# ronantakizawa/cudabulletproof

Measured on AMD Instinct MI355X. Metric: 64-bit range-proof verifies/sec (batched), higher is better.
Workload: dtype u64

## Files before the change

### cudabulletproof_amd/__init__.py

```python
import ctypes
import os
import subprocess

import numpy as np

HERE = os.path.dirname(os.path.abspath(__file__))
ROOT = os.path.dirname(HERE)
LIB_PATH = os.path.join(HERE, "libcudabulletproof_hip.so")
CSRC = os.path.join(HERE, "csrc")
SOURCES = ["bp_terms1.hip", "bp_terms2.hip", "bp_terms4.hip", "bp_terms16.hip", "bp_kernels.hip", "bp_prove.hip",
           "bp_prove_seed.hip", "bp_ipa_prove.hip", "bp_pippenger.hip", "bp_capi.hip"]

_lib = None


class BulletproofError(RuntimeError):
    pass


def build(force=False, verbose=False):
    srcs = [os.path.join(CSRC, s) for s in SOURCES]
    deps = srcs + [os.path.join(CSRC, f) for f in os.listdir(CSRC) if f.endswith(".h")]
    deps.append(os.path.join(ROOT, "include", "cudabulletproof_hip.h"))
    if not force and os.path.exists(LIB_PATH):
        t = os.path.getmtime(LIB_PATH)
        if all(os.path.getmtime(d) <= t for d in deps):
            return LIB_PATH
    import tempfile
    flags = ["--offload-arch=gfx950", "-O3", "-std=c++17", "-fPIC", "-Wno-unused-result"]
    flags += os.environ.get("HIPBP_EXTRA_CFLAGS", "").split()
    with tempfile.TemporaryDirectory() as tmp:
        objs = [os.path.join(tmp, os.path.basename(s) + ".o") for s in srcs]
        procs = []
        for s, o in zip(srcs, objs):
            cmd = ["hipcc"] + flags + ["-c", s, "-o", o]
            if verbose:
                print(" ".join(cmd))
            procs.append((cmd, subprocess.Popen(cmd)))
        for cmd, p in procs:
            if p.wait() != 0:
                raise subprocess.CalledProcessError(p.returncode, cmd)
        cmd = ["hipcc", "--offload-arch=gfx950", "-shared", "-fPIC", "-o", LIB_PATH + ".tmp"] + objs
        if verbose:
            print(" ".join(cmd))
        subprocess.check_call(cmd)
    os.replace(LIB_PATH + ".tmp", LIB_PATH)
    return LIB_PATH


_c = ctypes.c_void_p
_sz = ctypes.c_size_t


class FieldVector(ctypes.Structure):
    _fields_ = [("elements", _c), ("length", _sz)]


PointVector = FieldVector


class InnerProductProof(ctypes.Structure):
    _fields_ = [("n", _sz), ("a", FieldVector), ("b", FieldVector), ("c", ctypes.c_uint64 * 4),
                ("L", PointVector), ("R", PointVector), ("L_len", _sz), ("x", ctypes.c_uint64 * 4)]


class RangeProofC(ctypes.Structure):
    _fields_ = [("V", ctypes.c_uint64 * 16), ("A", ctypes.c_uint64 * 16), ("S", ctypes.c_uint64 * 16),
                ("T1", ctypes.c_uint64 * 16), ("T2", ctypes.c_uint64 * 16), ("taux", ctypes.c_uint64 * 4),
                ("mu", ctypes.c_uint64 * 4), ("t", ctypes.c_uint64 * 4), ("ip_proof", InnerProductProof)]


class ProofBatchC(ctypes.Structure):
    _fields_ = [("count", _sz), ("n", _sz), ("ab_len", _sz), ("L_len", _sz)] + \
               [(k, _c) for k in ("V", "A", "S", "T1", "T2", "t", "a", "b", "c", "x", "L", "R", "taux", "mu", "Vp")]


class ProveInputC(ctypes.Structure):
    _fields_ = [("count", _sz), ("n", _sz)] + [(k, _c) for k in ("v", "gamma", "sL", "sR", "rnd")]


class ProofOutC(ctypes.Structure):
    _fields_ = [(k, _c) for k in ("V", "A", "S", "T1", "T2", "taux", "mu", "t", "c", "x", "a", "b", "L", "R", "valid")]


class ProveIpaInputC(ctypes.Structure):
    _fields_ = [("count", _sz), ("n", _sz)] + [(k, _c) for k in ("a", "b", "c", "transcript")]


class IpaProofOutC(ctypes.Structure):
    _fields_ = [(k, _c) for k in ("a", "b", "c", "x", "c_final", "L", "R")]


assert ctypes.sizeof(InnerProductProof) == 144 and ctypes.sizeof(RangeProofC) == 880

EXPORTS = [
    "cuda_point_vector_multi_scalar_mul", "cuda_point_vector_multi_scalar_mul_shared",
    "cuda_field_vector_inner_product", "cuda_field_vector_inner_product_shared",
    "cuda_batch_field_vector_inner_product", "cuda_batch_field_add", "cuda_batch_field_sub",
    "cuda_batch_field_mul", "cuda_batch_field_mul_karatsuba", "cuda_batch_field_square",
    "cuda_batch_field_invert", "cuda_soa_field_add", "cuda_range_proof_verify", "cuda_inner_product_verify",
    "cuda_benchmark_multi_scalar_mul", "cuda_benchmark_inner_product", "cuda_benchmark_field_operations",
    "cuda_benchmark_range_proof", "hipbp_last_error", "hipbp_device_count", "hipbp_batch_range_proof_verify",
    "hipbp_batch_range_proof_verify_std", "hipbp_batch_range_proof_verify_gens", "hipbp_batch_inner_product_verify", "hipbp_batch_generate_range_proof", "hipbp_msm",
    "hipbp_msm_pippenger", "hipbp_msm_pippenger_batch", "hipbp_msm_pippenger_windows",
    "hipbp_msm_pippenger_horner", "hipbp_msm_batch", "hipbp_msm_batch_gens", "hipbp_point_tree", "hipbp_field_op",
    "hipbp_sha_probe", "hipbp_sync", "hipbp_timing_enable",
    "hipbp_timing_collect", "hipbp_kernel_count", "hipbp_kernel_name", "hipbp_pipeline_create",
    "hipbp_pipeline_push", "hipbp_pipeline_flush", "hipbp_pipeline_depth", "hipbp_pipeline_destroy",
    "hipbp_pipeline_defer_msm",
    "hipbp_release_stream_workspaces",
    "hipbp_batch_inner_product_prove", "hipbp_batch_inner_product_prove_gens", "hipbp_inner_product_prove_host",
    "hipbp_derive_prover_scalars", "hipbp_batch_generate_range_proof_seeded",
    "hipbp_batch_generate_range_proof_seeded_gens", "hipbp_batch_generate_range_proof_host",
    "hipbp_batch_generate_range_proof_accepted", "hipbp_batch_generate_range_proof_accepted_gens",
    "hipbp_derive_prover_scalars_at", "hipbp_accepted_last_stats",
]


def lib():
    global _lib
    if _lib is None:
        if not os.path.exists(LIB_PATH):
            raise BulletproofError(f"{LIB_PATH} missing: run cudabulletproof_amd.build() (hipcc, gfx950)")
        try:
            import torch
        except ImportError:
            pass
        L = ctypes.CDLL(LIB_PATH)
        L.hipbp_last_error.restype = ctypes.c_char_p
        for f in ("cuda_range_proof_verify", "cuda_inner_product_verify"):
            getattr(L, f).restype = ctypes.c_bool
        for f in ("hipbp_batch_range_proof_verify", "hipbp_batch_range_proof_verify_host",
                  "hipbp_batch_range_proof_verify_std", "hipbp_batch_range_proof_verify_gens",
                  "hipbp_batch_inner_product_verify", "hipbp_batch_generate_range_proof", "hipbp_msm",
                  "hipbp_msm_pippenger", "hipbp_msm_pippenger_batch", "hipbp_msm_pippenger_windows",
                  "hipbp_msm_pippenger_horner", "hipbp_msm_batch", "hipbp_msm_batch_gens", "hipbp_point_tree",
                  "hipbp_field_op", "hipbp_sha_probe", "hipbp_sync", "hipbp_device_count",
                  "hipbp_release_stream_workspaces", "hipbp_batch_inner_product_prove",
                  "hipbp_batch_inner_product_prove_gens", "hipbp_inner_product_prove_host",
                  "hipbp_derive_prover_scalars", "hipbp_batch_generate_range_proof_seeded",
                  "hipbp_batch_generate_range_proof_seeded_gens", "hipbp_batch_generate_range_proof_host",
                  "hipbp_batch_generate_range_proof_accepted", "hipbp_batch_generate_range_proof_accepted_gens",
                  "hipbp_derive_prover_scalars_at", "hipbp_accepted_last_stats"):
            getattr(L, f).restype = ctypes.c_int
        _lib = L
    return _lib


def require_gpu():
    n = lib().hipbp_device_count()
    if n < 1:
        raise BulletproofError("no HIP device visible: the engine has no CPU fallback")
    return n


def _chk(rc):
    if rc != 0:
        raise BulletproofError(lib().hipbp_last_error().decode())


def _p(a):
    return ctypes.c_void_p(a.ctypes.data)


def _u64(a, last):
    a = np.ascontiguousarray(a, dtype=np.uint64)
    if a.shape[-1] != last:
        raise ValueError(f"expected trailing dimension {last}, got {a.shape}")
    return a


def cuda_point_vector_multi_scalar_mul(scalars, points, shared=False):
    require_gpu()
    s, P = _u64(scalars, 4), _u64(points, 16)
    if len(s) != len(P):
        raise ValueError("Vector lengths must match for multi-scalar multiplication")
    out = np.zeros(16, np.uint64)
    sv, pv = FieldVector(_p(s).value, len(s)), PointVector(_p(P).value, len(P))
    f = lib().cuda_point_vector_multi_scalar_mul_shared if shared else lib().cuda_point_vector_multi_scalar_mul
    f(_p(out), ctypes.byref(sv), ctypes.byref(pv))
    return out


def cuda_field_vector_inner_product(a, b, shared=False):
    require_gpu()
    a, b = _u64(a, 4), _u64(b, 4)
    out = np.zeros(4, np.uint64)
    av, bv = FieldVector(_p(a).value, len(a)), FieldVector(_p(b).value, len(b))
    f = lib().cuda_field_vector_inner_product_shared if shared else lib().cuda_field_vector_inner_product
    f(_p(out), ctypes.byref(av), ctypes.byref(bv))
    return out


def cuda_batch_field_vector_inner_product(a_vectors, b_vectors):
    require_gpu()
    a, b = _u64(a_vectors, 4), _u64(b_vectors, 4)
    nv, n = a.shape[0], a.shape[1]
    av = (FieldVector * nv)(*[FieldVector(_p(a).value + i * n * 32, n) for i in range(nv)])
    bv = (FieldVector * nv)(*[FieldVector(_p(b).value + i * n * 32, n) for i in range(nv)])
    out = np.zeros((nv, 4), np.uint64)
    lib().cuda_batch_field_vector_inner_product(_p(out), av, bv, _sz(nv))
    return out


def _field(name, a, b=None):
    require_gpu()
    a = _u64(a, 4).reshape(-1, 4)
    out = np.zeros_like(a)
    if b is None:
        getattr(lib(), name)(_p(out), _p(a), _sz(len(a)))
    else:
        b = _u64(b, 4).reshape(-1, 4)
        if len(b) != len(a):
            raise ValueError("length mismatch")
        getattr(lib(), name)(_p(out), _p(a), _p(b), _sz(len(a)))
    return out


def cuda_batch_field_add(a, b):
    return _field("cuda_batch_field_add", a, b)


def cuda_batch_field_sub(a, b):
    return _field("cuda_batch_field_sub", a, b)


def cuda_batch_field_mul(a, b):
    return _field("cuda_batch_field_mul", a, b)


def cuda_batch_field_mul_karatsuba(a, b):
    return _field("cuda_batch_field_mul_karatsuba", a, b)


def cuda_batch_field_square(a):
    return _field("cuda_batch_field_square", a)


def cuda_batch_field_invert(a):
    return _field("cuda_batch_field_invert", a)


def cuda_soa_field_add(a, b):
    return _field("cuda_soa_field_add", a, b)


def _range_proof_struct(proof, n, keep):
    head = np.asarray(proof["head"], np.uint64)
    a, b = _u64(proof["a"], 4), _u64(proof["b"], 4)
    L, R = _u64(proof["L"], 16).reshape(-1, 16), _u64(proof["R"], 16).reshape(-1, 16)
    keep += [a, b, L, R]
    rp = RangeProofC()
    for i, k in enumerate(("V", "A", "S", "T1", "T2")):
        getattr(rp, k)[:] = [int(v) for v in head[16 * i:16 * i + 16]]
    for i, k in enumerate(("taux", "mu", "t")):
        getattr(rp, k)[:] = [int(v) for v in head[80 + 4 * i:84 + 4 * i]]
    ip = rp.ip_proof
    ip.n = n
    ip.a = FieldVector(_p(a).value, len(a))
    ip.b = FieldVector(_p(b).value, len(b))
    ip.c[:] = [int(v) for v in head[92:96]]
    ip.L = PointVector(_p(L).value, len(L))
    ip.R = PointVector(_p(R).value, len(R))
    ip.L_len = len(L)
    ip.x[:] = [int(v) for v in head[96:100]]
    return rp


def cuda_range_proof_verify(proof, V, n, G, H, g, h):
    require_gpu()
    keep = []
    rp = _range_proof_struct(proof, n, keep)
    V, g, h = _u64(V, 16), _u64(g, 16), _u64(h, 16)
    G, H = _u64(G, 16), _u64(H, 16)
    gv, hv = PointVector(_p(G).value, len(G)), PointVector(_p(H).value, len(H))
    return bool(lib().cuda_range_proof_verify(ctypes.byref(rp), _p(V), _sz(n), ctypes.byref(gv), ctypes.byref(hv),
                                              _p(g), _p(h)))


def batch_range_proof_verify_host(proofs, V, n, G, H, g, h, num_gpus=0):
    require_gpu()
    keep = []
    count = len(proofs)
    arr = (RangeProofC * max(count, 1))()
    for i, pr in enumerate(proofs):
        arr[i] = _range_proof_struct(pr, n, keep)
    V = _u64(V, 16).reshape(-1, 16)
    g, h = _u64(g, 16), _u64(h, 16)
    G, H = _u64(G, 16), _u64(H, 16)
    gv, hv = PointVector(_p(G).value, len(G)), PointVector(_p(H).value, len(H))
# ... 263 lines not shown
    require_gpu()
    sd = _seed_arg(seed)
    v, gamma = _u64(v, 4).reshape(-1, 4), _u64(gamma, 4).reshape(-1, 4)
    if len(v) != len(gamma):
        raise ValueError("v and gamma must have the same length")
    G, H, g, h = _u64(G, 16), _u64(H, 16), _u64(g, 16), _u64(h, 16)
    count = len(v)
    arr = (RangeProofC * max(count, 1))()
    valid = np.zeros(max(count, 1), np.uint8)
    gv, hv = PointVector(_p(G).value, len(G)), PointVector(_p(H).value, len(H))
    _chk(lib().hipbp_batch_generate_range_proof_host(arr, _p(valid), _p(v), _p(gamma), _sz(count), _sz(int(n)),
                                                     ctypes.byref(gv), ctypes.byref(hv), _p(g), _p(h), sd,
                                                     ctypes.c_uint64(int(index_base) & (2**64 - 1))))
    proofs = []
    for i in range(count):
        rp = arr[i]
        ip = rp.ip_proof
        head = np.concatenate([np.array(getattr(rp, k), np.uint64) for k in ("V", "A", "S", "T1", "T2", "taux", "mu", "t")] +
                              [np.array(ip.c, np.uint64), np.array(ip.x, np.uint64)])
        proofs.append(dict(head=head, a=_take(ip.a, 4), b=_take(ip.b, 4), L=_take(ip.L, 16), R=_take(ip.R, 16),
                           n=int(ip.n), L_len=int(ip.L_len)))
    return proofs, valid[:count].astype(bool)


def batch_inner_product_prove(n, a, b, c, G, H, Q, transcript=None, stream=None, gens=None):
    import contextlib

    import torch
    B = int(a.shape[0])
    Lr = int(n).bit_length() - 1
    dev = a.device
    with torch.cuda.stream(stream) if stream is not None else contextlib.nullcontext():
        z = lambda *shape: torch.empty(*shape, dtype=torch.int64, device=dev)
        out = dict(a=z(B, 1, 4), b=z(B, 1, 4), c=z(B, 4), x=z(B, 4), c_final=z(B, 4), L=z(B, max(Lr, 0), 16),
                   R=z(B, max(Lr, 0), 16))
    ins = [t.contiguous() for t in (a, b, c)] + [transcript.contiguous() if transcript is not None else None]
    if ins[0].numel() != B * int(n) * 4 or ins[1].numel() != B * int(n) * 4 or ins[2].numel() != B * 4:
        raise BulletproofError("batch_inner_product_prove: a, b must be (B, n, 4) and c (B, 4)")
    ic = ProveIpaInputC(B, int(n), *[t.data_ptr() if t is not None else None for t in ins])
    oc = IpaProofOutC(*[out[k].data_ptr() if out[k].numel() else None for k in ("a", "b", "c", "x", "c_final", "L", "R")])
    if gens is not None:
        _chk(lib().hipbp_batch_inner_product_prove_gens(ctypes.byref(ic), _c(gens.h), ctypes.byref(oc),
                                                        _stream_ptr(stream)))
    else:
        _chk(lib().hipbp_batch_inner_product_prove(ctypes.byref(ic), _c(G.data_ptr()), _c(H.data_ptr()),
                                                   _c(Q.data_ptr()), ctypes.byref(oc), _stream_ptr(stream)))
    out["_keep"] = ins
    return out


def ipa_proof_batch(n, proof, c="c_final"):
    import torch
    if c not in ("c", "c_final"):
        raise ValueError("c must be 'c' or 'c_final'")
    B, dev = int(proof["a"].shape[0]), proof["a"].device
    zp = torch.zeros(B, 16, dtype=torch.int64, device=dev)
    return RangeProofBatch(n, V=zp, A=zp, S=zp, T1=zp, T2=zp, t=torch.zeros(B, 4, dtype=torch.int64, device=dev),
                           a=proof["a"], b=proof["b"], c=proof[c], x=proof["x"], L=proof["L"], R=proof["R"])


def inner_product_prove(a, b, G, H, Q, c, transcript=None):
    require_gpu()
    a, b, G, H = _u64(a, 4), _u64(b, 4), _u64(G, 16), _u64(H, 16)
    Q, c = _u64(Q, 16), _u64(c, 4)
    tr = np.zeros(32, np.uint8) if transcript is None else np.ascontiguousarray(transcript, np.uint8)
    pr = InnerProductProof()
    av, bv = FieldVector(_p(a).value, len(a)), FieldVector(_p(b).value, len(b))
    gv, hv = PointVector(_p(G).value, len(G)), PointVector(_p(H).value, len(H))
    rc = lib().hipbp_inner_product_prove_host(ctypes.byref(pr), ctypes.byref(av), ctypes.byref(bv), ctypes.byref(gv),
                                              ctypes.byref(hv), _p(Q), _p(c), _p(tr))
    if rc != 0:
        if not pr.a.elements and rc == 1:
            return None
        _chk(rc)
    return dict(a=_take(pr.a, 4), b=_take(pr.b, 4), c=np.array(pr.c, np.uint64), x=np.array(pr.x, np.uint64),
                L=_take(pr.L, 16), R=_take(pr.R, 16), L_len=int(pr.L_len), n=int(pr.n))


def msm(result, scalars, points, stream=None):
    _chk(lib().hipbp_msm(_c(result.data_ptr()), _c(scalars.data_ptr()), _c(points.data_ptr()),
                         _sz(points.shape[0]), _stream_ptr(stream)))


def msm_batch(results, scalars, points, stream=None):
    n = points.shape[0]
    count = results.shape[0]
    if scalars.numel() != count * n * 4:
        raise BulletproofError("msm_batch: scalars must hold count * n rows")
    _chk(lib().hipbp_msm_batch(_c(results.data_ptr()), _c(scalars.data_ptr()), _c(points.data_ptr()), _sz(n),
                               _sz(count), _stream_ptr(stream)))


def msm_batch_gens(results, scalars, gens, stream=None):
    count, n2 = results.shape[0], 2 * gens.n
    if scalars.numel() != count * n2 * 4:
        raise BulletproofError("msm_batch_gens: scalars must hold count * 2n rows")
    _chk(lib().hipbp_msm_batch_gens(_c(results.data_ptr()), _c(scalars.data_ptr()), _c(gens.h), _sz(count),
                                    _stream_ptr(stream)))


def msm_pippenger(result, scalars, points, window_bits=12, stream=None):
    _chk(lib().hipbp_msm_pippenger(_c(result.data_ptr()), _c(scalars.data_ptr()), _c(points.data_ptr()),
                                   _sz(points.shape[0]), ctypes.c_int(window_bits), _stream_ptr(stream)))


def msm_pippenger_batch(results, scalars, points, window_bits=12, stream=None):
    count, n = results.shape[0], points.shape[0]
    if scalars.numel() != count * n * 4:
        raise BulletproofError("msm_pippenger_batch: scalars must hold count * n rows")
    _chk(lib().hipbp_msm_pippenger_batch(_c(results.data_ptr()), _c(scalars.data_ptr()), _c(points.data_ptr()),
                                         _sz(n), _sz(count), ctypes.c_int(window_bits), _stream_ptr(stream)))


def pippenger_num_windows(window_bits=12):
    return (256 + int(window_bits) - 1) // int(window_bits)


def msm_pippenger_windows(window_sums, scalars, points, w_begin, w_end, window_bits=12, stream=None):
    W = pippenger_num_windows(window_bits)
    if window_sums.numel() != W * 16:
        raise BulletproofError(f"msm_pippenger_windows: window_sums must be ({W}, 16)")
    if scalars.numel() != points.shape[0] * 4:
        raise BulletproofError("msm_pippenger_windows: one scalar per point")
    _chk(lib().hipbp_msm_pippenger_windows(_c(window_sums.data_ptr()), _c(scalars.data_ptr()),
                                           _c(points.data_ptr()), _sz(points.shape[0]), ctypes.c_int(window_bits),
                                           ctypes.c_int(w_begin), ctypes.c_int(w_end), _stream_ptr(stream)))


def msm_pippenger_horner(results, window_sums, window_bits=12, stream=None):
    W = pippenger_num_windows(window_bits)
    count = results.numel() // 16
    if window_sums.numel() != count * W * 16:
        raise BulletproofError(f"msm_pippenger_horner: window_sums must hold count * {W} rows")
    _chk(lib().hipbp_msm_pippenger_horner(_c(results.data_ptr()), _c(window_sums.data_ptr()), _sz(count),
                                          ctypes.c_int(window_bits), _stream_ptr(stream)))


def release_stream_workspaces(stream=None):
    _chk(lib().hipbp_release_stream_workspaces(_stream_ptr(stream)))


def point_tree(result, points, stream=None):
    _chk(lib().hipbp_point_tree(_c(result.data_ptr()), _c(points.data_ptr()), _sz(points.shape[0]),
                                _stream_ptr(stream)))


def field_op(op, r, a, b=None, stream=None):
    ops = {"add": 0, "sub": 1, "mul": 2, "square": 3, "soa_add": 4, "invert": 5, "fold": 6, "sq": 7,
           "addsub_add": 8, "addsub_sub": 9,
           "mul_q4": 10,
           "mul_k": 11,
           "mul_q4_k": 12,
           "add_lat": 13, "add_defer": 14, "addsub_lat_add": 15, "addsub_lat_sub": 16,
           "addsub_defer_add": 17, "addsub_defer_sub": 18, "fold_lat": 19, "fold_defer": 20}
    _chk(lib().hipbp_field_op(ops[op], _c(r.data_ptr()), _c(a.data_ptr()), _c(b.data_ptr()) if b is not None else None,
                              _sz(a.shape[0]), _stream_ptr(stream)))


def sha_probe(kind, out, inp, stream=None):
    _chk(lib().hipbp_sha_probe(int(kind), _c(out.data_ptr()), _c(inp.data_ptr()), _sz(inp.shape[0]),
                               _stream_ptr(stream)))


def timing_enable(on=True):
    L = lib()
    L.hipbp_timing_enable.restype = ctypes.c_int
    _chk(L.hipbp_timing_enable(1 if on else 0))


def timing_collect():
    L = lib()
    L.hipbp_kernel_name.restype = ctypes.c_char_p
    L.hipbp_timing_collect.restype = ctypes.c_int
    k = L.hipbp_kernel_count()
    ms = (ctypes.c_double * k)()
    cnt = (ctypes.c_uint64 * k)()
    _chk(L.hipbp_timing_collect(ms, cnt))
    return {L.hipbp_kernel_name(i).decode(): (ms[i], cnt[i]) for i in range(k)}


class VerifyPipeline:

    def __init__(self, max_batch, n, G, H, h, range_mode=True, stream=None, g=None):
        L = lib()
        L.hipbp_pipeline_create.restype = ctypes.c_void_p
        L.hipbp_pipeline_push.restype = ctypes.c_int
        L.hipbp_pipeline_flush.restype = ctypes.c_int
        L.hipbp_pipeline_depth.restype = ctypes.c_int
        self._keep = (G, H, h, g)
        self.stream = stream
        self.mode = int(range_mode)
        self.h = L.hipbp_pipeline_create(_sz(max_batch), _sz(n), self.mode, _c(G.data_ptr()), _c(H.data_ptr()),
                                         _c(g.data_ptr()) if g is not None else None, _c(h.data_ptr()),
                                         _stream_ptr(stream))
        if not self.h:
            raise BulletproofError(L.hipbp_last_error().decode())
        self.depth = L.hipbp_pipeline_depth(_c(self.h))

    def push(self, batch, ok=None, P_out=None, check_out=None, P_in=None, flags_out=None, poly_out=None):
        s = batch.c_struct() if batch is not None else None
        opt = lambda t: _c(t.data_ptr()) if t is not None else None
        _chk(lib().hipbp_pipeline_push(
            _c(self.h), ctypes.byref(s) if s is not None else None, opt(P_in), opt(ok), opt(P_out), opt(check_out),
            opt(flags_out), opt(poly_out)))

    def flush(self):
        _chk(lib().hipbp_pipeline_flush(_c(self.h)))

    def use_gens(self, gens):
        _chk(lib().hipbp_pipeline_use_gens(_c(self.h), _c(gens.h)))
        self._gens = gens

    def defer_msm(self, on=True):
        _chk(lib().hipbp_pipeline_defer_msm(_c(self.h), ctypes.c_int(1 if on else 0)))

    def prefix_tables(self, bits):
        _chk(lib().hipbp_pipeline_prefix_tables(_c(self.h), ctypes.c_int(int(bits))))

    def close(self):
        if self.h:
            lib().hipbp_pipeline_destroy(_c(self.h))
            self.h = None

    def __del__(self):
        try:
            self.close()
        except Exception:
            pass
```

### cudabulletproof_amd/csrc/bp_capi.hip

```cpp
#include <hip/hip_runtime.h>
#include <map>
#include <mutex>
#include <string>
#include <vector>
#include <cstdio>
#include <cstdlib>
#include <cstring>
#include <algorithm>
#include <chrono>
#include <thread>

#include "../../include/cudabulletproof_hip.h"
#include "bp_tick_plan.h"
#include "bp_buf.h"
#include "ge25519_dev.h"
#include "bp_prove_seed.h"

static_assert(sizeof(fe25519) == 32, "fe25519 layout");
static_assert(sizeof(ge25519) == 128, "ge25519 layout");
static_assert(sizeof(bp::fe) == 32 && sizeof(bp::ge) == 128, "device layout");
static_assert(sizeof(InnerProductProof) == 144, "InnerProductProof layout (SURVEY 8b)");
static_assert(sizeof(RangeProof) == 880, "RangeProof layout (SURVEY 8b)");

namespace {
// ... 1319 lines not shown
        w.L = Lr ? (bp::ge*)out->L + p0 * Lr : nullptr;
        w.R = Lr ? (bp::ge*)out->R + p0 * Lr : nullptr;
        w.ptab = ptab; w.pbits = ptab ? pbits : 0;
        bp::launch_ipa_load(w, ia + p0 * n, ibv + p0 * n, itr ? itr + p0 : nullptr, st);
        for (int r = 0; r < Lr; r++) bp::launch_ipa_round(w, r, G, H, Q, e.dtab, st);
        bp::launch_ipa_final(w, ic + p0, (bp::fe*)out->a + p0, (bp::fe*)out->b + p0, (bp::fe*)out->c + p0,
                             (bp::fe*)out->x + p0, out->c_final ? (bp::fe*)out->c_final + p0 : nullptr, st);
        BP_RET_ON(hipGetLastError());
    }
    if (chunks > 1) {
        BP_RET_ON(hipEventRecord(ib->ipa_ev[1], ib->ipa_side));
        BP_RET_ON(hipStreamWaitEvent(s, ib->ipa_ev[1], 0));
    }
    return HIPBP_OK;
}

static int ipa_check(const hipbp_ipa_prove_input* in, const hipbp_ipa_proof_out* out) {
    if (!in || !out) { g_err = "ipa prover: null argument"; return HIPBP_ERR_ARG; }
    if (!is_pow2(in->n) || in->n > MAX_N) { g_err = "ipa prover: n must be a power of two <= 65536"; return HIPBP_ERR_ARG; }
    if (in->count > ((size_t)1 << 24)) { g_err = "ipa prover: batch too large"; return HIPBP_ERR_ARG; }
    if (!in->a || !in->b || !in->c) { g_err = "ipa prover: null input"; return HIPBP_ERR_ARG; }
    if (!out->a || !out->b || !out->c || !out->x || (in->n > 1 && (!out->L || !out->R))) {
        g_err = "ipa prover: null output";
        return HIPBP_ERR_ARG;
    }
    return HIPBP_OK;
}

int hipbp_batch_inner_product_prove(const hipbp_ipa_prove_input* in, const ge25519* G, const ge25519* H,
                                    const ge25519* Q, hipbp_ipa_proof_out* out, void* stream) {
    BP_ENGINE_OR_RET(e);
    if (!G || !H || !Q) { g_err = "ipa prover: null generator"; return HIPBP_ERR_ARG; }
    if (int rc = ipa_check(in, out)) return rc;
    if (in->count == 0) return HIPBP_OK;
    std::lock_guard<std::mutex> lk(e->mu);
    return ipa_enqueue(*e, in, (const bp::ge*)G, (const bp::ge*)H, (const bp::ge*)Q, nullptr, 0, out,
                       pick(stream));
}

int hipbp_batch_inner_product_prove_gens(const hipbp_ipa_prove_input* in, void* gens, hipbp_ipa_proof_out* out,
                                         void* stream) {
    BP_ENGINE_OR_RET(e);
    Gens* gs = (Gens*)gens;
    if (!gs) { g_err = "null gens"; return HIPBP_ERR_ARG; }
    if (int rc = ipa_check(in, out)) return rc;
    if (int rc = gens_check(gs, in->n, "ipa prover: input n differs from the generator set's")) return rc;
    if (in->count == 0) return HIPBP_OK;
    std::lock_guard<std::mutex> lk(e->mu);
    return ipa_enqueue(*e, in, gs->G(), gs->H(), gs->h(), gs->bits ? gs->tab.as<bp::ge>() : nullptr, gs->bits, out,
                       pick(stream));
}

int hipbp_inner_product_prove_host(InnerProductProof* proof, const FieldVector* a, const FieldVector* b,
                                   const PointVector* G, const PointVector* H, const ge25519* Q,
                                   const fe25519* c_in, const uint8_t* transcript32) {
    if (!proof || !a || !b || !G || !H || !Q || !c_in) { g_err = "ipa prover: null argument"; return HIPBP_ERR_ARG; }
    if (a->length != b->length || a->length != G->length || a->length != H->length) {
        fprintf(stderr, "Error: Vector lengths must match for inner product proof\n");
        return HIPBP_ERR_ARG;
    }
    const size_t n = a->length;
    if (!is_pow2(n)) {
        fprintf(stderr, "Error: Inner product proof length must be a power of 2\n");
        return HIPBP_ERR_ARG;
    }
    if (n > MAX_N) { g_err = "ipa prover: n must be a power of two <= 65536"; return HIPBP_ERR_ARG; }
    Engine& e = engine_or_exit();
    std::lock_guard<std::mutex> lk(e.mu);
    const size_t FE = sizeof(fe25519), GE = sizeof(ge25519), Lr = (size_t)log2i(n);
    BP_EXIT_ON(e.ipa_stage.need((2 * n + 1 + 2 * Lr) * GE + (2 * n + 6) * FE));
    ge25519* dG = e.ipa_stage.as<ge25519>();
    ge25519 *dH = dG + n, *dQ = dH + n, *dL = dQ + 1, *dR = dL + Lr;
    fe25519* da = (fe25519*)(dR + Lr);
    fe25519 *db = da + n, *dc = db + n, *dt = dc + 1, *oa = dt + 1;
    hipStream_t s = e.stream;
    BP_EXIT_ON(hipMemcpyAsync(dG, G->elements, n * GE, hipMemcpyHostToDevice, s));
    BP_EXIT_ON(hipMemcpyAsync(dH, H->elements, n * GE, hipMemcpyHostToDevice, s));
    BP_EXIT_ON(hipMemcpyAsync(dQ, Q, GE, hipMemcpyHostToDevice, s));
    BP_EXIT_ON(hipMemcpyAsync(da, a->elements, n * FE, hipMemcpyHostToDevice, s));
    BP_EXIT_ON(hipMemcpyAsync(db, b->elements, n * FE, hipMemcpyHostToDevice, s));
    BP_EXIT_ON(hipMemcpyAsync(dc, c_in, FE, hipMemcpyHostToDevice, s));
    if (transcript32) BP_EXIT_ON(hipMemcpyAsync(dt, transcript32, FE, hipMemcpyHostToDevice, s));
    hipbp_ipa_prove_input in{1, n, da, db, dc, transcript32 ? dt : nullptr};
    hipbp_ipa_proof_out out{oa, oa + 1, oa + 2, oa + 3, nullptr, dL, dR};
    if (ipa_enqueue(e, &in, (const bp::ge*)dG, (const bp::ge*)dH, (const bp::ge*)dQ, nullptr, 0, &out, s) != HIPBP_OK) {
        fprintf(stderr, "HIP error in inner_product_prove - %s\n", g_err.c_str());
        exit(EXIT_FAILURE);
    }
    fe25519 res[4];
    if (!bp::proof_vectors_alloc(*proof, n, Lr)) {
        fprintf(stderr, "Error: Failed to allocate memory for field vector\n");
        exit(1);
    }
    BP_EXIT_ON(hipMemcpyAsync(res, oa, 4 * FE, hipMemcpyDeviceToHost, s));
    if (Lr) {
        BP_EXIT_ON(hipMemcpyAsync(proof->L.elements, dL, Lr * GE, hipMemcpyDeviceToHost, s));
        BP_EXIT_ON(hipMemcpyAsync(proof->R.elements, dR, Lr * GE, hipMemcpyDeviceToHost, s));
    }
    BP_EXIT_ON(hipStreamSynchronize(s));
    *proof->a.elements = res[0];
    *proof->b.elements = res[1];
    proof->c = res[2];
    proof->x = res[3];
    return HIPBP_OK;
}

int hipbp_pipeline_use_gens(void* handle, void* gens) {
    Pipeline* pl = (Pipeline*)handle;
    Gens* gs = (Gens*)gens;
    if (!pl || !gs) { g_err = "null pipeline or gens"; return HIPBP_ERR_ARG; }
    if ((int)gs->n != pl->n) { g_err = "pipeline n differs from the generator set's"; return HIPBP_ERR_ARG; }
    if (gs->device != pl->e->device) { g_err = "gens: created on another device"; return HIPBP_ERR_ARG; }
    std::lock_guard<std::mutex> lk(pl->e->mu);
    if (pl->busy()) { g_err = "use_gens: pipeline has batches in flight (flush first)"; return HIPBP_ERR_ARG; }
    BP_RET_ON(hipStreamSynchronize(pl->s));
    BP_RET_ON(pl->ptab.release());
    pl->set_gens(gs->G(), gs->H(), gs->g(), gs->h());
    pl->ext_tab = gs->bits ? gs->tab.as<bp::ge>() : nullptr;
    pl->pbits = gs->bits;
    return HIPBP_OK;
}

int hipbp_pipeline_defer_msm(void* handle, int on) {
    Pipeline* pl = (Pipeline*)handle;
    if (!pl) { g_err = "null pipeline"; return HIPBP_ERR_ARG; }
    if (on && !bp::defer_ok(pl->cfg)) {
        g_err = "defer_msm: needs cuda_range_proof_verify / range_proof_verify semantics, 4 <= n <= the lane-tree limit "
                "and n <= 512 (a split tick's region list)";
        return HIPBP_ERR_ARG;
    }
    std::lock_guard<std::mutex> lk(pl->e->mu);
    pl->defer_msm = on != 0;
    return HIPBP_OK;
}

int hipbp_point_tree(ge25519* result, const ge25519* points, size_t n, void* stream) {
    BP_ENGINE_OR_RET(e);
    if (n == 0) return HIPBP_OK;
    if (!result || !points) { g_err = "null argument"; return HIPBP_ERR_ARG; }
    std::lock_guard<std::mutex> lk(e->mu);
    hipStream_t s = pick(stream);
    Buf(&w)[bp::MB_COUNT] = e->streams[s].msm;
    size_t sz[bp::MB_COUNT];
    bp::tree_sizes(n, sz);
    BP_RET_ON(need_all(w, sz));
    bp::launch_tree_full((bp::ge*)result, (const bp::ge*)points, n, w[bp::MB_TREE0].as<bp::ge>(),
                         w[bp::MB_TREE1].as<bp::ge>(), s);
    BP_RET_ON(hipGetLastError());
    return HIPBP_OK;
}

int hipbp_field_op(int op, fe25519* r, const fe25519* a, const fe25519* b, size_t count, void* stream) {
    BP_ENGINE_OR_RET(e);
    if (op < 0 || op > 20) { g_err = "bad op"; return HIPBP_ERR_ARG; }
    if (!a || (!b && op != 3 && op != 5 && op != 7 && op != 11 && op != 12)) { g_err = "null operand"; return HIPBP_ERR_ARG; }
    if (count == 0) return HIPBP_OK;
    hipStream_t s = pick(stream);
    if (op == 5)
        bp::launch_invert((bp::fe*)r, (const bp::fe*)a, count, s);
    else
        bp::launch_field_op(op, (bp::fe*)r, (const bp::fe*)a, (const bp::fe*)b, count, s);
    BP_RET_ON(hipGetLastError());
    return HIPBP_OK;
}

int hipbp_sha_probe(int kind, fe25519* out, const fe25519* in, size_t count, void* stream) {
    BP_ENGINE_OR_RET(e);
    if (kind < 0 || kind > 5) { g_err = "bad sha probe kind"; return HIPBP_ERR_ARG; }
    if (!out || !in) { g_err = "null operand"; return HIPBP_ERR_ARG; }
    if (count == 0) return HIPBP_OK;
    bp::launch_sha_probe(kind, (bp::fe*)out, (const bp::fe*)in, count, pick(stream));
    BP_RET_ON(hipGetLastError());
    return HIPBP_OK;
}


void cuda_point_vector_multi_scalar_mul(ge25519* result, const FieldVector* scalars, const PointVector* points) {
    if (scalars->length != points->length) {
        fprintf(stderr, "Error: Vector lengths must match for multi-scalar multiplication\n");
        return;
    }
    size_t n = scalars->length;
    if (n == 0) return;
    Engine& e = engine_or_exit();
    std::lock_guard<std::mutex> lk(e.mu);
    BP_EXIT_ON(e.op_a.need(n * sizeof(fe25519)));
    BP_EXIT_ON(e.op_b.need(n * sizeof(ge25519)));
    BP_EXIT_ON(e.op_out.need(sizeof(ge25519)));
    BP_EXIT_ON(hipMemcpyAsync(e.op_a.p, scalars->elements, n * sizeof(fe25519), hipMemcpyHostToDevice, e.stream));
    BP_EXIT_ON(hipMemcpyAsync(e.op_b.p, points->elements, n * sizeof(ge25519), hipMemcpyHostToDevice, e.stream));
    BP_EXIT_ON(msm_run(e, e.op_out.as<bp::ge>(), e.op_a.as<bp::fe>(), e.op_b.as<bp::ge>(), n, 1, e.stream));
    BP_EXIT_ON(hipMemcpyAsync(result, e.op_out.p, sizeof(ge25519), hipMemcpyDeviceToHost, e.stream));
    BP_EXIT_ON(hipStreamSynchronize(e.stream));
}

void cuda_point_vector_multi_scalar_mul_shared(ge25519* result, const FieldVector* scalars,
                                               const PointVector* points) {
    cuda_point_vector_multi_scalar_mul(result, scalars, points);
}

static void ip_common(fe25519* result, const FieldVector* a, const FieldVector* b, bool force_shared) {
    if (a->length != b->length) {
        fprintf(stderr, "Error: Vector lengths must match for inner product\n");
        return;
    }
    size_t n = a->length;
    if (n == 0) return;
    Engine& e = engine_or_exit();
    std::lock_guard<std::mutex> lk(e.mu);
    BP_EXIT_ON(e.op_a.need(n * sizeof(fe25519)));
    BP_EXIT_ON(e.op_b.need(n * sizeof(fe25519)));
    BP_EXIT_ON(e.op_out.need(sizeof(fe25519)));
    BP_EXIT_ON(e.ip_part.need(1024 * sizeof(fe25519)));
    BP_EXIT_ON(hipMemcpyAsync(e.op_a.p, a->elements, n * sizeof(fe25519), hipMemcpyHostToDevice, e.stream));
    BP_EXIT_ON(hipMemcpyAsync(e.op_b.p, b->elements, n * sizeof(fe25519), hipMemcpyHostToDevice, e.stream));
    if (force_shared || n <= 512)
        bp::launch_ip_shared(e.op_out.as<bp::fe>(), e.op_a.as<bp::fe>(), e.op_b.as<bp::fe>(), n, e.stream);
    else
        bp::launch_ip_grid(e.op_out.as<bp::fe>(), e.ip_part.as<bp::fe>(), e.op_a.as<bp::fe>(),
                           e.op_b.as<bp::fe>(), n, e.stream);
    BP_EXIT_ON(hipGetLastError());
    BP_EXIT_ON(hipMemcpyAsync(result, e.op_out.p, sizeof(fe25519), hipMemcpyDeviceToHost, e.stream));
    BP_EXIT_ON(hipStreamSynchronize(e.stream));
}

void cuda_field_vector_inner_product(fe25519* result, const FieldVector* a, const FieldVector* b) {
    ip_common(result, a, b, false);
}

void cuda_field_vector_inner_product_shared(fe25519* result, const FieldVector* a, const FieldVector* b) {
    ip_common(result, a, b, true);
}

void cuda_batch_field_vector_inner_product(fe25519* results, const FieldVector* a_vectors,
                                           const FieldVector* b_vectors, size_t num_vectors) {
    if (num_vectors == 0) return;
    size_t n = a_vectors[0].length;
    Engine& e = engine_or_exit();
    std::lock_guard<std::mutex> lk(e.mu);
    size_t tot = num_vectors * n;
    BP_EXIT_ON(e.op_a.need(tot * sizeof(fe25519) + 32));
    BP_EXIT_ON(e.op_b.need(tot * sizeof(fe25519) + 32));
    BP_EXIT_ON(e.op_out.need(num_vectors * sizeof(fe25519)));
    for (size_t i = 0; i < num_vectors; i++) {
        BP_EXIT_ON(hipMemcpyAsync(e.op_a.as<fe25519>() + i * n, a_vectors[i].elements, n * sizeof(fe25519),
                                  hipMemcpyHostToDevice, e.stream));
        BP_EXIT_ON(hipMemcpyAsync(e.op_b.as<fe25519>() + i * n, b_vectors[i].elements, n * sizeof(fe25519),
                                  hipMemcpyHostToDevice, e.stream));
    }
    bp::launch_ip_batch(e.op_out.as<bp::fe>(), e.op_a.as<bp::fe>(), e.op_b.as<bp::fe>(), n, num_vectors, e.stream);
    BP_EXIT_ON(hipGetLastError());
    BP_EXIT_ON(hipMemcpyAsync(results, e.op_out.p, num_vectors * sizeof(fe25519), hipMemcpyDeviceToHost, e.stream));
    BP_EXIT_ON(hipStreamSynchronize(e.stream));
}

static void field_common(int op, fe25519* results, const fe25519* a, const fe25519* b, size_t count) {
    if (count == 0) return;
    Engine& e = engine_or_exit();
    std::lock_guard<std::mutex> lk(e.mu);
    BP_EXIT_ON(e.op_a.need(count * sizeof(fe25519)));
    BP_EXIT_ON(e.op_b.need(count * sizeof(fe25519)));
    BP_EXIT_ON(e.op_out.need(count * sizeof(fe25519)));
    BP_EXIT_ON(hipMemcpyAsync(e.op_a.p, a, count * sizeof(fe25519), hipMemcpyHostToDevice, e.stream));
    if (b) BP_EXIT_ON(hipMemcpyAsync(e.op_b.p, b, count * sizeof(fe25519), hipMemcpyHostToDevice, e.stream));
    if (op == 5)
        bp::launch_invert(e.op_out.as<bp::fe>(), e.op_a.as<bp::fe>(), count, e.stream);
    else
        bp::launch_field_op(op, e.op_out.as<bp::fe>(), e.op_a.as<bp::fe>(), e.op_b.as<bp::fe>(), count, e.stream);
    BP_EXIT_ON(hipGetLastError());
    BP_EXIT_ON(hipMemcpyAsync(results, e.op_out.p, count * sizeof(fe25519), hipMemcpyDeviceToHost, e.stream));
    BP_EXIT_ON(hipStreamSynchronize(e.stream));
}

void cuda_batch_field_add(fe25519* r, const fe25519* a, const fe25519* b, size_t count) { field_common(0, r, a, b, count); }
void cuda_batch_field_sub(fe25519* r, const fe25519* a, const fe25519* b, size_t count) { field_common(1, r, a, b, count); }
void cuda_batch_field_mul(fe25519* r, const fe25519* a, const fe25519* b, size_t count) { field_common(2, r, a, b, count); }
void cuda_batch_field_mul_karatsuba(fe25519* r, const fe25519* a, const fe25519* b, size_t count) {
    field_common(2, r, a, b, count);
}
void cuda_batch_field_square(fe25519* r, const fe25519* in, size_t count) { field_common(3, r, in, nullptr, count); }
void cuda_batch_field_invert(fe25519* r, const fe25519* in, size_t count) { field_common(5, r, in, nullptr, count); }
void cuda_soa_field_add(fe25519* r, const fe25519* a, const fe25519* b, size_t count) { field_common(4, r, a, b, count); }

static bool stage_single(Engine& e, const InnerProductProof* ip, const RangeProof* rp, const ge25519* V,
                         hipbp_proof_batch* b) {
    size_t abl = ip->a.length, Lr = ip->L_len;
    if (ip->b.length != abl || abl == 0 || ip->L.length < Lr || ip->R.length < Lr) return false;
    const bp::ChunkLayout lay{1, abl, Lr};
    const size_t bytes = lay.bytes();
    BP_EXIT_ON(e.proof1.need(bytes));
    BP_EXIT_ON(e.need_pinned(bytes));
    BP_EXIT_ON(hipStreamSynchronize(e.stream));
    lay.pack(e.pinned.p, 0, *ip, rp, V);
    BP_EXIT_ON(hipMemcpyAsync(e.proof1.p, e.pinned.p, bytes, hipMemcpyHostToDevice, e.stream));
    lay.view(e.proof1.p, b);
    return true;
}

static bool verify_single(const InnerProductProof* ip, const RangeProof* rp, const ge25519* V, const ge25519* P,
                          size_t n, const PointVector* G, const PointVector* H, const ge25519* h) {
    Engine& e = engine_or_exit();
    std::lock_guard<std::mutex> lk(e.mu);
    hipbp_proof_batch b;
    memset(&b, 0, sizeof b);
    if (!stage_single(e, ip, rp, V, &b)) return false;
    b.n = n;
    const size_t cap0 = e.gens1.cap;
    BP_EXIT_ON(e.gens1.need(2 * n * sizeof(ge25519) + 3 * sizeof(ge25519)));
    if (e.gens1.cap != cap0) e.single_gens.clear();
    ge25519* dg = e.gens1.as<ge25519>();
    const size_t GB = n * sizeof(ge25519);
    std::vector<uint8_t>& sg = e.single_gens;
    const bool same = e.single_gens_dev == (const void*)dg && sg.size() == 2 * GB + sizeof(ge25519) &&
                      memcmp(sg.data(), G->elements, GB) == 0 && memcmp(sg.data() + GB, H->elements, GB) == 0 &&
// ... 428 lines not shown
```

### cudabulletproof_amd/csrc/bp_kernels.h

```cpp
#pragma once
#include <hip/hip_runtime.h>
#include <stddef.h>
#include <stdint.h>

namespace bp {
struct fe;
struct ge;

struct BatchView {
    int B;
    int n;
    int ab_len;
    int L_len;
    const ge* V;
    const ge* A;
    const ge* S;
    const ge* T1;
    const ge* T2;
    const fe* t;
    const fe* a;
    const fe* b;
    const fe* c;
    const fe* x;
    const ge* L;
// ... 103 lines not shown
}

__host__ __device__ inline bool round_per_lane(int n, int r) { return (n >> r) < 64; }

constexpr int MSM_BINS = 513;

enum SortSetKind { SS_STAGE0 = 0, SS_ROUND = 1, SS_FT = 2 };
constexpr int LANE_SORT_SETS = 18;
constexpr int LANE_SORT_BLOCK = 256;
struct LaneSortPlan {
    int count;
    int pad;
    const SlotDev* slot;
    struct Set {
        int kind, r;
        unsigned long long items;
        uint32_t* perm;
        unsigned block0;
        unsigned pad;
    } set[LANE_SORT_SETS];
    unsigned blocks;
    int longest_first;
};
void launch_lane_sort(const LaneSortPlan& plan, unsigned* bins, unsigned* offs, hipStream_t s);

enum RegionKind { RK_STAGE0 = 0, RK_ROUND = 1, RK_FINAL_TERMS = 2, RK_FINAL = 4, RK_PREP = 5,
                  RK_TREE = 6, RK_POLY = 7, RK_M3 = 8,
                  RK_LTREE = 9 ,
                  RK_MSMT = 10  };
struct Region {
    int kind;
    int slot;
    int r;
    int pad;
    unsigned long long begin;
    unsigned long long items;
};
constexpr int LANE_TREE_MAX = 64;
constexpr int MAX_REGIONS = 24;
struct RegionList {
    int count;
    int pad;
    unsigned long long total;
    Region reg[MAX_REGIONS];
};

enum KernelKind { KT_PREP = 0, KT_TERMS, KT_TREE, KT_COMBINE, KT_COUNT };

void launch_prefix_tables(ge* tab, const ge* G, const ge* H, const ge* h, const ge* g, int n, int K, hipStream_t s);
void launch_terms(const RegionList& rl, const SlotDev* slots, const ge* G, const ge* H, const ge* g, const ge* h,
                  const ge* dtab, const fe* two_i, hipStream_t s, int ql = 1);
void launch_upload(void* dst, const void* src, size_t bytes, hipStream_t s);
#define BP_DECL_TERMS(Q)                                                                                    \
    void launch_terms##Q(const RegionList& rl, const SlotDev* slots, const ge* G, const ge* H, const ge* g,  \
                         const ge* h, const ge* dtab, const fe* two_i, hipStream_t s, unsigned lds_pad);
BP_DECL_TERMS(1)
BP_DECL_TERMS(2)
BP_DECL_TERMS(4)
BP_DECL_TERMS(16)
#undef BP_DECL_TERMS
inline bool region_is_sm(int kind) {
    return kind == RK_STAGE0 || kind == RK_ROUND || kind == RK_FINAL_TERMS || kind == RK_M3 || kind == RK_MSMT;
}
inline int region_lanes(int kind, int ql) {
    if (region_is_sm(kind)) return ql;
    return (ql >= 4 && (kind == RK_FINAL || kind == RK_LTREE || kind == RK_PREP)) ? 4 : 1;
}

constexpr size_t MSM_SORT_MIN = 4096;
void launch_msm_points(ge* pts, const fe* scal, const ge* P, size_t m, uint32_t* perm, unsigned* bins,
                       const ge* dtab, hipStream_t s, size_t pm = 0, const ge* ptab = nullptr, int K = 0);
void launch_tree(ge* out, const ge* in, int S, size_t m, hipStream_t s);
void launch_ops_scan(unsigned* bins, int longest_first, hipStream_t s);
struct PipPair;
hipError_t msm_pippenger(PipPair& pp, ge* result, const fe* scal, const ge* P, size_t n, size_t count, int c,
                         const ge* dtab, hipStream_t s);
hipError_t msm_pippenger_windows(PipPair& pp, ge* Sw, const fe* scal, const ge* P, size_t n, int c, int w0, int w1,
                                 const ge* dtab, hipStream_t s);
hipError_t pippenger_horner(ge* result, const ge* Sw, size_t count, int c, hipStream_t s);



struct ProveIn {
    int B, n, L;
    const fe* v;
    const fe* gamma;
    const fe* sL;
    const fe* sR;
    const fe* rnd;
};
struct ProveOut {
    ge *V, *A, *S, *T1, *T2;
    fe *taux, *mu, *t, *c, *x, *a, *b;
    ge *L, *R;
    uint8_t* valid;
};
struct ProveWs {
    fe* ps;
    ge* pterm;
    ge* chain;
    ge* pts;
    fe* st;
    fe* tsc;
    ge* tt;
    fe* acur;
    fe* bcur;
    fe* iscal;
    fe* csc;
    ge* iterm;
    fe* misc;
    uint8_t* valid;
    uint32_t* list;
    unsigned* cnt;
    size_t cap;
    ge* ctab;
    uint32_t* slist;
    unsigned* sbins;
    const ge* ptab;
    int pbits;
};
enum ProveStage { PS_PREP = 0, PS_TERMS0, PS_CHAIN0, PS_COMMIT, PS_TERMS1, PS_TX, PS_RTERMS, PS_RCHAIN, PS_ROUND,
                  PS_FINAL, PS_SORT0  };
void launch_prove(int stage, int r, const ProveIn& in, const ProveWs& ws, const ProveOut& out, const ge* G,
                  const ge* H, const ge* g, const ge* h, const ge* dtab, const fe* two_i, hipStream_t s);

struct IpaWs {
    int B, n, Lr;
    fe* a;
    fe* b;
    fe* prod;
    fe* sc;
    fe* csc;
    ge* term;
    ge* cq;
    ge* chain;
    fe* tr;
    fe* uu;
    fe* x;
    uint32_t* slist;
    uint32_t* llist;
    unsigned* ctl;
    ge* L;
    ge* R;
    const ge* ptab;
    int pbits;
};
void launch_ipa_load(const IpaWs& ws, const fe* a, const fe* b, const fe* tr , hipStream_t s);
void launch_ipa_round(const IpaWs& ws, int r, const ge* G, const ge* H, const ge* Q, const ge* dtab, hipStream_t s);
void launch_ipa_final(const IpaWs& ws, const fe* c_in, fe* a, fe* b, fe* c, fe* x, fe* c_final ,
                      hipStream_t s);

void launch_field_op(int op, fe* r, const fe* a, const fe* b, size_t count, hipStream_t s);
void launch_sha_probe(int kind, fe* out, const fe* in, size_t count, hipStream_t s);
void launch_ip_shared(fe* out, const fe* a, const fe* b, size_t n, hipStream_t s);
void launch_ip_grid(fe* out, fe* part, const fe* a, const fe* b, size_t n, hipStream_t s);
void launch_ip_batch(fe* out, const fe* a, const fe* b, size_t n, size_t nvec, hipStream_t s);
void launch_invert(fe* r, const fe* a, size_t count, hipStream_t s);
void launch_tree_full(ge* result, const ge* in, size_t n, ge* part0, ge* part1, hipStream_t s, int S = 1);
void launch_msm_full(ge* result, const fe* scal, const ge* P, size_t n, ge* ptsbuf, ge* part0, ge* part1,
                     uint32_t* perm, unsigned* bins, const ge* dtab, hipStream_t s, size_t count = 1,
                     const ge* ptab = nullptr, int K = 0);
}
```

### cudabulletproof_amd/csrc/bp_kernels.hip

```cpp
#include "bp_kernels.h"
#include "ge25519_dev.h"
#include "ge25519_quad.h"
#include "sha256_dev.h"

namespace bp {

constexpr int TPB = 256;
#ifndef BP_TERMS_OCC
#define BP_TERMS_OCC 4
#endif


__device__ __forceinline__ size_t gid() { return (size_t)blockIdx.x * blockDim.x + threadIdx.x; }

__global__ __launch_bounds__(TPB) void k_prefix_tables(ge* tab, const ge* __restrict__ G, const ge* __restrict__ H,
                                                       const ge* __restrict__ h, const ge* __restrict__ g, int n,
                                                       int K, size_t total) {
    const size_t i = gid();
    if (i >= total) return;
    const size_t b = i >> K;
    const uint32_t p = (uint32_t)(i & ((1ull << K) - 1));
    const ge* P = b < (size_t)n ? &G[b] : b < 2 * (size_t)n ? &H[b - n] : b == 2 * (size_t)n ? h : g;
    if (!P) return;
    const geq q = ge_prep(*P);
// ... 123 lines not shown
void launch_tree(ge* out, const ge* in, int S, size_t m, hipStream_t s) {
    int nb = (int)((m + TPB - 1) / TPB);
    k_tree<<<S * nb, TPB, 0, s>>>(out, in, m, nb);
}

__device__ __forceinline__ int lane_key(const SlotDev& sd, int kind, int r, size_t j) {
    const BatchView& bv = sd.bv;
    const VerifyWs& ws = sd.ws;
    const size_t B = bv.B;
    const int n = bv.n, Lr = bv.L_len;
    fe s;
    int K = 0;
    if (kind == SS_STAGE0) {
        size_t i = stage0_class_item(sd, r, (uint32_t)j);
        if (sd.ptab) K = sd.pbits;
        const size_t nA = sd.range_mode ? B * 2 * n : 0, nB = Lr > 0 ? B * 2 * n : 0;
        if (i < nA) {
            size_t seg = i / n, p = seg >> 1;
            s = (seg & 1) ? ws.sH[p * n + i % n] : ws.sG[p];
        } else if (i - nA < nB) {
            i -= nA;
            size_t p = i / (2 * n);
            int grp = (int)(i % (2 * n)) / (n >> 1);
            s = grp < 2 ? ws.uinv[p * Lr] : ws.u[p * Lr];
        } else if (i - nA - nB < 2 * B) {
            i -= nA + nB;
            bool isC = i & 1;
            if (!isC && !sd.range_mode) return 0;
            s = ws.sc[(i >> 1) * 4 + (isC ? 3 : 0)];
        } else {
            i -= nA + nB + 2 * B;
            s = ws.psc[(i / 7) * 8 + i % 7];
            const int k = (int)(i % 7);
            if (k == 2 || k == 5 || k == 6) K = 0;
        }
    } else if (kind == SS_ROUND) {
        const int np = n >> (r + 1);
        size_t p = j / (4 * np);
        int grp = (int)(j % (4 * np)) / np;
        s = grp < 2 ? ws.uinv[p * Lr + r] : ws.u[p * Lr + r];
    } else {
        s = ws.sc[(j >> 1) * 4 + ((j & 1) ? 2 : 1)];
    }
    return sm_ops_prefix(s, K);
}

__device__ __forceinline__ int lane_set_of(const LaneSortPlan& pl, unsigned b, LaneSortPlan::Set& st) {
    int idx = 0;
    st = pl.set[0];
#pragma unroll
    for (int k = 1; k < LANE_SORT_SETS; k++)
        if (k < pl.count && b >= pl.set[k].block0) { st = pl.set[k]; idx = k; }
    return idx;
}

__global__ __launch_bounds__(LANE_SORT_BLOCK) void k_lane_hist(LaneSortPlan pl, unsigned* bins) {
    __shared__ unsigned h[OPS_BINS];
    for (int k = threadIdx.x; k < OPS_BINS; k += LANE_SORT_BLOCK) h[k] = 0;
    __syncthreads();
    LaneSortPlan::Set st;
    const int si = lane_set_of(pl, blockIdx.x, st);
    const size_t j = (size_t)(blockIdx.x - st.block0) * LANE_SORT_BLOCK + threadIdx.x;
    if (j < st.items) atomicAdd(&h[lane_key(*pl.slot, st.kind, st.r, j)], 1u);
    __syncthreads();
    for (int k = threadIdx.x; k < OPS_BINS; k += LANE_SORT_BLOCK)
        if (h[k]) atomicAdd(&bins[si * OPS_BINS + k], h[k]);
}

constexpr int LS_PER = (OPS_BINS + LANE_SORT_BLOCK - 1) / LANE_SORT_BLOCK;
__global__ __launch_bounds__(LANE_SORT_BLOCK) void k_lane_scan(unsigned* bins, unsigned* offs, int longest_first) {
    __shared__ unsigned wsum[LANE_SORT_BLOCK / 64];
    const int t = threadIdx.x;
    unsigned* bb = bins + (size_t)blockIdx.x * OPS_BINS;
    unsigned v[LS_PER], sum = 0;
#pragma unroll
    for (int u = 0; u < LS_PER; u++) {
        const int p = LS_PER * t + u, k = longest_first ? OPS_BINS - 1 - p : p;
        v[u] = p < OPS_BINS ? bb[k] : 0u;
        sum += v[u];
    }
    unsigned inc = sum;
#pragma unroll
    for (int d = 1; d < 64; d <<= 1) {
        const unsigned x = __shfl_up(inc, d, 64);
        if ((t & 63) >= d) inc += x;
    }
    if ((t & 63) == 63) wsum[t >> 6] = inc;
    __syncthreads();
    unsigned run = inc - sum;
    for (int w = 0; w < (t >> 6); w++) run += wsum[w];
#pragma unroll
    for (int u = 0; u < LS_PER; u++) {
        const int p = LS_PER * t + u, k = longest_first ? OPS_BINS - 1 - p : p;
        if (p < OPS_BINS) {
            offs[(size_t)blockIdx.x * OPS_BINS + k] = run;
            bb[k] = 0;
        }
        run += v[u];
    }
}

__global__ __launch_bounds__(LANE_SORT_BLOCK) void k_lane_scatter(LaneSortPlan pl, unsigned* offs) {
    __shared__ unsigned cnt[OPS_BINS], base[OPS_BINS];
    for (int k = threadIdx.x; k < OPS_BINS; k += LANE_SORT_BLOCK) cnt[k] = 0;
    __syncthreads();
    LaneSortPlan::Set st;
    const int si = lane_set_of(pl, blockIdx.x, st);
    const size_t j = (size_t)(blockIdx.x - st.block0) * LANE_SORT_BLOCK + threadIdx.x;
    int key = 0;
    unsigned rank = 0;
    if (j < st.items) {
        key = lane_key(*pl.slot, st.kind, st.r, j);
        rank = atomicAdd(&cnt[key], 1u);
    }
    __syncthreads();
    for (int k = threadIdx.x; k < OPS_BINS; k += LANE_SORT_BLOCK)
        if (cnt[k]) base[k] = atomicAdd(&offs[si * OPS_BINS + k], cnt[k]);
    __syncthreads();
    if (j < st.items) st.perm[base[key] + rank] = (uint32_t)j;
}

void launch_lane_sort(const LaneSortPlan& plan, unsigned* bins, unsigned* offs, hipStream_t s) {
    if (!plan.count || !plan.blocks) return;
    k_lane_hist<<<plan.blocks, LANE_SORT_BLOCK, 0, s>>>(plan, bins);
    k_lane_scan<<<plan.count, LANE_SORT_BLOCK, 0, s>>>(bins, offs, plan.longest_first);
    k_lane_scatter<<<plan.blocks, LANE_SORT_BLOCK, 0, s>>>(plan, offs);
}

static inline unsigned nblk(size_t items) { return (unsigned)((items + TPB - 1) / TPB); }

void launch_terms(const RegionList& rl, const SlotDev* slots, const ge* G, const ge* H, const ge* g, const ge* h,
                  const ge* dtab, const fe* two_i, hipStream_t s, int ql) {
    if (!rl.total) return;
    static const unsigned pad = [] { const char* e = getenv("HIPBP_TERMS_LDS_PAD"); return e ? (unsigned)atoi(e) : 0u; }();
    if (ql == 16) launch_terms16(rl, slots, G, H, g, h, dtab, two_i, s, pad);
    else if (ql == 4) launch_terms4(rl, slots, G, H, g, h, dtab, two_i, s, pad);
    else if (ql == 2) launch_terms2(rl, slots, G, H, g, h, dtab, two_i, s, pad);
    else launch_terms1(rl, slots, G, H, g, h, dtab, two_i, s, pad);
}


__global__ __launch_bounds__(TPB) void k_field_op(int op, fe* r, const fe* __restrict__ a, const fe* __restrict__ b,
                                                  size_t count) {
    size_t i = gid();
    if (op == 10 || op == 12) {
        i >>= 2;
        if (i >= count) return;
        const fe z = op == 10 ? fe_mul_q4(a[i], b[i]) : fe_mul_q4_k(a[i]);
        if ((threadIdx.x & 3) == 0) r[i] = z;
        return;
    }
    if (i >= count) return;
    fe x = a[i], y;
    if (op != 3 && op != 7 && op != 11) y = b[i];
    fe z;
    switch (op) {
        case 0: z = fe_add(x, y); break;
        case 1: z = fe_sub(x, y); break;
        case 2: z = fe_mul(x, y); break;
        case 3: z = fe_square_kernel_quirk(x); break;
        case 6: {
            uint64_t t[8] = {x.v[0], x.v[1], x.v[2], x.v[3], y.v[0], y.v[1], y.v[2], y.v[3]};
            z = fe_fold512(t);
            break;
        }
        case 7: z = fe_sq(x); break;
        case 11: z = fe_mul_k(x); break;
        case 8:
        case 9: {
            fe sm, df;
            fe_addsub(x, y, sm, df);
            z = op == 8 ? sm : df;
            break;
        }
        case 13: z = fe_add<1>(x, y); break;
        case 14: {
            uint32_t acc = 0;
            z = fe_add<2>(x, y, &acc);
            if (acc == 0xFFFFFFFFu) z = fe_add<1>(x, y);
            break;
        }
        case 15:
        case 16: {
            fe sm, df;
            fe_addsub<1>(x, y, sm, df);
            z = op == 15 ? sm : df;
            break;
        }
        case 17:
        case 18: {
            fe sm, df;
            uint32_t acc = 0;
            fe_addsub<2>(x, y, sm, df, &acc);
            if (acc == 0xFFFFFFFFu) fe_addsub<1>(x, y, sm, df);
            z = op == 17 ? sm : df;
            break;
        }
        case 19:
        case 20: {
            uint64_t t[8] = {x.v[0], x.v[1], x.v[2], x.v[3], y.v[0], y.v[1], y.v[2], y.v[3]};
            if (op == 19) {
                z = fe_fold512<1>(t);
            } else {
                uint32_t acc = 0;
                z = fe_fold512<2>(t, &acc);
                if (acc == 0xFFFFFFFFu) z = fe_fold512<1>(t);
            }
            break;
        }
        default:
#pragma unroll
            for (int k = 0; k < 4; k++) z.v[k] = x.v[k] + y.v[k];
            break;
    }
    r[i] = z;
}

__global__ __launch_bounds__(TPB) void k_sha_probe(int kind, fe* out, const fe* __restrict__ in, size_t count) {
    const size_t i = gid();
    if (i >= count) return;
    const fe* f = in + i * 6;
    auto pt = [&](int k) { return ge{f[k], f[k + 1], fe_set(1), fe_set(0)}; };
    fe r;
    switch (kind) {
        case 0: r = chal_y(pt(0), pt(2), pt(4)); break;
        case 1: r = chal_z(f[0]); break;
        case 2: r = chal_x(pt(0), pt(2)); break;
        case 3: r = chal_ip(f[0], f[1], f[2]); break;
        case 4: r = chal_ip_start(f[0], f[1], f[2]); break;
        default: r = sha_4fe(f[0], f[1], f[2], f[3]); break;
    }
    out[i] = r;
}

void launch_sha_probe(int kind, fe* out, const fe* in, size_t count, hipStream_t s) {
    if (count == 0) return;
    k_sha_probe<<<nblk(count), TPB, 0, s>>>(kind, out, in, count);
}

void launch_field_op(int op, fe* r, const fe* a, const fe* b, size_t count, hipStream_t s) {
    if (count == 0) return;
    k_field_op<<<nblk(op == 10 || op == 12 ? 4 * count : count), TPB, 0, s>>>(op, r, a, b, count);
}


__device__ __forceinline__ fe fe_wave_tail(fe v, int tid, unsigned st, size_t lim) {
    for (; st > 0; st >>= 1) {
        fe o;
#pragma unroll
        for (int i = 0; i < 4; i++) {
            uint32_t lo = (uint32_t)__shfl_down((int)(uint32_t)v.v[i], st, 64);
            uint32_t hi = (uint32_t)__shfl_down((int)(uint32_t)(v.v[i] >> 32), st, 64);
            o.v[i] = (uint64_t)lo | ((uint64_t)hi << 32);
        }
        if (tid < (int)st && (size_t)(tid + st) < lim) v = fe_add(v, o);
    }
    return v;
}

__global__ __launch_bounds__(512) void k_ip_shared(fe* out, const fe* __restrict__ a, const fe* __restrict__ b,
                                                   size_t n) {
    __shared__ fe sh[512];
    int tid = threadIdx.x;
    sh[tid] = fe_mul(a[tid], b[tid]);
    __syncthreads();
    unsigned st = blockDim.x / 2;
    for (; st > 32; st >>= 1) {
        if (tid < (int)st && (size_t)(tid + st) < n) sh[tid] = fe_add(sh[tid], sh[tid + st]);
        __syncthreads();
    }
    if (tid < 64) {
        fe v = sh[tid];
        v = fe_wave_tail(v, tid, st, n);
        if (tid == 0) *out = v;
    }
}

__global__ __launch_bounds__(TPB) void k_ip_grid(fe* out, const fe* __restrict__ a, const fe* __restrict__ b,
                                                 size_t n, size_t grid_threads, int warp_tail) {
    (void)warp_tail;
    __shared__ fe sh[TPB];
    int tid = threadIdx.x;
    size_t vec = blockIdx.y;
    a += vec * n;
    b += vec * n;
    fe acc = fe_set(0);
    for (size_t idx = (size_t)blockIdx.x * TPB + tid; idx < n; idx += grid_threads) acc = fe_add(acc, fe_mul(a[idx], b[idx]));
    sh[tid] = acc;
    __syncthreads();
    unsigned st = TPB / 2;
    for (; st > 32; st >>= 1) {
        if (tid < (int)st) sh[tid] = fe_add(sh[tid], sh[tid + st]);
        __syncthreads();
    }
    if (tid < 64) {
        fe v = sh[tid];
        v = fe_wave_tail(v, tid, st, TPB);
        if (tid == 0) out[vec * gridDim.x + blockIdx.x] = v;
    }
}

__global__ __launch_bounds__(TPB) void k_ip_reduce(fe* out, const fe* __restrict__ part, size_t np) {
    __shared__ fe sh[TPB];
    int tid = threadIdx.x;
    sh[tid] = (size_t)tid < np ? part[tid] : fe_set(0);
    __syncthreads();
    unsigned st = TPB / 2;
    for (; st > 32; st >>= 1) {
        if (tid < (int)st && (size_t)(tid + st) < np) sh[tid] = fe_add(sh[tid], sh[tid + st]);
        __syncthreads();
    }
    if (tid < 64) {
        fe v = sh[tid];
        v = fe_wave_tail(v, tid, st, np);
        if (tid == 0) *out = v;
    }
}

void launch_ip_shared(fe* out, const fe* a, const fe* b, size_t n, hipStream_t s) {
    unsigned nt = (unsigned)(n < 512 ? n : 512);
    if (nt == 0) return;
    k_ip_shared<<<1, nt, 0, s>>>(out, a, b, n);
}

void launch_ip_grid(fe* out, fe* part, const fe* a, const fe* b, size_t n, hipStream_t s) {
    size_t nb = (n + TPB - 1) / TPB;
    if (nb > 1024) nb = 1024;
    k_ip_grid<<<dim3((unsigned)nb, 1), TPB, 0, s>>>(part, a, b, n, nb * TPB, 0);
    k_ip_reduce<<<1, TPB, 0, s>>>(out, part, nb);
}

void launch_ip_batch(fe* out, const fe* a, const fe* b, size_t n, size_t nvec, hipStream_t s) {
    size_t nb = (n + TPB - 1) / TPB;
    if (nb > 1024) nb = 1024;
    if (nb == 0) nb = 1;
    k_ip_grid<<<dim3(1, (unsigned)nvec), TPB, 0, s>>>(out, a, b, n, nb * TPB, 1);
}

__global__ __launch_bounds__(TPB) void k_invert(fe* r, const fe* __restrict__ a, size_t count) {
    size_t i = gid();
    if (i < count) r[i] = fe_invert(a[i]);
}
void launch_invert(fe* r, const fe* a, size_t count, hipStream_t s) {
    if (count) k_invert<<<nblk(count), TPB, 0, s>>>(r, a, count);
}

void launch_tree_full(ge* result, const ge* in, size_t n, ge* part0, ge* part1, hipStream_t s, int S) {
    size_t m = n;
    ge* bufs[2] = {part0, part1};
    int w = 0;
    while (true) {
        size_t nb = (m + TPB - 1) / TPB;
        ge* out = (nb == 1) ? result : bufs[w];
        launch_tree(out, in, S, m, s);
        if (nb == 1) break;
        in = out;
        m = nb;
        w ^= 1;
    }
}

void launch_msm_full(ge* result, const fe* scal, const ge* P, size_t n, ge* ptsbuf, ge* part0, ge* part1,
                     uint32_t* perm, unsigned* bins, const ge* dtab, hipStream_t s, size_t count, const ge* ptab,
                     int K) {
    launch_msm_points(ptsbuf, scal, P, n * count, perm, bins, dtab, s, n, ptab, K);
    launch_tree_full(result, ptsbuf, n, part0, part1, s, (int)count);
}

}
```

### cudabulletproof_amd/csrc/fe25519_dev.h

```cpp
#pragma once
#include <hip/hip_runtime.h>
#include <stdint.h>

#ifndef BP_MUL_ASM
#define BP_MUL_ASM 1
#endif
#include "mul512_asm.h"
#ifndef BP_FIELD_ASM
#define BP_FIELD_ASM 1
#endif
#include "field_asm.h"

namespace bp {

struct fe {
    uint64_t v[4];
};

#define BP_DEV __host__ __device__ __forceinline__

constexpr uint64_t P0 = 0xFFFFFFFFFFFFFFEDull;
constexpr uint64_t P3 = 0x7FFFFFFFFFFFFFFFull;
constexpr uint64_t M64 = 0xFFFFFFFFFFFFFFFFull;

BP_DEV fe fe_set(uint64_t x) { return fe{{x, 0, 0, 0}}; }

BP_DEV bool fe_ge_p(const fe& t) {
    bool top = (t.v[3] >> 63) != 0;
    bool eq = (t.v[3] == P3) & (t.v[2] == M64) & (t.v[1] == M64) & (t.v[0] >= P0);
    return top | eq;
}

BP_DEV fe fe_lossy_sub_p(const fe& t) {
    fe d;
    uint64_t br1 = t.v[0] < P0;
    d.v[0] = t.v[0] + 19;
    d.v[1] = t.v[1] + 1 - br1;
    uint64_t br2 = (br1 == 0) & (t.v[1] != M64);
    d.v[2] = t.v[2] + 1 - br2;
    uint64_t br3 = (br2 == 0) & (t.v[2] != M64);
    d.v[3] = t.v[3] - P3 - br3;
    return d;
}

BP_DEV fe fe_cond_sub_p(const fe& t, bool m) {
    bool br1 = t.v[0] < P0;
    bool br2 = !br1 & (t.v[1] != M64);
    bool br3 = !br2 & (t.v[2] != M64);
    fe o;
    o.v[0] = t.v[0] + (m ? 19ull : 0ull);
    o.v[1] = t.v[1] + (uint64_t)(m & !br1);
    o.v[2] = t.v[2] + (uint64_t)(m & !br2);
    o.v[3] = t.v[3] + (m ? (0x8000000000000000ull + (uint64_t)!br3) : 0ull);
    return o;
}

BP_DEV fe fe_fix(const fe& t, bool carry) {
    bool lt0 = t.v[0] < P0;
    bool f1 = t.v[1] == M64, f2 = t.v[2] == M64;
    bool top = (int64_t)t.v[3] < 0;
    bool e3 = t.v[3] == P3;
    bool m = carry | top | (e3 & f2 & f1 & !lt0);
    bool br2 = !lt0 & !f1;
    bool br3 = !br2 & !f2;
    fe o;
    o.v[0] = t.v[0] + (m ? 19ull : 0ull);
    o.v[1] = t.v[1] + (uint64_t)(m & !lt0);
    o.v[2] = t.v[2] + (uint64_t)(m & !br2);
    o.v[3] = t.v[3] + (m ? (0x8000000000000000ull + (uint64_t)!br3) : 0ull);
    return o;
}

BP_DEV uint64_t mul19(uint64_t x) {
#ifdef __HIP_DEVICE_COMPILE__
    uint64_t y, z;
    asm("v_lshl_add_u64 %0, %1, 4, %1" : "=v"(y) : "v"(x));
    asm("v_lshl_add_u64 %0, %1, 1, %2" : "=v"(z) : "v"(x), "v"(y));
    return z;
#else
    return x * 19ull;
#endif
}

BP_DEV fe fe_canon(const fe& t) {
#if BP_FIELD_ASM && defined(__HIP_DEVICE_COMPILE__)
    uint32_t a[8], o[8];
#pragma unroll
    for (int i = 0; i < 4; i++) {
        a[2 * i] = (uint32_t)t.v[i];
        a[2 * i + 1] = (uint32_t)(t.v[i] >> 32);
    }
    fe_canon_asm(o, a);
    return fe{{(uint64_t)o[0] | ((uint64_t)o[1] << 32), (uint64_t)o[2] | ((uint64_t)o[3] << 32),
               (uint64_t)o[4] | ((uint64_t)o[5] << 32), (uint64_t)o[6] | ((uint64_t)o[7] << 32)}};
#else
    return fe_cond_sub_p(t, fe_ge_p(t));
#endif
}

BP_DEV uint32_t lo32(uint64_t x) { return (uint32_t)x; }
BP_DEV uint32_t hi32(uint64_t x) { return (uint32_t)(x >> 32); }
BP_DEV uint64_t cat64(uint32_t lo, uint32_t hi) { return (uint64_t)lo | ((uint64_t)hi << 32); }

template <int LAT = 0>
BP_DEV fe fe_add(const fe& f, const fe& g, uint32_t* acc = nullptr) {
#if BP_FIELD_ASM && defined(__HIP_DEVICE_COMPILE__)
    uint32_t a[8], b[8], o[8];
#pragma unroll
    for (int i = 0; i < 4; i++) {
        a[2 * i] = lo32(f.v[i]); a[2 * i + 1] = hi32(f.v[i]);
        b[2 * i] = lo32(g.v[i]); b[2 * i + 1] = hi32(g.v[i]);
    }
    if constexpr (LAT == 2) fe_add_asm_lat_acc(o, a, b, *acc); else if constexpr (LAT == 1) fe_add_asm_lat(o, a, b); else fe_add_asm(o, a, b);
    return fe{{cat64(o[0], o[1]), cat64(o[2], o[3]), cat64(o[4], o[5]), cat64(o[6], o[7])}};
#else
    fe h;
    unsigned c = 0;
#pragma unroll
    for (int i = 0; i < 4; i++) {
        uint32_t l = __builtin_addc(lo32(f.v[i]), lo32(g.v[i]), c, &c);
        uint32_t u = __builtin_addc(hi32(f.v[i]), hi32(g.v[i]), c, &c);
        h.v[i] = cat64(l, u);
    }
    return fe_fix(h, c != 0);
#endif
}

BP_DEV fe fe_sub(const fe& f, const fe& g) {
#if BP_FIELD_ASM && defined(__HIP_DEVICE_COMPILE__)
    uint32_t a[8], b[8], o[8];
#pragma unroll
    for (int i = 0; i < 4; i++) {
        a[2 * i] = lo32(f.v[i]); a[2 * i + 1] = hi32(f.v[i]);
        b[2 * i] = lo32(g.v[i]); b[2 * i + 1] = hi32(g.v[i]);
    }
    fe_sub_asm(o, a, b);
    return fe{{cat64(o[0], o[1]), cat64(o[2], o[3]), cat64(o[4], o[5]), cat64(o[6], o[7])}};
#else
    fe t;
    unsigned br = 0;
#pragma unroll
    for (int i = 0; i < 4; i++) {
        unsigned b1, b2;
        uint32_t l = __builtin_subc(lo32(f.v[i]), lo32(g.v[i]), br, &b1);
        uint32_t u = __builtin_subc(hi32(f.v[i]), hi32(g.v[i]), b1, &b2);
        t.v[i] = cat64(l, u);
        br = b2 & !((g.v[i] == M64) & (br != 0));
    }
    const bool m = br != 0;
    fe o;
    o.v[0] = t.v[0] - (m ? 19ull : 0ull);
    bool cy0 = t.v[0] >= 19;
    o.v[1] = t.v[1] - (uint64_t)(m & !cy0);
    bool cy1 = o.v[1] != M64;
    o.v[2] = t.v[2] - (uint64_t)(m & !cy1);
    bool cy2 = o.v[2] != M64;
    o.v[3] = t.v[3] + (m ? (cy2 ? 0x8000000000000000ull : P3) : 0ull);
    return o;
#endif
}

template <int LAT = 0>
BP_DEV void fe_addsub(const fe& f, const fe& g, fe& sum, fe& diff, uint32_t* acc = nullptr) {
#if BP_FIELD_ASM && defined(__HIP_DEVICE_COMPILE__)
    uint32_t a[8], b[8], os[8], od[8];
#pragma unroll
    for (int i = 0; i < 4; i++) {
        a[2 * i] = lo32(f.v[i]); a[2 * i + 1] = hi32(f.v[i]);
        b[2 * i] = lo32(g.v[i]); b[2 * i + 1] = hi32(g.v[i]);
    }
    if constexpr (LAT == 2) fe_addsub_asm_lat_acc(os, od, a, b, *acc);
    else if constexpr (LAT == 1) fe_addsub_asm_lat(os, od, a, b);
    else fe_addsub_asm(os, od, a, b);
    sum = fe{{cat64(os[0], os[1]), cat64(os[2], os[3]), cat64(os[4], os[5]), cat64(os[6], os[7])}};
    diff = fe{{cat64(od[0], od[1]), cat64(od[2], od[3]), cat64(od[4], od[5]), cat64(od[6], od[7])}};
#else
    sum = fe_add(f, g);
    diff = fe_sub(f, g);
#endif
}

template <int LAT = 0>
BP_DEV fe fe_fold512(const uint64_t t[8], uint32_t* acc = nullptr) {
#if BP_FIELD_ASM && defined(__HIP_DEVICE_COMPILE__)
    uint32_t a[8], xh[8], o[8];
#pragma unroll
    for (int i = 0; i < 4; i++) {
        uint64_t x = mul19(t[i + 4]);
        a[2 * i] = lo32(t[i]); a[2 * i + 1] = hi32(t[i]);
        xh[2 * i] = lo32(x); xh[2 * i + 1] = hi32(x);
    }
    if constexpr (LAT == 2) fe_fold_asm_lat_acc(o, a, xh, *acc); else if constexpr (LAT == 1) fe_fold_asm_lat(o, a, xh); else fe_fold_asm(o, a, xh);
    return fe{{cat64(o[0], o[1]), cat64(o[2], o[3]), cat64(o[4], o[5]), cat64(o[6], o[7])}};
#else
    fe h;
    unsigned cy = 0;
#pragma unroll
    for (int i = 0; i < 4; i++) {
        uint64_t x = mul19(t[i + 4]);
        unsigned k, c;
        uint32_t l = __builtin_addc(lo32(t[i]), lo32(x), cy, &k);
        uint32_t u = __builtin_addc(hi32(t[i]), hi32(x), k, &c);
        h.v[i] = cat64(l, u);
        cy = c & !((x == M64) & (cy != 0));
    }
    return fe_fix(h, cy != 0);
#endif
}

BP_DEV void mul512(uint64_t t[8], const fe& f, const fe& g) {
    uint32_t a[8], b[8], w[16];
#pragma unroll
    for (int i = 0; i < 4; i++) {
        a[2 * i] = (uint32_t)f.v[i];
        a[2 * i + 1] = (uint32_t)(f.v[i] >> 32);
        b[2 * i] = (uint32_t)g.v[i];
        b[2 * i + 1] = (uint32_t)(g.v[i] >> 32);
    }
#if BP_MUL_ASM && defined(__HIP_DEVICE_COMPILE__)
    mul512_bounded_asm(w, a, b);
    if (__builtin_expect(__any(max(a[0], b[7]) > MUL_BOUNDED_WORD), 0)) mul512_asm(w, a, b);
#else
    uint64_t acc = 0;
    uint32_t c2 = 0;
#pragma unroll
    for (int k = 0; k < 15; k++) {
#pragma unroll
        for (int i = 0; i < 8; i++) {
            int j = k - i;
            if (j < 0 || j > 7) continue;
            uint64_t p = (uint64_t)a[i] * b[j];
            acc += p;
            c2 += acc < p;
        }
        w[k] = (uint32_t)acc;
        acc = (acc >> 32) | ((uint64_t)c2 << 32);
        c2 = 0;
    }
    w[15] = (uint32_t)acc;
#endif
#pragma unroll
    for (int i = 0; i < 8; i++) t[i] = (uint64_t)w[2 * i] | ((uint64_t)w[2 * i + 1] << 32);
}

BP_DEV fe fe_mul(const fe& f, const fe& g) {
    uint64_t t[8];
    mul512(t, f, g);
    return fe_fold512(t);
}

BP_DEV void sqr512(uint64_t t[8], const fe& f) {
    uint32_t a[8], o[16], w[16];
#pragma unroll
    for (int i = 0; i < 4; i++) {
        a[2 * i] = (uint32_t)f.v[i];
        a[2 * i + 1] = (uint32_t)(f.v[i] >> 32);
    }
#if BP_MUL_ASM && defined(__HIP_DEVICE_COMPILE__)
    sqr512_offdiag_bounded_asm(o, a);
    if (__builtin_expect(__any(max(a[0], a[7]) > MUL_BOUNDED_WORD), 0)) sqr512_offdiag_asm(o, a);
#else
    uint64_t acc = 0;
    uint32_t c2 = 0;
    o[0] = 0;
#pragma unroll
    for (int k = 1; k < 14; k++) {
#pragma unroll
        for (int i = 0; i < 8; i++) {
            int j = k - i;
            if (j <= i || j > 7) continue;
            uint64_t p = (uint64_t)a[i] * a[j];
            acc += p;
            c2 += acc < p;
        }
        o[k] = (uint32_t)acc;
        acc = (acc >> 32) | ((uint64_t)c2 << 32);
        c2 = 0;
    }
    o[14] = (uint32_t)acc;
    o[15] = (uint32_t)(acc >> 32);
#endif
    unsigned c = 0;
    uint64_t d0 = (uint64_t)a[0] * a[0];
    w[0] = (uint32_t)d0;
    w[1] = __builtin_addc(o[1] << 1, (uint32_t)(d0 >> 32), 0u, &c);
#pragma unroll
    for (int i = 1; i < 8; i++) {
        uint64_t di = (uint64_t)a[i] * a[i];
        uint32_t lo = (o[2 * i] << 1) | (o[2 * i - 1] >> 31);
        uint32_t hi = (o[2 * i + 1] << 1) | (o[2 * i] >> 31);
        w[2 * i] = __builtin_addc(lo, (uint32_t)di, c, &c);
        w[2 * i + 1] = __builtin_addc(hi, (uint32_t)(di >> 32), c, &c);
    }
#pragma unroll
    for (int i = 0; i < 8; i++) t[i] = (uint64_t)w[2 * i] | ((uint64_t)w[2 * i + 1] << 32);
}

BP_DEV fe fe_sq(const fe& f) {
    uint64_t t[8];
    sqr512(t, f);
    return fe_fold512(t);
}

BP_DEV fe fe_mul_one(const fe& f) { return fe_canon(f); }

BP_DEV fe fe_invert(const fe& f) {
    fe f2 = fe_sq(f);
    fe t1 = fe_sq(f2);
    t1 = fe_sq(t1);
    t1 = fe_mul(t1, f);
    fe t0 = fe_mul(t1, f2);
    t1 = fe_sq(t0);
    t1 = fe_sq(t1);
    t1 = fe_sq(t1);
    t1 = fe_sq(t1);
    t1 = fe_mul(t1, t1);
    fe t2 = fe_mul(f2, f);
    return fe_mul(t1, t2);
}

BP_DEV bool fe_is_one(const fe& f) {
    return (f.v[0] == 1) & (f.v[1] == 0) & (f.v[2] == 0) & (f.v[3] == 0);
}

BP_DEV bool fe_eq(const fe& a, const fe& b) {
    return (a.v[0] == b.v[0]) & (a.v[1] == b.v[1]) & (a.v[2] == b.v[2]) & (a.v[3] == b.v[3]);
}

BP_DEV fe fe_square_kernel_quirk(const fe& f) {
    uint64_t t[8] = {0, 0, 0, 0, 0, 0, 0, 0};
#pragma unroll
    for (int i = 0; i < 4; i++) {
        unsigned __int128 d = (unsigned __int128)f.v[i] * f.v[i];
        t[2 * i] += (uint64_t)d;
        if (2 * i + 1 < 8) t[2 * i + 1] += (uint64_t)(d >> 64);
#pragma unroll
        for (int j = i + 1; j < 4; j++) {
            unsigned __int128 m = ((unsigned __int128)f.v[i] * f.v[j]) << 1;
            t[i + j] += (uint64_t)m;
            if (i + j + 1 < 8) t[i + j + 1] += (uint64_t)(m >> 64);
        }
    }
    return fe_fold512(t);
}

BP_DEV uint32_t fe_byte(const fe& f, int i) { return (uint32_t)(f.v[i >> 3] >> (8 * (i & 7))) & 0xff; }

BP_DEV uint32_t fe_bit(const fe& s, int i) { return (uint32_t)(s.v[i >> 6] >> (i & 63)) & 1u; }

}
```

### cudabulletproof_amd/csrc/field_asm.h

```cpp
#pragma once
#include <stdint.h>
namespace bp {
__device__ __forceinline__ void fe_fix_fast_asm(uint32_t& h0, uint32_t& h1, uint32_t& h4, uint32_t& h7, uint32_t m1) {
    uint64_t l0 = (uint64_t)h0 | ((uint64_t)h1 << 32), sd;
    asm("v_mad_u64_u32 %[l0], %[sd], %[m1], 19, %[l0]\n\tv_add_u32 %[h4], %[h4], %[m1]\n\tv_lshl_add_u32 %[h7], %[m1], 31, %[h7]"
                 : [l0] "+v"(l0), [h4] "+v"(h4), [h7] "+v"(h7), [sd] "=&s"(sd)
                 : [m1] "v"(m1));
    h0 = (uint32_t)l0; h1 = (uint32_t)(l0 >> 32);
    (void)sd;
}
__device__ __forceinline__ void fe_subp_fast_asm(uint32_t& h0, uint32_t& h1, uint32_t& h7, uint32_t mn) {
    uint64_t l0 = (uint64_t)h0 | ((uint64_t)h1 << 32), sd;
    asm("v_mad_i64_i32 %[l0], %[sd], %[mn], 19, %[l0]\n\tv_lshl_add_u32 %[h7], %[mn], 31, %[h7]"
                 : [l0] "+v"(l0), [h7] "+v"(h7), [sd] "=&s"(sd)
                 : [mn] "v"(mn));
    h0 = (uint32_t)l0; h1 = (uint32_t)(l0 >> 32);
    (void)sd;
}

__device__ __forceinline__ void fe_add_asm(uint32_t o0[8], const uint32_t fa[8], const uint32_t ga[8]) {
    const uint32_t a0 = fa[0], a1 = fa[1], a2 = fa[2], a3 = fa[3], a4 = fa[4], a5 = fa[5], a6 = fa[6], a7 = fa[7];
    const uint32_t b0 = ga[0], b1 = ga[1], b2 = ga[2], b3 = ga[3], b4 = ga[4], b5 = ga[5], b6 = ga[6], b7 = ga[7];
    uint32_t h0, h1, h2, h3, h4, h5, h6, h7, vt1, vt2, vt3;
    uint64_t scy, srare;
// ... 64 lines not shown
                 : [p0l] "s"(0xFFFFFFEDu)
                 : "scc");
    out[0] = h0;
    out[1] = h1;
    out[2] = h2;
    out[3] = h3;
    out[4] = h4;
    out[5] = h5;
    out[6] = h6;
    out[7] = h7;
    (void)sf1; (void)sf2; (void)se3; (void)stp; (void)sg0; (void)sg1; (void)sm; (void)sd1; (void)sd2; (void)sd3; (void)sk0; (void)sk1; (void)sk2; (void)sk3; (void)srare; (void)vt1; (void)vt2; (void)vt3; (void)vt4;
}

__device__ __forceinline__ void fe_addsub_asm(uint32_t o0[8], uint32_t o1[8], const uint32_t fa[8], const uint32_t ga[8]) {
    const uint32_t a0 = fa[0], a1 = fa[1], a2 = fa[2], a3 = fa[3], a4 = fa[4], a5 = fa[5], a6 = fa[6], a7 = fa[7];
    const uint32_t b0 = ga[0], b1 = ga[1], b2 = ga[2], b3 = ga[3], b4 = ga[4], b5 = ga[5], b6 = ga[6], b7 = ga[7];
    uint32_t h0, h1, h2, h3, h4, h5, h6, h7, t0, t1, t2, t3, t4, t5, t6, t7, vt1, vt2, vt3, vt4, vt5;
    uint64_t scy, sby, srare;
    asm volatile("v_max3_u32 %[vt3], %[b2], %[b4], %[b6]\n\tv_add_co_u32 %[h0], %[scy], %[a0], %[b0]\n\tv_sub_co_u32 %[t0], %[sby], %[a0], %[b0]\n\tv_addc_co_u32 %[h1], %[scy], %[a1], %[b1], %[scy]\n\tv_subb_co_u32 %[t1], %[sby], %[a1], %[b1], %[sby]\n\tv_addc_co_u32 %[h2], %[scy], %[a2], %[b2], %[scy]\n\tv_subb_co_u32 %[t2], %[sby], %[a2], %[b2], %[sby]\n\tv_addc_co_u32 %[h3], %[scy], %[a3], %[b3], %[scy]\n\tv_subb_co_u32 %[t3], %[sby], %[a3], %[b3], %[sby]\n\tv_addc_co_u32 %[h4], %[scy], %[a4], %[b4], %[scy]\n\tv_subb_co_u32 %[t4], %[sby], %[a4], %[b4], %[sby]\n\tv_not_b32 %[vt4], %[t1]\n\tv_max3_u32 %[vt3], %[vt3], %[h1], %[h4]\n\tv_max3_u32 %[vt3], %[vt3], %[vt4], %[t2]\n\tv_max_u32 %[vt3], %[vt3], %[t4]\n\tv_cmp_eq_u32 %[srare], -1, %[vt3]\n\tv_addc_co_u32 %[h5], %[scy], %[a5], %[b5], %[scy]\n\tv_subb_co_u32 %[t5], %[sby], %[a5], %[b5], %[sby]\n\tv_addc_co_u32 %[h6], %[scy], %[a6], %[b6], %[scy]\n\tv_subb_co_u32 %[t6], %[sby], %[a6], %[b6], %[sby]\n\tv_addc_co_u32 %[h7], %[scy], %[a7], %[b7], %[scy]\n\tv_subb_co_u32 %[t7], %[sby], %[a7], %[b7], %[sby]\n\tv_lshrrev_b32 %[vt1], 31, %[h7]\n\tv_cndmask_b32 %[vt1], %[vt1], 1, %[scy]\n\tv_cndmask_b32 %[vt4], 0, -1, %[sby]"
                 : [h0] "=&v"(h0), [h1] "=&v"(h1), [h2] "=&v"(h2), [h3] "=&v"(h3), [h4] "=&v"(h4), [h5] "=&v"(h5), [h6] "=&v"(h6), [h7] "=&v"(h7), [t0] "=&v"(t0), [t1] "=&v"(t1), [t2] "=&v"(t2), [t3] "=&v"(t3), [t4] "=&v"(t4), [t5] "=&v"(t5), [t6] "=&v"(t6), [t7] "=&v"(t7), [vt1] "=&v"(vt1), [vt3] "=&v"(vt3), [vt4] "=&v"(vt4), [scy] "=&s"(scy), [sby] "=&s"(sby), [srare] "=&s"(srare)
                 : [a0] "v"(a0), [a1] "v"(a1), [a2] "v"(a2), [a3] "v"(a3), [a4] "v"(a4), [a5] "v"(a5), [a6] "v"(a6), [a7] "v"(a7), [b0] "v"(b0), [b1] "v"(b1), [b2] "v"(b2), [b3] "v"(b3), [b4] "v"(b4), [b5] "v"(b5), [b6] "v"(b6), [b7] "v"(b7));
    fe_fix_fast_asm(h0, h1, h4, h7, vt1);
    fe_subp_fast_asm(t0, t1, t7, vt4);
    if (__builtin_expect(srare != 0, 0)) {
        uint64_t sf1, sf2, se3, stp, sg0, sg1, sm, sd1, sd2, sd3, sk0, sk1, sk2, sk3, scy, sby, sq1, sq2, sq3;
        asm volatile("v_add_co_u32 %[h0], %[scy], %[a0], %[b0]\n\ts_nop 0\n\tv_addc_co_u32 %[h1], %[scy], %[a1], %[b1], %[scy]\n\ts_nop 0\n\tv_addc_co_u32 %[h2], %[scy], %[a2], %[b2], %[scy]\n\ts_nop 0\n\tv_addc_co_u32 %[h3], %[scy], %[a3], %[b3], %[scy]\n\ts_nop 0\n\tv_addc_co_u32 %[h4], %[scy], %[a4], %[b4], %[scy]\n\ts_nop 0\n\tv_addc_co_u32 %[h5], %[scy], %[a5], %[b5], %[scy]\n\ts_nop 0\n\tv_addc_co_u32 %[h6], %[scy], %[a6], %[b6], %[scy]\n\ts_nop 0\n\tv_addc_co_u32 %[h7], %[scy], %[a7], %[b7], %[scy]\n\tv_and_b32 %[vt1], %[h2], %[h3]\n\tv_and_b32 %[vt2], %[h4], %[h5]\n\tv_or_b32 %[vt3], %[c80], %[h7]\n\tv_cmp_eq_u32 %[sf1], -1, %[vt1]\n\tv_cmp_eq_u32 %[sf2], -1, %[vt2]\n\tv_and_b32 %[vt3], %[vt3], %[h6]\n\tv_cmp_eq_u32 %[se3], -1, %[vt3]\n\tv_cmp_gt_i32 %[stp], 0, %[h7]\n\tv_cmp_eq_u32 %[sg0], -1, %[h1]\n\tv_cmp_le_u32 %[sg1], %[p0l], %[h0]\n\ts_and_b64 %[sg0], %[sg0], %[sg1]\n\ts_and_b64 %[se3], %[se3], %[sf1]\n\ts_and_b64 %[se3], %[se3], %[sf2]\n\ts_and_b64 %[se3], %[se3], %[sg0]\n\ts_or_b64 %[sm], %[scy], %[stp]\n\ts_or_b64 %[sm], %[sm], %[se3]\n\ts_and_b64 %[sd1], %[sm], %[sg0]\n\ts_orn2_b64 %[sg1], %[sf1], %[sg0]\n\ts_and_b64 %[sd2], %[sm], %[sg1]\n\ts_andn2_b64 %[sg1], %[sg0], %[sf1]\n\ts_or_b64 %[sg1], %[sg1], %[sf2]\n\ts_and_b64 %[sd3], %[sm], %[sg1]\n\tv_cndmask_b32 %[vt1], 0, 19, %[sm]\n\tv_cndmask_b32 %[vt2], 0, %[c80], %[sm]\n\tv_add_co_u32 %[h0], %[sk0], %[h0], %[vt1]\n\tv_addc_co_u32 %[h2], %[sk1], %[h2], 0, %[sd1]\n\tv_addc_co_u32 %[h4], %[sk2], %[h4], 0, %[sd2]\n\tv_addc_co_u32 %[h6], %[sk3], %[h6], 0, %[sd3]\n\tv_addc_co_u32 %[h1], %[sk0], %[h1], 0, %[sk0]\n\tv_addc_co_u32 %[h3], %[sk1], %[h3], 0, %[sk1]\n\tv_addc_co_u32 %[h5], %[sk2], %[h5], 0, %[sk2]\n\tv_addc_co_u32 %[h7], %[sk3], %[h7], %[vt2], %[sk3]\n\tv_and_b32 %[vt1], %[b2], %[b3]\n\tv_cmp_eq_u32 %[sq1], -1, %[vt1]\n\tv_and_b32 %[vt1], %[b4], %[b5]\n\tv_cmp_eq_u32 %[sq2], -1, %[vt1]\n\tv_and_b32 %[vt1], %[b6], %[b7]\n\tv_cmp_eq_u32 %[sq3], -1, %[vt1]\n\tv_sub_co_u32 %[t0], %[sk0], %[a0], %[b0]\n\ts_nop 0\n\tv_subb_co_u32 %[t1], %[sby], %[a1], %[b1], %[sk0]\n\ts_nop 0\n\tv_subb_co_u32 %[t2], %[sk0], %[a2], %[b2], %[sby]\n\ts_nop 0\n\tv_subb_co_u32 %[t3], %[sk1], %[a3], %[b3], %[sk0]\n\ts_and_b64 %[sq1], %[sq1], %[sby]\n\ts_andn2_b64 %[sby], %[sk1], %[sq1]\n\tv_subb_co_u32 %[t4], %[sk0], %[a4], %[b4], %[sby]\n\ts_nop 0\n\tv_subb_co_u32 %[t5], %[sk1], %[a5], %[b5], %[sk0]\n\ts_and_b64 %[sq2], %[sq2], %[sby]\n\ts_andn2_b64 %[sby], %[sk1], %[sq2]\n\tv_subb_co_u32 %[t6], %[sk0], %[a6], %[b6], %[sby]\n\ts_nop 0\n\tv_subb_co_u32 %[t7], %[sk1], %[a7], %[b7], %[sk0]\n\ts_and_b64 %[sq3], %[sq3], %[sby]\n\ts_andn2_b64 %[sby], %[sk1], %[sq3]\n\tv_cndmask_b32 %[vt1], 0, 19, %[sby]\n\tv_cndmask_b32 %[vt2], 0, %[c80], %[sby]\n\tv_sub_co_u32 %[t0], %[sk0], %[t0], %[vt1]\n\ts_nop 0\n\tv_subb_co_u32 %[t1], %[sd1], %[t1], 0, %[sk0]\n\ts_nop 0\n\tv_subb_co_u32 %[t2], %[sk1], %[t2], 0, %[sd1]\n\ts_nop 0\n\tv_subb_co_u32 %[t3], %[sk1], %[t3], 0, %[sk1]\n\tv_and_b32 %[vt1], %[t2], %[t3]\n\tv_cmp_eq_u32 %[sd2], -1, %[vt1]\n\ts_and_b64 %[sd2], %[sd2], %[sby]\n\tv_subb_co_u32 %[t4], %[sk2], %[t4], 0, %[sd2]\n\ts_nop 0\n\tv_subb_co_u32 %[t5], %[sk2], %[t5], 0, %[sk2]\n\tv_and_b32 %[vt1], %[t4], %[t5]\n\tv_cmp_eq_u32 %[sd3], -1, %[vt1]\n\ts_and_b64 %[sd3], %[sd3], %[sby]\n\tv_subb_co_u32 %[t6], %[sk3], %[t6], 0, %[sd3]\n\ts_nop 0\n\tv_subb_co_u32 %[t7], %[sk3], %[t7], 0, %[sk3]\n\tv_add_u32 %[t7], %[t7], %[vt2]"
                     : [h0] "=&v"(h0), [h1] "=&v"(h1), [h2] "=&v"(h2), [h3] "=&v"(h3), [h4] "=&v"(h4), [h5] "=&v"(h5), [h6] "=&v"(h6), [h7] "=&v"(h7), [t0] "=&v"(t0), [t1] "=&v"(t1), [t2] "=&v"(t2), [t3] "=&v"(t3), [t4] "=&v"(t4), [t5] "=&v"(t5), [t6] "=&v"(t6), [t7] "=&v"(t7), [vt1] "=&v"(vt1), [vt2] "=&v"(vt2), [vt3] "=&v"(vt3), [vt4] "=&v"(vt4), [vt5] "=&v"(vt5), [sf1] "=&s"(sf1), [sf2] "=&s"(sf2), [se3] "=&s"(se3), [stp] "=&s"(stp), [sg0] "=&s"(sg0), [sg1] "=&s"(sg1), [sm] "=&s"(sm), [sd1] "=&s"(sd1), [sd2] "=&s"(sd2), [sd3] "=&s"(sd3), [sk0] "=&s"(sk0), [sk1] "=&s"(sk1), [sk2] "=&s"(sk2), [sk3] "=&s"(sk3), [scy] "=&s"(scy), [sby] "=&s"(sby), [sq1] "=&s"(sq1), [sq2] "=&s"(sq2), [sq3] "=&s"(sq3)
                     : [a0] "v"(a0), [a1] "v"(a1), [a2] "v"(a2), [a3] "v"(a3), [a4] "v"(a4), [a5] "v"(a5), [a6] "v"(a6), [a7] "v"(a7), [b0] "v"(b0), [b1] "v"(b1), [b2] "v"(b2), [b3] "v"(b3), [b4] "v"(b4), [b5] "v"(b5), [b6] "v"(b6), [b7] "v"(b7), [c80] "v"(0x80000000u), [p0l] "s"(0xFFFFFFEDu)
                     : "scc");
        (void)sf1; (void)sf2; (void)se3; (void)stp; (void)sg0; (void)sg1; (void)sm; (void)sd1; (void)sd2; (void)sd3; (void)sk0; (void)sk1; (void)sk2; (void)sk3; (void)scy; (void)sby; (void)sq1; (void)sq2; (void)sq3;
    }
    o0[0] = h0; o0[1] = h1; o0[2] = h2; o0[3] = h3; o0[4] = h4; o0[5] = h5; o0[6] = h6; o0[7] = h7;
    o1[0] = t0; o1[1] = t1; o1[2] = t2; o1[3] = t3; o1[4] = t4; o1[5] = t5; o1[6] = t6; o1[7] = t7;
    (void)scy; (void)sby; (void)srare; (void)vt1; (void)vt2; (void)vt3; (void)vt4; (void)vt5;
}

__device__ __forceinline__ void q4_sum_asm(uint32_t r[16], const uint32_t w[10]) {
    const uint32_t w0 = w[0], w1 = w[1], w2 = w[2], w3 = w[3], w4 = w[4], w5 = w[5], w6 = w[6], w7 = w[7], w8 = w[8], w9 = w[9];
    uint32_t q2, q3, q4, q5, q6, q7, q8, q9, q10, q11, r4, r5, r6, r7, r8, r9, r10, r11, r12, r13, r14, r15, n0, n1, n2, n3, n4, n5, n6, n7, n8, n9, m0, m1, m2, m3, m4, m5, m6, m7, m8, m9, m10, m11;
    uint64_t sa, sb;
    asm volatile("s_nop 1\n\tv_mov_b32_dpp %[m0], %[w0] quad_perm:[2,2,2,2] row_mask:0xf bank_mask:0xf bound_ctrl:1\n\tv_mov_b32_dpp %[m1], %[w1] quad_perm:[2,2,2,2] row_mask:0xf bank_mask:0xf bound_ctrl:1\n\tv_mov_b32_dpp %[n0], %[w0] quad_perm:[1,1,3,3] row_mask:0xf bank_mask:0xf bound_ctrl:1\n\tv_add_co_u32 %[q2], %[sa], %[w2], %[n0]\n\tv_mov_b32_dpp %[n1], %[w1] quad_perm:[1,1,3,3] row_mask:0xf bank_mask:0xf bound_ctrl:1\n\tv_addc_co_u32 %[q3], %[sa], %[w3], %[n1], %[sa]\n\tv_mov_b32_dpp %[m2], %[q2] quad_perm:[2,2,2,2] row_mask:0xf bank_mask:0xf bound_ctrl:1\n\tv_mov_b32_dpp %[n2], %[w2] quad_perm:[1,1,3,3] row_mask:0xf bank_mask:0xf bound_ctrl:1\n\tv_addc_co_u32 %[q4], %[sa], %[w4], %[n2], %[sa]\n\tv_add_co_u32 %[r4], %[sb], %[q4], %[m0]\n\tv_mov_b32_dpp %[m3], %[q3] quad_perm:[2,2,2,2] row_mask:0xf bank_mask:0xf bound_ctrl:1\n\tv_mov_b32_dpp %[m4], %[q4] quad_perm:[2,2,2,2] row_mask:0xf bank_mask:0xf bound_ctrl:1\n\tv_mov_b32_dpp %[n3], %[w3] quad_perm:[1,1,3,3] row_mask:0xf bank_mask:0xf bound_ctrl:1\n\tv_addc_co_u32 %[q5], %[sa], %[w5], %[n3], %[sa]\n\tv_addc_co_u32 %[r5], %[sb], %[q5], %[m1], %[sb]\n\tv_mov_b32_dpp %[n4], %[w4] quad_perm:[1,1,3,3] row_mask:0xf bank_mask:0xf bound_ctrl:1\n\tv_addc_co_u32 %[q6], %[sa], %[w6], %[n4], %[sa]\n\tv_addc_co_u32 %[r6], %[sb], %[q6], %[m2], %[sb]\n\tv_mov_b32_dpp %[m5], %[q5] quad_perm:[2,2,2,2] row_mask:0xf bank_mask:0xf bound_ctrl:1\n\tv_mov_b32_dpp %[m6], %[q6] quad_perm:[2,2,2,2] row_mask:0xf bank_mask:0xf bound_ctrl:1\n\tv_mov_b32_dpp %[n5], %[w5] quad_perm:[1,1,3,3] row_mask:0xf bank_mask:0xf bound_ctrl:1\n\tv_addc_co_u32 %[q7], %[sa], %[w7], %[n5], %[sa]\n\tv_addc_co_u32 %[r7], %[sb], %[q7], %[m3], %[sb]\n\tv_mov_b32_dpp %[n6], %[w6] quad_perm:[1,1,3,3] row_mask:0xf bank_mask:0xf bound_ctrl:1\n\tv_addc_co_u32 %[q8], %[sa], %[w8], %[n6], %[sa]\n\tv_addc_co_u32 %[r8], %[sb], %[q8], %[m4], %[sb]\n\tv_mov_b32_dpp %[m7], %[q7] quad_perm:[2,2,2,2] row_mask:0xf bank_mask:0xf bound_ctrl:1\n\tv_mov_b32_dpp %[m8], %[q8] quad_perm:[2,2,2,2] row_mask:0xf bank_mask:0xf bound_ctrl:1\n\tv_mov_b32_dpp %[n7], %[w7] quad_perm:[1,1,3,3] row_mask:0xf bank_mask:0xf bound_ctrl:1\n\tv_addc_co_u32 %[q9], %[sa], %[w9], %[n7], %[sa]\n\tv_addc_co_u32 %[r9], %[sb], %[q9], %[m5], %[sb]\n\tv_mov_b32_dpp %[n8], %[w8] quad_perm:[1,1,3,3] row_mask:0xf bank_mask:0xf bound_ctrl:1\n\tv_addc_co_u32 %[q10], %[sa], 0, %[n8], %[sa]\n\tv_addc_co_u32 %[r10], %[sb], %[q10], %[m6], %[sb]\n\tv_mov_b32_dpp %[m9], %[q9] quad_perm:[2,2,2,2] row_mask:0xf bank_mask:0xf bound_ctrl:1\n\tv_mov_b32_dpp %[m10], %[q10] quad_perm:[2,2,2,2] row_mask:0xf bank_mask:0xf bound_ctrl:1\n\tv_mov_b32_dpp %[n9], %[w9] quad_perm:[1,1,3,3] row_mask:0xf bank_mask:0xf bound_ctrl:1\n\tv_addc_co_u32 %[q11], %[sa], 0, %[n9], %[sa]\n\tv_addc_co_u32 %[r11], %[sb], %[q11], %[m7], %[sb]\n\ts_nop 0\n\tv_addc_co_u32 %[r12], %[sb], 0, %[m8], %[sb]\n\tv_mov_b32_dpp %[m11], %[q11] quad_perm:[2,2,2,2] row_mask:0xf bank_mask:0xf bound_ctrl:1\n\tv_addc_co_u32 %[r13], %[sb], 0, %[m9], %[sb]\n\ts_nop 0\n\tv_addc_co_u32 %[r14], %[sb], 0, %[m10], %[sb]\n\ts_nop 0\n\tv_addc_co_u32 %[r15], %[sb], 0, %[m11], %[sb]"
                 : [q2] "=&v"(q2), [q3] "=&v"(q3), [q4] "=&v"(q4), [q5] "=&v"(q5), [q6] "=&v"(q6), [q7] "=&v"(q7), [q8] "=&v"(q8), [q9] "=&v"(q9), [q10] "=&v"(q10), [q11] "=&v"(q11), [r4] "=&v"(r4), [r5] "=&v"(r5), [r6] "=&v"(r6), [r7] "=&v"(r7), [r8] "=&v"(r8), [r9] "=&v"(r9), [r10] "=&v"(r10), [r11] "=&v"(r11), [r12] "=&v"(r12), [r13] "=&v"(r13), [r14] "=&v"(r14), [r15] "=&v"(r15), [n0] "=&v"(n0), [n1] "=&v"(n1), [n2] "=&v"(n2), [n3] "=&v"(n3), [n4] "=&v"(n4), [n5] "=&v"(n5), [n6] "=&v"(n6), [n7] "=&v"(n7), [n8] "=&v"(n8), [n9] "=&v"(n9), [m0] "=&v"(m0), [m1] "=&v"(m1), [m2] "=&v"(m2), [m3] "=&v"(m3), [m4] "=&v"(m4), [m5] "=&v"(m5), [m6] "=&v"(m6), [m7] "=&v"(m7), [m8] "=&v"(m8), [m9] "=&v"(m9), [m10] "=&v"(m10), [m11] "=&v"(m11), [sa] "=&s"(sa), [sb] "=&s"(sb)
                 : [w0] "v"(w0), [w1] "v"(w1), [w2] "v"(w2), [w3] "v"(w3), [w4] "v"(w4), [w5] "v"(w5), [w6] "v"(w6), [w7] "v"(w7), [w8] "v"(w8), [w9] "v"(w9));
    r[0] = w0; r[1] = w1; r[2] = q2; r[3] = q3;
    r[4] = r4; r[5] = r5; r[6] = r6; r[7] = r7; r[8] = r8; r[9] = r9; r[10] = r10; r[11] = r11; r[12] = r12; r[13] = r13; r[14] = r14; r[15] = r15;
    (void)sa; (void)sb; 
}

__device__ __forceinline__ void fe_add_asm_lat(uint32_t o0[8], const uint32_t fa[8], const uint32_t ga[8]) {
    const uint32_t a0 = fa[0], a1 = fa[1], a2 = fa[2], a3 = fa[3], a4 = fa[4], a5 = fa[5], a6 = fa[6], a7 = fa[7];
    const uint32_t b0 = ga[0], b1 = ga[1], b2 = ga[2], b3 = ga[3], b4 = ga[4], b5 = ga[5], b6 = ga[6], b7 = ga[7];
    uint32_t h0, h1, h2, h3, h4, h5, h6, h7, vt1, vt2, vt3;
    uint64_t scy, srare;
    asm volatile("v_add_co_u32 %[h0], %[scy], %[a0], %[b0]\n\ts_nop 0\n\tv_addc_co_u32 %[h1], %[scy], %[a1], %[b1], %[scy]\n\ts_nop 0\n\tv_addc_co_u32 %[h2], %[scy], %[a2], %[b2], %[scy]\n\ts_nop 0\n\tv_addc_co_u32 %[h3], %[scy], %[a3], %[b3], %[scy]\n\ts_nop 0\n\tv_addc_co_u32 %[h4], %[scy], %[a4], %[b4], %[scy]\n\tv_max_u32 %[vt3], %[h1], %[h4]\n\tv_cmp_eq_u32 %[srare], -1, %[vt3]\n\tv_addc_co_u32 %[h5], %[scy], %[a5], %[b5], %[scy]\n\ts_nop 0\n\tv_addc_co_u32 %[h6], %[scy], %[a6], %[b6], %[scy]\n\ts_nop 0\n\tv_addc_co_u32 %[h7], %[scy], %[a7], %[b7], %[scy]\n\tv_lshrrev_b32 %[vt1], 31, %[h7]\n\ts_nop 0\n\tv_cndmask_b32 %[vt1], %[vt1], 1, %[scy]"
                 : [h0] "=&v"(h0), [h1] "=&v"(h1), [h2] "=&v"(h2), [h3] "=&v"(h3), [h4] "=&v"(h4), [h5] "=&v"(h5), [h6] "=&v"(h6), [h7] "=&v"(h7), [vt1] "=&v"(vt1), [vt3] "=&v"(vt3), [scy] "=&s"(scy), [srare] "=&s"(srare)
                 : [a0] "v"(a0), [a1] "v"(a1), [a2] "v"(a2), [a3] "v"(a3), [a4] "v"(a4), [a5] "v"(a5), [a6] "v"(a6), [a7] "v"(a7), [b0] "v"(b0), [b1] "v"(b1), [b2] "v"(b2), [b3] "v"(b3), [b4] "v"(b4), [b5] "v"(b5), [b6] "v"(b6), [b7] "v"(b7));
    fe_fix_fast_asm(h0, h1, h4, h7, vt1);
    if (__builtin_expect(srare != 0, 0)) {
        uint64_t sf1, sf2, se3, stp, sg0, sg1, sm, sd1, sd2, sd3, sk0, sk1, sk2, sk3, scy;
        asm volatile("v_add_co_u32 %[h0], %[scy], %[a0], %[b0]\n\ts_nop 0\n\tv_addc_co_u32 %[h1], %[scy], %[a1], %[b1], %[scy]\n\ts_nop 0\n\tv_addc_co_u32 %[h2], %[scy], %[a2], %[b2], %[scy]\n\ts_nop 0\n\tv_addc_co_u32 %[h3], %[scy], %[a3], %[b3], %[scy]\n\ts_nop 0\n\tv_addc_co_u32 %[h4], %[scy], %[a4], %[b4], %[scy]\n\ts_nop 0\n\tv_addc_co_u32 %[h5], %[scy], %[a5], %[b5], %[scy]\n\ts_nop 0\n\tv_addc_co_u32 %[h6], %[scy], %[a6], %[b6], %[scy]\n\ts_nop 0\n\tv_addc_co_u32 %[h7], %[scy], %[a7], %[b7], %[scy]\n\tv_and_b32 %[vt1], %[h2], %[h3]\n\tv_and_b32 %[vt2], %[h4], %[h5]\n\tv_or_b32 %[vt3], %[c80], %[h7]\n\tv_cmp_eq_u32 %[sf1], -1, %[vt1]\n\tv_cmp_eq_u32 %[sf2], -1, %[vt2]\n\tv_and_b32 %[vt3], %[vt3], %[h6]\n\tv_cmp_eq_u32 %[se3], -1, %[vt3]\n\tv_cmp_gt_i32 %[stp], 0, %[h7]\n\tv_cmp_eq_u32 %[sg0], -1, %[h1]\n\tv_cmp_le_u32 %[sg1], %[p0l], %[h0]\n\ts_and_b64 %[sg0], %[sg0], %[sg1]\n\ts_and_b64 %[se3], %[se3], %[sf1]\n\ts_and_b64 %[se3], %[se3], %[sf2]\n\ts_and_b64 %[se3], %[se3], %[sg0]\n\ts_or_b64 %[sm], %[scy], %[stp]\n\ts_or_b64 %[sm], %[sm], %[se3]\n\ts_and_b64 %[sd1], %[sm], %[sg0]\n\ts_orn2_b64 %[sg1], %[sf1], %[sg0]\n\ts_and_b64 %[sd2], %[sm], %[sg1]\n\ts_andn2_b64 %[sg1], %[sg0], %[sf1]\n\ts_or_b64 %[sg1], %[sg1], %[sf2]\n\ts_and_b64 %[sd3], %[sm], %[sg1]\n\tv_cndmask_b32 %[vt1], 0, 19, %[sm]\n\tv_cndmask_b32 %[vt2], 0, %[c80], %[sm]\n\tv_add_co_u32 %[h0], %[sk0], %[h0], %[vt1]\n\tv_addc_co_u32 %[h2], %[sk1], %[h2], 0, %[sd1]\n\tv_addc_co_u32 %[h4], %[sk2], %[h4], 0, %[sd2]\n\tv_addc_co_u32 %[h6], %[sk3], %[h6], 0, %[sd3]\n\tv_addc_co_u32 %[h1], %[sk0], %[h1], 0, %[sk0]\n\tv_addc_co_u32 %[h3], %[sk1], %[h3], 0, %[sk1]\n\tv_addc_co_u32 %[h5], %[sk2], %[h5], 0, %[sk2]\n\tv_addc_co_u32 %[h7], %[sk3], %[h7], %[vt2], %[sk3]"
                     : [h0] "=&v"(h0), [h1] "=&v"(h1), [h2] "=&v"(h2), [h3] "=&v"(h3), [h4] "=&v"(h4), [h5] "=&v"(h5), [h6] "=&v"(h6), [h7] "=&v"(h7), [vt1] "=&v"(vt1), [vt2] "=&v"(vt2), [vt3] "=&v"(vt3), [sf1] "=&s"(sf1), [sf2] "=&s"(sf2), [se3] "=&s"(se3), [stp] "=&s"(stp), [sg0] "=&s"(sg0), [sg1] "=&s"(sg1), [sm] "=&s"(sm), [sd1] "=&s"(sd1), [sd2] "=&s"(sd2), [sd3] "=&s"(sd3), [sk0] "=&s"(sk0), [sk1] "=&s"(sk1), [sk2] "=&s"(sk2), [sk3] "=&s"(sk3), [scy] "=&s"(scy)
                     : [a0] "v"(a0), [a1] "v"(a1), [a2] "v"(a2), [a3] "v"(a3), [a4] "v"(a4), [a5] "v"(a5), [a6] "v"(a6), [a7] "v"(a7), [b0] "v"(b0), [b1] "v"(b1), [b2] "v"(b2), [b3] "v"(b3), [b4] "v"(b4), [b5] "v"(b5), [b6] "v"(b6), [b7] "v"(b7), [c80] "v"(0x80000000u), [p0l] "s"(0xFFFFFFEDu)
                     : "scc");
        (void)sf1; (void)sf2; (void)se3; (void)stp; (void)sg0; (void)sg1; (void)sm; (void)sd1; (void)sd2; (void)sd3; (void)sk0; (void)sk1; (void)sk2; (void)sk3; (void)scy;
    }
    o0[0] = h0; o0[1] = h1; o0[2] = h2; o0[3] = h3; o0[4] = h4; o0[5] = h5; o0[6] = h6; o0[7] = h7;
    (void)scy; (void)srare; (void)vt1; (void)vt2; (void)vt3;
}

__device__ __forceinline__ void fe_fold_asm_lat(uint32_t o0[8], const uint32_t ta[8], const uint32_t xa[8]) {
    const uint32_t a0 = ta[0], a1 = ta[1], a2 = ta[2], a3 = ta[3], a4 = ta[4], a5 = ta[5], a6 = ta[6], a7 = ta[7];
    const uint32_t x0 = xa[0], x1 = xa[1], x2 = xa[2], x3 = xa[3], x4 = xa[4], x5 = xa[5], x6 = xa[6], x7 = xa[7];
    uint32_t h0, h1, h2, h3, h4, h5, h6, h7, vt1, vt2, vt3;
    uint64_t scy, srare;
    asm volatile("v_max3_u32 %[vt3], %[x2], %[x4], %[x6]\n\tv_add_co_u32 %[h0], %[scy], %[a0], %[x0]\n\ts_nop 0\n\tv_addc_co_u32 %[h1], %[scy], %[a1], %[x1], %[scy]\n\ts_nop 0\n\tv_addc_co_u32 %[h2], %[scy], %[a2], %[x2], %[scy]\n\ts_nop 0\n\tv_addc_co_u32 %[h3], %[scy], %[a3], %[x3], %[scy]\n\ts_nop 0\n\tv_addc_co_u32 %[h4], %[scy], %[a4], %[x4], %[scy]\n\tv_max3_u32 %[vt3], %[vt3], %[h1], %[h4]\n\tv_cmp_eq_u32 %[srare], -1, %[vt3]\n\tv_addc_co_u32 %[h5], %[scy], %[a5], %[x5], %[scy]\n\ts_nop 0\n\tv_addc_co_u32 %[h6], %[scy], %[a6], %[x6], %[scy]\n\ts_nop 0\n\tv_addc_co_u32 %[h7], %[scy], %[a7], %[x7], %[scy]\n\tv_lshrrev_b32 %[vt1], 31, %[h7]\n\ts_nop 0\n\tv_cndmask_b32 %[vt1], %[vt1], 1, %[scy]"
                 : [h0] "=&v"(h0), [h1] "=&v"(h1), [h2] "=&v"(h2), [h3] "=&v"(h3), [h4] "=&v"(h4), [h5] "=&v"(h5), [h6] "=&v"(h6), [h7] "=&v"(h7), [vt1] "=&v"(vt1), [vt3] "=&v"(vt3), [scy] "=&s"(scy), [srare] "=&s"(srare)
                 : [a0] "v"(a0), [a1] "v"(a1), [a2] "v"(a2), [a3] "v"(a3), [a4] "v"(a4), [a5] "v"(a5), [a6] "v"(a6), [a7] "v"(a7), [x0] "v"(x0), [x1] "v"(x1), [x2] "v"(x2), [x3] "v"(x3), [x4] "v"(x4), [x5] "v"(x5), [x6] "v"(x6), [x7] "v"(x7));
    fe_fix_fast_asm(h0, h1, h4, h7, vt1);
    if (__builtin_expect(srare != 0, 0)) {
        uint64_t sf1, sf2, se3, stp, sg0, sg1, sm, sd1, sd2, sd3, sk0, sk1, sk2, sk3, scy, sq1, sq2, sq3;
        asm volatile("v_and_b32 %[vt1], %[x2], %[x3]\n\tv_cmp_eq_u32 %[sq1], -1, %[vt1]\n\tv_and_b32 %[vt1], %[x4], %[x5]\n\tv_cmp_eq_u32 %[sq2], -1, %[vt1]\n\tv_and_b32 %[vt1], %[x6], %[x7]\n\tv_cmp_eq_u32 %[sq3], -1, %[vt1]\n\tv_add_co_u32 %[h0], %[sk0], %[a0], %[x0]\n\ts_nop 0\n\tv_addc_co_u32 %[h1], %[scy], %[a1], %[x1], %[sk0]\n\ts_nop 0\n\tv_addc_co_u32 %[h2], %[sk0], %[a2], %[x2], %[scy]\n\ts_nop 0\n\tv_addc_co_u32 %[h3], %[sk1], %[a3], %[x3], %[sk0]\n\ts_and_b64 %[sq1], %[sq1], %[scy]\n\ts_andn2_b64 %[scy], %[sk1], %[sq1]\n\tv_addc_co_u32 %[h4], %[sk0], %[a4], %[x4], %[scy]\n\ts_nop 0\n\tv_addc_co_u32 %[h5], %[sk1], %[a5], %[x5], %[sk0]\n\ts_and_b64 %[sq2], %[sq2], %[scy]\n\ts_andn2_b64 %[scy], %[sk1], %[sq2]\n\tv_addc_co_u32 %[h6], %[sk0], %[a6], %[x6], %[scy]\n\ts_nop 0\n\tv_addc_co_u32 %[h7], %[sk1], %[a7], %[x7], %[sk0]\n\ts_and_b64 %[sq3], %[sq3], %[scy]\n\ts_andn2_b64 %[scy], %[sk1], %[sq3]\n\tv_and_b32 %[vt1], %[h2], %[h3]\n\tv_and_b32 %[vt2], %[h4], %[h5]\n\tv_or_b32 %[vt3], %[c80], %[h7]\n\tv_cmp_eq_u32 %[sf1], -1, %[vt1]\n\tv_cmp_eq_u32 %[sf2], -1, %[vt2]\n\tv_and_b32 %[vt3], %[vt3], %[h6]\n\tv_cmp_eq_u32 %[se3], -1, %[vt3]\n\tv_cmp_gt_i32 %[stp], 0, %[h7]\n\tv_cmp_eq_u32 %[sg0], -1, %[h1]\n\tv_cmp_le_u32 %[sg1], %[p0l], %[h0]\n\ts_and_b64 %[sg0], %[sg0], %[sg1]\n\ts_and_b64 %[se3], %[se3], %[sf1]\n\ts_and_b64 %[se3], %[se3], %[sf2]\n\ts_and_b64 %[se3], %[se3], %[sg0]\n\ts_or_b64 %[sm], %[scy], %[stp]\n\ts_or_b64 %[sm], %[sm], %[se3]\n\ts_and_b64 %[sd1], %[sm], %[sg0]\n\ts_orn2_b64 %[sg1], %[sf1], %[sg0]\n\ts_and_b64 %[sd2], %[sm], %[sg1]\n\ts_andn2_b64 %[sg1], %[sg0], %[sf1]\n\ts_or_b64 %[sg1], %[sg1], %[sf2]\n\ts_and_b64 %[sd3], %[sm], %[sg1]\n\tv_cndmask_b32 %[vt1], 0, 19, %[sm]\n\tv_cndmask_b32 %[vt2], 0, %[c80], %[sm]\n\tv_add_co_u32 %[h0], %[sk0], %[h0], %[vt1]\n\tv_addc_co_u32 %[h2], %[sk1], %[h2], 0, %[sd1]\n\tv_addc_co_u32 %[h4], %[sk2], %[h4], 0, %[sd2]\n\tv_addc_co_u32 %[h6], %[sk3], %[h6], 0, %[sd3]\n\tv_addc_co_u32 %[h1], %[sk0], %[h1], 0, %[sk0]\n\tv_addc_co_u32 %[h3], %[sk1], %[h3], 0, %[sk1]\n\tv_addc_co_u32 %[h5], %[sk2], %[h5], 0, %[sk2]\n\tv_addc_co_u32 %[h7], %[sk3], %[h7], %[vt2], %[sk3]"
                     : [h0] "=&v"(h0), [h1] "=&v"(h1), [h2] "=&v"(h2), [h3] "=&v"(h3), [h4] "=&v"(h4), [h5] "=&v"(h5), [h6] "=&v"(h6), [h7] "=&v"(h7), [vt1] "=&v"(vt1), [vt2] "=&v"(vt2), [vt3] "=&v"(vt3), [sf1] "=&s"(sf1), [sf2] "=&s"(sf2), [se3] "=&s"(se3), [stp] "=&s"(stp), [sg0] "=&s"(sg0), [sg1] "=&s"(sg1), [sm] "=&s"(sm), [sd1] "=&s"(sd1), [sd2] "=&s"(sd2), [sd3] "=&s"(sd3), [sk0] "=&s"(sk0), [sk1] "=&s"(sk1), [sk2] "=&s"(sk2), [sk3] "=&s"(sk3), [scy] "=&s"(scy), [sq1] "=&s"(sq1), [sq2] "=&s"(sq2), [sq3] "=&s"(sq3)
                     : [a0] "v"(a0), [a1] "v"(a1), [a2] "v"(a2), [a3] "v"(a3), [a4] "v"(a4), [a5] "v"(a5), [a6] "v"(a6), [a7] "v"(a7), [x0] "v"(x0), [x1] "v"(x1), [x2] "v"(x2), [x3] "v"(x3), [x4] "v"(x4), [x5] "v"(x5), [x6] "v"(x6), [x7] "v"(x7), [c80] "v"(0x80000000u), [p0l] "s"(0xFFFFFFEDu)
                     : "scc");
        (void)sf1; (void)sf2; (void)se3; (void)stp; (void)sg0; (void)sg1; (void)sm; (void)sd1; (void)sd2; (void)sd3; (void)sk0; (void)sk1; (void)sk2; (void)sk3; (void)scy; (void)sq1; (void)sq2; (void)sq3;
    }
    o0[0] = h0; o0[1] = h1; o0[2] = h2; o0[3] = h3; o0[4] = h4; o0[5] = h5; o0[6] = h6; o0[7] = h7;
    (void)scy; (void)srare; (void)vt1; (void)vt2; (void)vt3;
}

__device__ __forceinline__ void fe_addsub_asm_lat(uint32_t o0[8], uint32_t o1[8], const uint32_t fa[8], const uint32_t ga[8]) {
    const uint32_t a0 = fa[0], a1 = fa[1], a2 = fa[2], a3 = fa[3], a4 = fa[4], a5 = fa[5], a6 = fa[6], a7 = fa[7];
    const uint32_t b0 = ga[0], b1 = ga[1], b2 = ga[2], b3 = ga[3], b4 = ga[4], b5 = ga[5], b6 = ga[6], b7 = ga[7];
    uint32_t h0, h1, h2, h3, h4, h5, h6, h7, t0, t1, t2, t3, t4, t5, t6, t7, vt1, vt2, vt3, vt4, vt5;
    uint64_t scy, sby, srare;
    asm volatile("v_max3_u32 %[vt3], %[b2], %[b4], %[b6]\n\tv_add_co_u32 %[h0], %[scy], %[a0], %[b0]\n\tv_sub_co_u32 %[t0], %[sby], %[a0], %[b0]\n\tv_addc_co_u32 %[h1], %[scy], %[a1], %[b1], %[scy]\n\tv_subb_co_u32 %[t1], %[sby], %[a1], %[b1], %[sby]\n\tv_addc_co_u32 %[h2], %[scy], %[a2], %[b2], %[scy]\n\tv_subb_co_u32 %[t2], %[sby], %[a2], %[b2], %[sby]\n\tv_addc_co_u32 %[h3], %[scy], %[a3], %[b3], %[scy]\n\tv_subb_co_u32 %[t3], %[sby], %[a3], %[b3], %[sby]\n\tv_addc_co_u32 %[h4], %[scy], %[a4], %[b4], %[scy]\n\tv_subb_co_u32 %[t4], %[sby], %[a4], %[b4], %[sby]\n\tv_not_b32 %[vt4], %[t1]\n\tv_max3_u32 %[vt3], %[vt3], %[h1], %[h4]\n\tv_max3_u32 %[vt3], %[vt3], %[vt4], %[t2]\n\tv_max_u32 %[vt3], %[vt3], %[t4]\n\tv_cmp_eq_u32 %[srare], -1, %[vt3]\n\tv_addc_co_u32 %[h5], %[scy], %[a5], %[b5], %[scy]\n\tv_subb_co_u32 %[t5], %[sby], %[a5], %[b5], %[sby]\n\tv_addc_co_u32 %[h6], %[scy], %[a6], %[b6], %[scy]\n\tv_subb_co_u32 %[t6], %[sby], %[a6], %[b6], %[sby]\n\tv_addc_co_u32 %[h7], %[scy], %[a7], %[b7], %[scy]\n\tv_subb_co_u32 %[t7], %[sby], %[a7], %[b7], %[sby]\n\tv_lshrrev_b32 %[vt1], 31, %[h7]\n\tv_cndmask_b32 %[vt1], %[vt1], 1, %[scy]\n\tv_cndmask_b32 %[vt4], 0, -1, %[sby]"
                 : [h0] "=&v"(h0), [h1] "=&v"(h1), [h2] "=&v"(h2), [h3] "=&v"(h3), [h4] "=&v"(h4), [h5] "=&v"(h5), [h6] "=&v"(h6), [h7] "=&v"(h7), [t0] "=&v"(t0), [t1] "=&v"(t1), [t2] "=&v"(t2), [t3] "=&v"(t3), [t4] "=&v"(t4), [t5] "=&v"(t5), [t6] "=&v"(t6), [t7] "=&v"(t7), [vt1] "=&v"(vt1), [vt3] "=&v"(vt3), [vt4] "=&v"(vt4), [scy] "=&s"(scy), [sby] "=&s"(sby), [srare] "=&s"(srare)
                 : [a0] "v"(a0), [a1] "v"(a1), [a2] "v"(a2), [a3] "v"(a3), [a4] "v"(a4), [a5] "v"(a5), [a6] "v"(a6), [a7] "v"(a7), [b0] "v"(b0), [b1] "v"(b1), [b2] "v"(b2), [b3] "v"(b3), [b4] "v"(b4), [b5] "v"(b5), [b6] "v"(b6), [b7] "v"(b7));
    fe_fix_fast_asm(h0, h1, h4, h7, vt1);
    fe_subp_fast_asm(t0, t1, t7, vt4);
    if (__builtin_expect(srare != 0, 0)) {
        uint64_t sf1, sf2, se3, stp, sg0, sg1, sm, sd1, sd2, sd3, sk0, sk1, sk2, sk3, scy, sby, sq1, sq2, sq3;
        asm volatile("v_add_co_u32 %[h0], %[scy], %[a0], %[b0]\n\ts_nop 0\n\tv_addc_co_u32 %[h1], %[scy], %[a1], %[b1], %[scy]\n\ts_nop 0\n\tv_addc_co_u32 %[h2], %[scy], %[a2], %[b2], %[scy]\n\ts_nop 0\n\tv_addc_co_u32 %[h3], %[scy], %[a3], %[b3], %[scy]\n\ts_nop 0\n\tv_addc_co_u32 %[h4], %[scy], %[a4], %[b4], %[scy]\n\ts_nop 0\n\tv_addc_co_u32 %[h5], %[scy], %[a5], %[b5], %[scy]\n\ts_nop 0\n\tv_addc_co_u32 %[h6], %[scy], %[a6], %[b6], %[scy]\n\ts_nop 0\n\tv_addc_co_u32 %[h7], %[scy], %[a7], %[b7], %[scy]\n\tv_and_b32 %[vt1], %[h2], %[h3]\n\tv_and_b32 %[vt2], %[h4], %[h5]\n\tv_or_b32 %[vt3], %[c80], %[h7]\n\tv_cmp_eq_u32 %[sf1], -1, %[vt1]\n\tv_cmp_eq_u32 %[sf2], -1, %[vt2]\n\tv_and_b32 %[vt3], %[vt3], %[h6]\n\tv_cmp_eq_u32 %[se3], -1, %[vt3]\n\tv_cmp_gt_i32 %[stp], 0, %[h7]\n\tv_cmp_eq_u32 %[sg0], -1, %[h1]\n\tv_cmp_le_u32 %[sg1], %[p0l], %[h0]\n\ts_and_b64 %[sg0], %[sg0], %[sg1]\n\ts_and_b64 %[se3], %[se3], %[sf1]\n\ts_and_b64 %[se3], %[se3], %[sf2]\n\ts_and_b64 %[se3], %[se3], %[sg0]\n\ts_or_b64 %[sm], %[scy], %[stp]\n\ts_or_b64 %[sm], %[sm], %[se3]\n\ts_and_b64 %[sd1], %[sm], %[sg0]\n\ts_orn2_b64 %[sg1], %[sf1], %[sg0]\n\ts_and_b64 %[sd2], %[sm], %[sg1]\n\ts_andn2_b64 %[sg1], %[sg0], %[sf1]\n\ts_or_b64 %[sg1], %[sg1], %[sf2]\n\ts_and_b64 %[sd3], %[sm], %[sg1]\n\tv_cndmask_b32 %[vt1], 0, 19, %[sm]\n\tv_cndmask_b32 %[vt2], 0, %[c80], %[sm]\n\tv_add_co_u32 %[h0], %[sk0], %[h0], %[vt1]\n\tv_addc_co_u32 %[h2], %[sk1], %[h2], 0, %[sd1]\n\tv_addc_co_u32 %[h4], %[sk2], %[h4], 0, %[sd2]\n\tv_addc_co_u32 %[h6], %[sk3], %[h6], 0, %[sd3]\n\tv_addc_co_u32 %[h1], %[sk0], %[h1], 0, %[sk0]\n\tv_addc_co_u32 %[h3], %[sk1], %[h3], 0, %[sk1]\n\tv_addc_co_u32 %[h5], %[sk2], %[h5], 0, %[sk2]\n\tv_addc_co_u32 %[h7], %[sk3], %[h7], %[vt2], %[sk3]\n\tv_and_b32 %[vt1], %[b2], %[b3]\n\tv_cmp_eq_u32 %[sq1], -1, %[vt1]\n\tv_and_b32 %[vt1], %[b4], %[b5]\n\tv_cmp_eq_u32 %[sq2], -1, %[vt1]\n\tv_and_b32 %[vt1], %[b6], %[b7]\n\tv_cmp_eq_u32 %[sq3], -1, %[vt1]\n\tv_sub_co_u32 %[t0], %[sk0], %[a0], %[b0]\n\ts_nop 0\n\tv_subb_co_u32 %[t1], %[sby], %[a1], %[b1], %[sk0]\n\ts_nop 0\n\tv_subb_co_u32 %[t2], %[sk0], %[a2], %[b2], %[sby]\n\ts_nop 0\n\tv_subb_co_u32 %[t3], %[sk1], %[a3], %[b3], %[sk0]\n\ts_and_b64 %[sq1], %[sq1], %[sby]\n\ts_andn2_b64 %[sby], %[sk1], %[sq1]\n\tv_subb_co_u32 %[t4], %[sk0], %[a4], %[b4], %[sby]\n\ts_nop 0\n\tv_subb_co_u32 %[t5], %[sk1], %[a5], %[b5], %[sk0]\n\ts_and_b64 %[sq2], %[sq2], %[sby]\n\ts_andn2_b64 %[sby], %[sk1], %[sq2]\n\tv_subb_co_u32 %[t6], %[sk0], %[a6], %[b6], %[sby]\n\ts_nop 0\n\tv_subb_co_u32 %[t7], %[sk1], %[a7], %[b7], %[sk0]\n\ts_and_b64 %[sq3], %[sq3], %[sby]\n\ts_andn2_b64 %[sby], %[sk1], %[sq3]\n\tv_cndmask_b32 %[vt1], 0, 19, %[sby]\n\tv_cndmask_b32 %[vt2], 0, %[c80], %[sby]\n\tv_sub_co_u32 %[t0], %[sk0], %[t0], %[vt1]\n\ts_nop 0\n\tv_subb_co_u32 %[t1], %[sd1], %[t1], 0, %[sk0]\n\ts_nop 0\n\tv_subb_co_u32 %[t2], %[sk1], %[t2], 0, %[sd1]\n\ts_nop 0\n\tv_subb_co_u32 %[t3], %[sk1], %[t3], 0, %[sk1]\n\tv_and_b32 %[vt1], %[t2], %[t3]\n\tv_cmp_eq_u32 %[sd2], -1, %[vt1]\n\ts_and_b64 %[sd2], %[sd2], %[sby]\n\tv_subb_co_u32 %[t4], %[sk2], %[t4], 0, %[sd2]\n\ts_nop 0\n\tv_subb_co_u32 %[t5], %[sk2], %[t5], 0, %[sk2]\n\tv_and_b32 %[vt1], %[t4], %[t5]\n\tv_cmp_eq_u32 %[sd3], -1, %[vt1]\n\ts_and_b64 %[sd3], %[sd3], %[sby]\n\tv_subb_co_u32 %[t6], %[sk3], %[t6], 0, %[sd3]\n\ts_nop 0\n\tv_subb_co_u32 %[t7], %[sk3], %[t7], 0, %[sk3]\n\tv_add_u32 %[t7], %[t7], %[vt2]"
                     : [h0] "=&v"(h0), [h1] "=&v"(h1), [h2] "=&v"(h2), [h3] "=&v"(h3), [h4] "=&v"(h4), [h5] "=&v"(h5), [h6] "=&v"(h6), [h7] "=&v"(h7), [t0] "=&v"(t0), [t1] "=&v"(t1), [t2] "=&v"(t2), [t3] "=&v"(t3), [t4] "=&v"(t4), [t5] "=&v"(t5), [t6] "=&v"(t6), [t7] "=&v"(t7), [vt1] "=&v"(vt1), [vt2] "=&v"(vt2), [vt3] "=&v"(vt3), [vt4] "=&v"(vt4), [vt5] "=&v"(vt5), [sf1] "=&s"(sf1), [sf2] "=&s"(sf2), [se3] "=&s"(se3), [stp] "=&s"(stp), [sg0] "=&s"(sg0), [sg1] "=&s"(sg1), [sm] "=&s"(sm), [sd1] "=&s"(sd1), [sd2] "=&s"(sd2), [sd3] "=&s"(sd3), [sk0] "=&s"(sk0), [sk1] "=&s"(sk1), [sk2] "=&s"(sk2), [sk3] "=&s"(sk3), [scy] "=&s"(scy), [sby] "=&s"(sby), [sq1] "=&s"(sq1), [sq2] "=&s"(sq2), [sq3] "=&s"(sq3)
                     : [a0] "v"(a0), [a1] "v"(a1), [a2] "v"(a2), [a3] "v"(a3), [a4] "v"(a4), [a5] "v"(a5), [a6] "v"(a6), [a7] "v"(a7), [b0] "v"(b0), [b1] "v"(b1), [b2] "v"(b2), [b3] "v"(b3), [b4] "v"(b4), [b5] "v"(b5), [b6] "v"(b6), [b7] "v"(b7), [c80] "v"(0x80000000u), [p0l] "s"(0xFFFFFFEDu)
                     : "scc");
        (void)sf1; (void)sf2; (void)se3; (void)stp; (void)sg0; (void)sg1; (void)sm; (void)sd1; (void)sd2; (void)sd3; (void)sk0; (void)sk1; (void)sk2; (void)sk3; (void)scy; (void)sby; (void)sq1; (void)sq2; (void)sq3;
    }
    o0[0] = h0; o0[1] = h1; o0[2] = h2; o0[3] = h3; o0[4] = h4; o0[5] = h5; o0[6] = h6; o0[7] = h7;
    o1[0] = t0; o1[1] = t1; o1[2] = t2; o1[3] = t3; o1[4] = t4; o1[5] = t5; o1[6] = t6; o1[7] = t7;
    (void)scy; (void)sby; (void)srare; (void)vt1; (void)vt2; (void)vt3; (void)vt4; (void)vt5;
}

__device__ __forceinline__ void fe_add_asm_lat_acc(uint32_t o0[8], const uint32_t fa[8], const uint32_t ga[8], uint32_t& acc) {
    const uint32_t a0 = fa[0], a1 = fa[1], a2 = fa[2], a3 = fa[3], a4 = fa[4], a5 = fa[5], a6 = fa[6], a7 = fa[7];
    const uint32_t b0 = ga[0], b1 = ga[1], b2 = ga[2], b3 = ga[3], b4 = ga[4], b5 = ga[5], b6 = ga[6], b7 = ga[7];
    uint32_t h0, h1, h2, h3, h4, h5, h6, h7, vt1, vt3;
    uint64_t scy;
    asm volatile("v_add_co_u32 %[h0], %[scy], %[a0], %[b0]\n\ts_nop 0\n\tv_addc_co_u32 %[h1], %[scy], %[a1], %[b1], %[scy]\n\ts_nop 0\n\tv_addc_co_u32 %[h2], %[scy], %[a2], %[b2], %[scy]\n\ts_nop 0\n\tv_addc_co_u32 %[h3], %[scy], %[a3], %[b3], %[scy]\n\ts_nop 0\n\tv_addc_co_u32 %[h4], %[scy], %[a4], %[b4], %[scy]\n\tv_max_u32 %[vt3], %[h1], %[h4]\n\tv_max_u32 %[acc], %[acc], %[vt3]\n\tv_addc_co_u32 %[h5], %[scy], %[a5], %[b5], %[scy]\n\ts_nop 0\n\tv_addc_co_u32 %[h6], %[scy], %[a6], %[b6], %[scy]\n\ts_nop 0\n\tv_addc_co_u32 %[h7], %[scy], %[a7], %[b7], %[scy]\n\tv_lshrrev_b32 %[vt1], 31, %[h7]\n\ts_nop 0\n\tv_cndmask_b32 %[vt1], %[vt1], 1, %[scy]"
                 : [h0] "=&v"(h0), [h1] "=&v"(h1), [h2] "=&v"(h2), [h3] "=&v"(h3), [h4] "=&v"(h4), [h5] "=&v"(h5), [h6] "=&v"(h6), [h7] "=&v"(h7), [vt1] "=&v"(vt1), [vt3] "=&v"(vt3), [acc] "+v"(acc), [scy] "=&s"(scy)
                 : [a0] "v"(a0), [a1] "v"(a1), [a2] "v"(a2), [a3] "v"(a3), [a4] "v"(a4), [a5] "v"(a5), [a6] "v"(a6), [a7] "v"(a7), [b0] "v"(b0), [b1] "v"(b1), [b2] "v"(b2), [b3] "v"(b3), [b4] "v"(b4), [b5] "v"(b5), [b6] "v"(b6), [b7] "v"(b7));
    fe_fix_fast_asm(h0, h1, h4, h7, vt1);
    o0[0] = h0; o0[1] = h1; o0[2] = h2; o0[3] = h3; o0[4] = h4; o0[5] = h5; o0[6] = h6; o0[7] = h7;
    (void)scy; (void)vt1; (void)vt3;
}

__device__ __forceinline__ void fe_fold_asm_lat_acc(uint32_t o0[8], const uint32_t ta[8], const uint32_t xa[8], uint32_t& acc) {
    const uint32_t a0 = ta[0], a1 = ta[1], a2 = ta[2], a3 = ta[3], a4 = ta[4], a5 = ta[5], a6 = ta[6], a7 = ta[7];
    const uint32_t x0 = xa[0], x1 = xa[1], x2 = xa[2], x3 = xa[3], x4 = xa[4], x5 = xa[5], x6 = xa[6], x7 = xa[7];
    uint32_t h0, h1, h2, h3, h4, h5, h6, h7, vt1, vt3;
    uint64_t scy;
    asm volatile("v_max3_u32 %[vt3], %[x2], %[x4], %[x6]\n\tv_add_co_u32 %[h0], %[scy], %[a0], %[x0]\n\ts_nop 0\n\tv_addc_co_u32 %[h1], %[scy], %[a1], %[x1], %[scy]\n\ts_nop 0\n\tv_addc_co_u32 %[h2], %[scy], %[a2], %[x2], %[scy]\n\ts_nop 0\n\tv_addc_co_u32 %[h3], %[scy], %[a3], %[x3], %[scy]\n\ts_nop 0\n\tv_addc_co_u32 %[h4], %[scy], %[a4], %[x4], %[scy]\n\tv_max3_u32 %[vt3], %[vt3], %[h1], %[h4]\n\tv_max_u32 %[acc], %[acc], %[vt3]\n\tv_addc_co_u32 %[h5], %[scy], %[a5], %[x5], %[scy]\n\ts_nop 0\n\tv_addc_co_u32 %[h6], %[scy], %[a6], %[x6], %[scy]\n\ts_nop 0\n\tv_addc_co_u32 %[h7], %[scy], %[a7], %[x7], %[scy]\n\tv_lshrrev_b32 %[vt1], 31, %[h7]\n\ts_nop 0\n\tv_cndmask_b32 %[vt1], %[vt1], 1, %[scy]"
                 : [h0] "=&v"(h0), [h1] "=&v"(h1), [h2] "=&v"(h2), [h3] "=&v"(h3), [h4] "=&v"(h4), [h5] "=&v"(h5), [h6] "=&v"(h6), [h7] "=&v"(h7), [vt1] "=&v"(vt1), [vt3] "=&v"(vt3), [acc] "+v"(acc), [scy] "=&s"(scy)
                 : [a0] "v"(a0), [a1] "v"(a1), [a2] "v"(a2), [a3] "v"(a3), [a4] "v"(a4), [a5] "v"(a5), [a6] "v"(a6), [a7] "v"(a7), [x0] "v"(x0), [x1] "v"(x1), [x2] "v"(x2), [x3] "v"(x3), [x4] "v"(x4), [x5] "v"(x5), [x6] "v"(x6), [x7] "v"(x7));
    fe_fix_fast_asm(h0, h1, h4, h7, vt1);
    o0[0] = h0; o0[1] = h1; o0[2] = h2; o0[3] = h3; o0[4] = h4; o0[5] = h5; o0[6] = h6; o0[7] = h7;
    (void)scy; (void)vt1; (void)vt3;
}

__device__ __forceinline__ void fe_addsub_asm_lat_acc(uint32_t o0[8], uint32_t o1[8], const uint32_t fa[8], const uint32_t ga[8], uint32_t& acc) {
    const uint32_t a0 = fa[0], a1 = fa[1], a2 = fa[2], a3 = fa[3], a4 = fa[4], a5 = fa[5], a6 = fa[6], a7 = fa[7];
    const uint32_t b0 = ga[0], b1 = ga[1], b2 = ga[2], b3 = ga[3], b4 = ga[4], b5 = ga[5], b6 = ga[6], b7 = ga[7];
    uint32_t h0, h1, h2, h3, h4, h5, h6, h7, t0, t1, t2, t3, t4, t5, t6, t7, vt1, vt3, vt4;
    uint64_t scy, sby;
    asm volatile("v_max3_u32 %[vt3], %[b2], %[b4], %[b6]\n\tv_add_co_u32 %[h0], %[scy], %[a0], %[b0]\n\tv_sub_co_u32 %[t0], %[sby], %[a0], %[b0]\n\tv_addc_co_u32 %[h1], %[scy], %[a1], %[b1], %[scy]\n\tv_subb_co_u32 %[t1], %[sby], %[a1], %[b1], %[sby]\n\tv_addc_co_u32 %[h2], %[scy], %[a2], %[b2], %[scy]\n\tv_subb_co_u32 %[t2], %[sby], %[a2], %[b2], %[sby]\n\tv_addc_co_u32 %[h3], %[scy], %[a3], %[b3], %[scy]\n\tv_subb_co_u32 %[t3], %[sby], %[a3], %[b3], %[sby]\n\tv_addc_co_u32 %[h4], %[scy], %[a4], %[b4], %[scy]\n\tv_subb_co_u32 %[t4], %[sby], %[a4], %[b4], %[sby]\n\tv_not_b32 %[vt4], %[t1]\n\tv_max3_u32 %[vt3], %[vt3], %[h1], %[h4]\n\tv_max3_u32 %[vt3], %[vt3], %[vt4], %[t2]\n\tv_max_u32 %[vt3], %[vt3], %[t4]\n\tv_max_u32 %[acc], %[acc], %[vt3]\n\tv_addc_co_u32 %[h5], %[scy], %[a5], %[b5], %[scy]\n\tv_subb_co_u32 %[t5], %[sby], %[a5], %[b5], %[sby]\n\tv_addc_co_u32 %[h6], %[scy], %[a6], %[b6], %[scy]\n\tv_subb_co_u32 %[t6], %[sby], %[a6], %[b6], %[sby]\n\tv_addc_co_u32 %[h7], %[scy], %[a7], %[b7], %[scy]\n\tv_subb_co_u32 %[t7], %[sby], %[a7], %[b7], %[sby]\n\tv_lshrrev_b32 %[vt1], 31, %[h7]\n\tv_cndmask_b32 %[vt1], %[vt1], 1, %[scy]\n\tv_cndmask_b32 %[vt4], 0, -1, %[sby]"
                 : [h0] "=&v"(h0), [h1] "=&v"(h1), [h2] "=&v"(h2), [h3] "=&v"(h3), [h4] "=&v"(h4), [h5] "=&v"(h5), [h6] "=&v"(h6), [h7] "=&v"(h7), [t0] "=&v"(t0), [t1] "=&v"(t1), [t2] "=&v"(t2), [t3] "=&v"(t3), [t4] "=&v"(t4), [t5] "=&v"(t5), [t6] "=&v"(t6), [t7] "=&v"(t7), [vt1] "=&v"(vt1), [vt3] "=&v"(vt3), [vt4] "=&v"(vt4), [acc] "+v"(acc), [scy] "=&s"(scy), [sby] "=&s"(sby)
                 : [a0] "v"(a0), [a1] "v"(a1), [a2] "v"(a2), [a3] "v"(a3), [a4] "v"(a4), [a5] "v"(a5), [a6] "v"(a6), [a7] "v"(a7), [b0] "v"(b0), [b1] "v"(b1), [b2] "v"(b2), [b3] "v"(b3), [b4] "v"(b4), [b5] "v"(b5), [b6] "v"(b6), [b7] "v"(b7));
    fe_fix_fast_asm(h0, h1, h4, h7, vt1);
    fe_subp_fast_asm(t0, t1, t7, vt4);
    o0[0] = h0; o0[1] = h1; o0[2] = h2; o0[3] = h3; o0[4] = h4; o0[5] = h5; o0[6] = h6; o0[7] = h7;
    o1[0] = t0; o1[1] = t1; o1[2] = t2; o1[3] = t3; o1[4] = t4; o1[5] = t5; o1[6] = t6; o1[7] = t7;
    (void)scy; (void)sby; (void)vt1; (void)vt3; (void)vt4;
}
}
```

### cudabulletproof_amd/csrc/ge25519_dev.h

```cpp
#pragma once
#include "fe25519_dev.h"

namespace bp {

#ifndef BP_LANE_ADDSUB
#define BP_LANE_ADDSUB 1
#endif
BP_DEV void lane_addsub(const fe& f, const fe& g, fe& sum, fe& diff) {
#if BP_LANE_ADDSUB
    fe_addsub(f, g, sum, diff);
#else
    diff = fe_sub(f, g);
    sum = fe_add(f, g);
#endif
}

struct ge {
    fe X, Y, Z, T;
};

struct geq {
    fe YmX, YpX, Z, T;
};

BP_DEV fe k_const() {
    return fe{{0x75EB4DCA135978A3ull, 0x00700A4D4141D8ABull, 0x8CC740797779E898ull, 0x52036CEE2B6FFE73ull}};
}

BP_DEV fe fe_mul_k(const fe& f) {
#if BP_MUL_ASM && defined(__HIP_DEVICE_COMPILE__)
    uint32_t a[8], w[16];
#pragma unroll
    for (int i = 0; i < 4; i++) {
        a[2 * i] = (uint32_t)f.v[i];
        a[2 * i + 1] = (uint32_t)(f.v[i] >> 32);
    }
    mul512_k_asm(w, a);
    uint64_t t[8];
#pragma unroll
    for (int i = 0; i < 8; i++) t[i] = (uint64_t)w[2 * i] | ((uint64_t)w[2 * i + 1] << 32);
    return fe_fold512(t);
#else
    return fe_mul(f, k_const());
#endif
}

BP_DEV ge ge_zero() { return ge{fe_set(0), fe_set(1), fe_set(1), fe_set(0)}; }

BP_DEV geq ge_prep(const ge& q) {
    return geq{fe_sub(q.Y, q.X), fe_add(q.Y, q.X), q.Z, q.T};
}

BP_DEV ge ge_add_q(const ge& p, const geq& q) {
    fe A = fe_mul(fe_sub(p.Y, p.X), q.YmX);
    fe B = fe_mul(fe_add(p.Y, p.X), q.YpX);
    fe C = fe_mul_k(fe_mul(p.T, q.T));
    fe D = fe_mul(p.Z, q.Z);
    D = fe_add(D, D);
    fe E, F, G, H;
    lane_addsub(B, A, H, E);
    lane_addsub(D, C, G, F);
    return ge{fe_mul(E, F), fe_mul(G, H), fe_mul(F, G), fe_mul(E, H)};
}

BP_DEV ge ge_add(const ge& p, const ge& q) { return ge_add_q(p, ge_prep(q)); }

BP_DEV ge ge_dbl(const ge& p) {
    fe A = fe_sq(fe_sub(p.Y, p.X));
    fe B = fe_sq(fe_add(p.Y, p.X));
    fe C = fe_mul_k(fe_sq(p.T));
    fe D = fe_sq(p.Z);
    D = fe_add(D, D);
    fe E, F, G, H;
    lane_addsub(B, A, H, E);
    lane_addsub(D, C, G, F);
    return ge{fe_mul(E, F), fe_mul(G, H), fe_mul(F, G), fe_mul(E, H)};
}

BP_DEV ge ge_norm_dev(const ge& p) {
    ge r;
    r.X = fe_mul_one(p.X);
    r.Y = fe_mul_one(p.Y);
    r.Z = fe_set(1);
    r.T = fe_mul(r.X, r.Y);
    return r;
}

BP_DEV ge ge_norm_host(const ge& p) {
    if (fe_is_one(fe_canon(p.Z))) return p;
    fe zi = fe_invert(p.Z);
    ge r;
    r.X = fe_mul(p.X, zi);
    r.Y = fe_mul(p.Y, zi);
    r.Z = fe_set(1);
    r.T = fe_mul(r.X, r.Y);
    return r;
}

BP_DEV int fe_clz256(const fe& s) {
    if (s.v[3]) return __clzll(s.v[3]);
    if (s.v[2]) return 64 + __clzll(s.v[2]);
    if (s.v[1]) return 128 + __clzll(s.v[1]);
    if (s.v[0]) return 192 + __clzll(s.v[0]);
    return 256;
}

BP_DEV ge ld_ge(const ge* p) { return *p; }

constexpr int PREFIX_MAX_BITS = 24;
BP_DEV uint32_t prefix_index(const fe& s, int K) { return (uint32_t)(s.v[3] >> (64 - K)); }

BP_DEV int sm_ops(const fe& s) {
    return (256 - fe_clz256(s)) + __popcll(s.v[0]) + __popcll(s.v[1]) + __popcll(s.v[2]) + __popcll(s.v[3]);
}
BP_DEV int sm_ops_prefix(const fe& s, int K) {
    if (K <= 0 || fe_clz256(s) >= K) return sm_ops(s);
    const uint64_t top = K == 64 ? 0 : (s.v[3] & (~0ull >> K));
    return (256 - K) + __popcll(s.v[0]) + __popcll(s.v[1]) + __popcll(s.v[2]) + __popcll(top);
}

template <bool QLDS>
BP_DEV fe qget(const fe* p) {
    if (QLDS) asm volatile("" ::: "memory");
    return *p;
}

template <bool QLDS>
BP_DEV ge ge_add_qp(const ge& p, const geq* q, bool zone = false) {
    fe A = fe_mul(fe_sub(p.Y, p.X), qget<QLDS>(&q->YmX));
    fe B = fe_mul(fe_add(p.Y, p.X), qget<QLDS>(&q->YpX));
    fe C = fe_mul_k(fe_mul(p.T, qget<QLDS>(&q->T)));
    fe D = zone ? fe_mul_one(p.Z) : fe_mul(p.Z, qget<QLDS>(&q->Z));
    D = fe_add(D, D);
    fe E, F, G, H;
    lane_addsub(B, A, H, E);
    lane_addsub(D, C, G, F);
    return ge{fe_mul(E, F), fe_mul(G, H), fe_mul(F, G), fe_mul(E, H)};
}

template <bool QLDS, bool ZONE = false>
BP_DEV ge ge_add_sel(const ge& p, const geq* q, bool use_q) {
    fe ymx = fe_sub(p.Y, p.X);
    fe qa = qget<QLDS>(&q->YmX);
    fe A = fe_mul(ymx, use_q ? qa : ymx);
    fe ypx = fe_add(p.Y, p.X);
    fe qb = qget<QLDS>(&q->YpX);
    fe B = fe_mul(ypx, use_q ? qb : ypx);
    fe qt = qget<QLDS>(&q->T);
    fe C = fe_mul_k(fe_mul(p.T, use_q ? qt : p.T));
    fe D;
    if (ZONE) {
        fe d1 = fe_mul_one(p.Z), d2 = fe_sq(p.Z);
        D = use_q ? d1 : d2;
    } else {
        fe qz = qget<QLDS>(&q->Z);
        D = fe_mul(p.Z, use_q ? qz : p.Z);
    }
    D = fe_add(D, D);
    fe E, F, G, H;
    lane_addsub(B, A, H, E);
    lane_addsub(D, C, G, F);
    return ge{fe_mul(E, F), fe_mul(G, H), fe_mul(F, G), fe_mul(E, H)};
}

struct BitStream {
    uint64_t cur, n1, n2, n3;
    int left;
};

BP_DEV BitStream bs_init(const fe& s, int i) {
    BitStream b{s.v[3], s.v[2], s.v[1], s.v[0], 0};
    int L = i >> 6;
#pragma unroll
    for (int k = 0; k < 3; k++) {
        bool sh = k < 3 - L;
        b.cur = sh ? b.n1 : b.cur;
        b.n1 = sh ? b.n2 : b.n1;
        b.n2 = sh ? b.n3 : b.n2;
        b.n3 = sh ? 0 : b.n3;
    }
    int bi = i & 63;
    b.cur <<= (63 - bi);
    b.left = bi + 1;
    return b;
}

BP_DEV uint32_t bs_next(BitStream& b) {
    uint32_t bit = (uint32_t)(b.cur >> 63);
    b.cur <<= 1;
    if (--b.left == 0) {
        b.cur = b.n1;
        b.n1 = b.n2;
        b.n2 = b.n3;
        b.n3 = 0;
        b.left = 64;
    }
    return bit;
}

template <bool QLDS>
BP_DEV ge sm_uniform(const fe& s_in, const geq* q, const ge* __restrict__ dtab, const ge* ptab, int K) {
    fe s;
#pragma unroll
    for (int i = 0; i < 4; i++) {
        uint32_t lo = __builtin_amdgcn_readfirstlane((uint32_t)s_in.v[i]);
        uint32_t hi = __builtin_amdgcn_readfirstlane((uint32_t)(s_in.v[i] >> 32));
        s.v[i] = (uint64_t)lo | ((uint64_t)hi << 32);
    }
    int lz = fe_clz256(s);
    const bool pre = K > 0 && lz < K && __all(ptab != nullptr);
    const int top = pre ? 255 - K : 255 - lz;
    ge r = ld_ge(pre ? &ptab[prefix_index(s, K)] : &dtab[lz]);
    if (top < 0) return r;
    const bool zone = __all(fe_is_one(qget<QLDS>(&q->Z)));
    BitStream bs = bs_init(s, top);
    for (int i = top; i >= 0; i--) {
        r = ge_dbl(r);
        if (bs_next(bs)) r = ge_add_qp<QLDS>(r, q, zone);
    }
    return r;
}

template <bool QLDS, bool ZONE>
BP_DEV ge sm_lane_loop(const fe& s, const geq* q, const ge* __restrict__ dtab, const ge* ptab, int K) {
    int lz = fe_clz256(s);
    const bool pre = K > 0 && lz < K && ptab != nullptr;
    ge r = ld_ge(pre ? &ptab[prefix_index(s, K)] : &dtab[lz]);
    int i = pre ? 255 - K : 255 - lz;
    BitStream bs = bs_init(s, i < 0 ? 0 : i);
    uint32_t bit = i >= 0 ? bs_next(bs) : 0;
    bool add_phase = false;
    while (i >= 0) {
        r = ge_add_sel<QLDS, ZONE>(r, q, add_phase);
        if (!add_phase && bit) {
            add_phase = true;
        } else {
            add_phase = false;
            i--;
            bit = bs_next(bs);
        }
    }
    return r;
}

template <bool QLDS>
BP_DEV ge sm_lane(const fe& s, const geq* q, const ge* __restrict__ dtab, const ge* ptab, int K) {
    if (__all(fe_is_one(qget<QLDS>(&q->Z)))) return sm_lane_loop<QLDS, true>(s, q, dtab, ptab, K);
    return sm_lane_loop<QLDS, false>(s, q, dtab, ptab, K);
}

template <bool QLDS>
BP_DEV ge scalarmult(const fe& s, const ge& P, geq* slot, const ge* __restrict__ dtab, const ge* ptab = nullptr,
                     int K = 0) {
    geq qreg;
    const geq* q;
    if (QLDS) {
        fe ymx = fe_sub(P.Y, P.X), ypx = fe_add(P.Y, P.X);
#pragma unroll
        for (int k = 0; k < 4; k++) {
            slot->YmX.v[k] = ymx.v[k];
            slot->YpX.v[k] = ypx.v[k];
            slot->Z.v[k] = P.Z.v[k];
            slot->T.v[k] = P.T.v[k];
        }
        q = slot;
    } else {
        qreg = ge_prep(P);
        q = &qreg;
    }
    uint32_t same = 1;
#pragma unroll
    for (int i = 0; i < 4; i++) {
        uint32_t lo = (uint32_t)s.v[i], hi = (uint32_t)(s.v[i] >> 32);
        same &= (lo == __builtin_amdgcn_readfirstlane(lo)) & (hi == __builtin_amdgcn_readfirstlane(hi));
    }
    if (__all(same)) return sm_uniform<QLDS>(s, q, dtab, ptab, K);
    return sm_lane<QLDS>(s, q, dtab, ptab, K);
}

}
```

### include/cudabulletproof_hip.h

```cpp
#ifndef CUDABULLETPROOF_HIP_H
#define CUDABULLETPROOF_HIP_H

#include <stddef.h>
#include <stdint.h>
#ifndef __cplusplus
#include <stdbool.h>
#endif

#ifndef CURVE25519_OPS_H
typedef struct { uint64_t limbs[4]; } fe25519;
typedef struct { fe25519 X, Y, Z, T; } ge25519;
#endif
#ifndef BULLETPROOF_VECTORS_H
typedef struct { fe25519* elements; size_t length; } FieldVector;
typedef struct { ge25519* elements; size_t length; } PointVector;
typedef struct {
    size_t n;
    FieldVector a;
    FieldVector b;
    fe25519 c;
    PointVector L;
    PointVector R;
    size_t L_len;
    fe25519 x;
// ... 18 lines not shown

void cuda_field_vector_inner_product(fe25519* result, const FieldVector* a, const FieldVector* b);
void cuda_field_vector_inner_product_shared(fe25519* result, const FieldVector* a, const FieldVector* b);
void cuda_batch_field_vector_inner_product(fe25519* results, const FieldVector* a_vectors,
                                           const FieldVector* b_vectors, size_t num_vectors);

void cuda_batch_field_add(fe25519* results, const fe25519* a, const fe25519* b, size_t count);
void cuda_batch_field_sub(fe25519* results, const fe25519* a, const fe25519* b, size_t count);
void cuda_batch_field_mul(fe25519* results, const fe25519* a, const fe25519* b, size_t count);
void cuda_batch_field_mul_karatsuba(fe25519* results, const fe25519* a, const fe25519* b, size_t count);
void cuda_batch_field_square(fe25519* results, const fe25519* inputs, size_t count);
void cuda_batch_field_invert(fe25519* results, const fe25519* inputs, size_t count);
void cuda_soa_field_add(fe25519* results, const fe25519* a, const fe25519* b, size_t count);

bool cuda_range_proof_verify(const RangeProof* proof, const ge25519* V, size_t n, const PointVector* G,
                             const PointVector* H, const ge25519* g, const ge25519* h);
bool cuda_inner_product_verify(const InnerProductProof* proof, const ge25519* P, const PointVector* G,
                               const PointVector* H, const ge25519* Q);

void cuda_benchmark_multi_scalar_mul(int iterations, size_t vector_size);
void cuda_benchmark_inner_product(int iterations, size_t vector_size);
void cuda_benchmark_field_operations(int iterations, size_t batch_size);
void cuda_benchmark_range_proof(int iterations, size_t bit_size);


typedef struct {
    size_t count, n, ab_len, L_len;
    const ge25519 *V, *A, *S, *T1, *T2;
    const fe25519 *t, *a, *b, *c, *x;
    const ge25519 *L, *R;
    const fe25519 *taux, *mu;
    const ge25519* Vp;
} hipbp_proof_batch;

typedef enum {
    HIPBP_OK = 0,
    HIPBP_ERR_ARG = 1,
    HIPBP_ERR_DEVICE = 2,
} hipbp_status;

const char* hipbp_last_error(void);
int hipbp_device_count(void);

int hipbp_batch_range_proof_verify_host(const RangeProof* proofs, const ge25519* V, size_t count, size_t n,
                                        const PointVector* G, const PointVector* H, const ge25519* g,
                                        const ge25519* h, int num_gpus, uint8_t* ok);

int hipbp_batch_range_proof_verify(const hipbp_proof_batch* batch, const ge25519* G, const ge25519* H,
                                   const ge25519* g, const ge25519* h, uint8_t* ok, ge25519* P_out,
                                   ge25519* check_out, void* stream);
int hipbp_batch_range_proof_verify_std(const hipbp_proof_batch* batch, const ge25519* G, const ge25519* H,
                                       const ge25519* g, const ge25519* h, uint8_t* ok, ge25519* P_out,
                                       ge25519* check_out, uint8_t* flags_out, ge25519* poly_out, void* stream);
int hipbp_batch_inner_product_verify(const hipbp_proof_batch* batch, const ge25519* P, const ge25519* G,
                                     const ge25519* H, const ge25519* Q, uint8_t* ok, ge25519* check_out,
                                     void* stream);
void* hipbp_pipeline_create(size_t max_batch, size_t n, int range_mode, const ge25519* G, const ge25519* H,
                            const ge25519* g, const ge25519* h, void* stream);
int hipbp_pipeline_push(void* pipeline, const hipbp_proof_batch* batch ,
                        const ge25519* P_in, uint8_t* ok, ge25519* P_out, ge25519* check_out,
                        uint8_t* flags_out , ge25519* poly_out );
int hipbp_pipeline_flush(void* pipeline);
int hipbp_pipeline_depth(void* pipeline);
int hipbp_pipeline_prefix_tables(void* pipeline, int bits);
void* hipbp_gens_create(size_t n, const ge25519* G, const ge25519* H, const ge25519* g, const ge25519* h,
                        int prefix_bits, void* stream);
void hipbp_gens_destroy(void* gens);
int hipbp_pipeline_use_gens(void* pipeline, void* gens);
int hipbp_batch_range_proof_verify_gens(const hipbp_proof_batch* batch, void* gens, uint8_t* ok, ge25519* P_out,
                                        ge25519* check_out, void* stream);
int hipbp_pipeline_defer_msm(void* pipeline, int on);
void hipbp_pipeline_destroy(void* pipeline);

typedef struct {
    size_t count, n;
    const fe25519* v;
    const fe25519* gamma;
    const fe25519* sL;
    const fe25519* sR;
    const fe25519* rnd;
} hipbp_prove_input;
typedef struct {
    ge25519 *V, *A, *S, *T1, *T2;
    fe25519 *taux, *mu, *t, *c, *x;
    fe25519 *a, *b;
    ge25519 *L, *R;
    uint8_t* valid;
} hipbp_proof_out;
int hipbp_batch_generate_range_proof(const hipbp_prove_input* in, const ge25519* G, const ge25519* H,
                                     const ge25519* g, const ge25519* h, hipbp_proof_out* out, void* stream);
int hipbp_batch_generate_range_proof_gens(const hipbp_prove_input* in, void* gens, hipbp_proof_out* out,
                                          void* stream);

int hipbp_derive_prover_scalars(const uint8_t* seed32, const fe25519* v, const fe25519* gamma, uint64_t index_base,
                                size_t count, size_t n, fe25519* sL, fe25519* sR, fe25519* rnd, void* stream);
int hipbp_batch_generate_range_proof_seeded(const hipbp_prove_input* in, const uint8_t* seed32, uint64_t index_base,
                                            const ge25519* G, const ge25519* H, const ge25519* g, const ge25519* h,
                                            hipbp_proof_out* out, void* stream);
int hipbp_batch_generate_range_proof_seeded_gens(const hipbp_prove_input* in, const uint8_t* seed32,
                                                 uint64_t index_base, void* gens, hipbp_proof_out* out, void* stream);
int hipbp_batch_generate_range_proof_accepted(const hipbp_prove_input* in, const uint8_t* seed32, uint64_t index_base,
                                              int max_attempts, int check, const ge25519* G, const ge25519* H,
                                              const ge25519* g, const ge25519* h, hipbp_proof_out* out,
                                              uint8_t* attempts, void* stream);
int hipbp_batch_generate_range_proof_accepted_gens(const hipbp_prove_input* in, const uint8_t* seed32,
                                                   uint64_t index_base, int max_attempts, int check, void* gens,
                                                   hipbp_proof_out* out, uint8_t* attempts, void* stream);
int hipbp_derive_prover_scalars_at(const uint8_t* seed32, const fe25519* v, const fe25519* gamma, uint64_t index_base,
                                   const uint8_t* attempt, size_t count, size_t n, fe25519* sL, fe25519* sR,
                                   fe25519* rnd, void* stream);
int hipbp_accepted_last_stats(int* rounds, uint32_t* proved, float* kernel_ms);
int hipbp_batch_generate_range_proof_host(RangeProof* proofs, uint8_t* valid, const fe25519* v, const fe25519* gamma,
                                          size_t count, size_t n, const PointVector* G, const PointVector* H,
                                          const ge25519* g, const ge25519* h, const uint8_t seed32[32],
                                          uint64_t index_base);

typedef struct {
    size_t count, n;
    const fe25519 *a, *b;
    const fe25519 *c;
    const fe25519 *transcript;
} hipbp_ipa_prove_input;
typedef struct {
    fe25519 *a, *b, *c, *x;
    fe25519 *c_final;
    ge25519 *L, *R;
} hipbp_ipa_proof_out;
int hipbp_batch_inner_product_prove(const hipbp_ipa_prove_input* in, const ge25519* G, const ge25519* H,
                                    const ge25519* Q, hipbp_ipa_proof_out* out, void* stream);
int hipbp_batch_inner_product_prove_gens(const hipbp_ipa_prove_input* in, void* gens, hipbp_ipa_proof_out* out,
                                         void* stream);
int hipbp_inner_product_prove_host(InnerProductProof* proof, const FieldVector* a, const FieldVector* b,
                                   const PointVector* G, const PointVector* H, const ge25519* Q,
                                   const fe25519* c_in, const uint8_t* transcript32 );

int hipbp_msm(ge25519* result, const fe25519* scalars, const ge25519* points, size_t n, void* stream);

int hipbp_msm_batch(ge25519* results, const fe25519* scalars, const ge25519* points, size_t n, size_t count,
                    void* stream);

int hipbp_msm_batch_gens(ge25519* results, const fe25519* scalars, const void* gens, size_t count, void* stream);

int hipbp_msm_pippenger(ge25519* result, const fe25519* scalars, const ge25519* points, size_t n,
                        int window_bits, void* stream);
int hipbp_msm_pippenger_batch(ge25519* results, const fe25519* scalars, const ge25519* points, size_t n,
                              size_t count, int window_bits, void* stream);
int hipbp_msm_pippenger_windows(ge25519* window_sums, const fe25519* scalars, const ge25519* points, size_t n,
                                int window_bits, int w_begin, int w_end, void* stream);
int hipbp_msm_pippenger_horner(ge25519* results, const ge25519* window_sums, size_t count, int window_bits,
                               void* stream);
int hipbp_point_tree(ge25519* result, const ge25519* points, size_t n, void* stream);
int hipbp_field_op(int op, fe25519* r, const fe25519* a, const fe25519* b, size_t count, void* stream);
int hipbp_sha_probe(int kind, fe25519* out, const fe25519* in, size_t count, void* stream);
int hipbp_release_stream_workspaces(void* stream);
int hipbp_sync(void* stream);

int hipbp_timing_enable(int on);
int hipbp_timing_collect(double* total_ms, uint64_t* launches);
int hipbp_kernel_count(void);
const char* hipbp_kernel_name(int kind);

#ifdef __cplusplus
}
#endif
#endif
```

Baseline: 216,200.

## Defer field-op carry and multiply-bound checks across scalar-mult ladder chunks

Adds field add/sub/fold/mul/square variants that fold their rare-case overflow and bounded-multiply conditions into per-lane accumulators instead of checking and branching after every operation. Scalar multiplication (uniform and per-lane ladders) now runs on these deferred variants and does one wave ballot every fixed chunk of iterations. If any lane's accumulator flags a possible bad case, the whole multiplication is redone with the exact path. This removes per-operation wave votes and branches from the hot ladder, at the cost of extra register pressure and an occasional full recompute. A probe entry point and test ops are also added.

Result: faster. 218,800, median of 6 (+1.2%).

```diff
diff --git a/cudabulletproof_amd/__init__.py b/cudabulletproof_amd/__init__.py
--- a/cudabulletproof_amd/__init__.py
+++ b/cudabulletproof_amd/__init__.py
@@ -104,7 +104,7 @@
     "hipbp_batch_range_proof_verify_std", "hipbp_batch_range_proof_verify_gens", "hipbp_batch_inner_product_verify", "hipbp_batch_generate_range_proof", "hipbp_msm",
     "hipbp_msm_pippenger", "hipbp_msm_pippenger_batch", "hipbp_msm_pippenger_windows",
     "hipbp_msm_pippenger_horner", "hipbp_msm_batch", "hipbp_msm_batch_gens", "hipbp_point_tree", "hipbp_field_op",
-    "hipbp_sha_probe", "hipbp_sync", "hipbp_timing_enable",
+    "hipbp_sha_probe", "hipbp_sm_probe", "hipbp_sync", "hipbp_timing_enable",
     "hipbp_timing_collect", "hipbp_kernel_count", "hipbp_kernel_name", "hipbp_pipeline_create",
     "hipbp_pipeline_push", "hipbp_pipeline_flush", "hipbp_pipeline_depth", "hipbp_pipeline_destroy",
     "hipbp_pipeline_defer_msm",
@@ -135,7 +135,7 @@
                   "hipbp_batch_inner_product_verify", "hipbp_batch_generate_range_proof", "hipbp_msm",
                   "hipbp_msm_pippenger", "hipbp_msm_pippenger_batch", "hipbp_msm_pippenger_windows",
                   "hipbp_msm_pippenger_horner", "hipbp_msm_batch", "hipbp_msm_batch_gens", "hipbp_point_tree",
-                  "hipbp_field_op", "hipbp_sha_probe", "hipbp_sync", "hipbp_device_count",
+                  "hipbp_field_op", "hipbp_sha_probe", "hipbp_sm_probe", "hipbp_sync", "hipbp_device_count",
                   "hipbp_release_stream_workspaces", "hipbp_batch_inner_product_prove",
                   "hipbp_batch_inner_product_prove_gens", "hipbp_inner_product_prove_host",
                   "hipbp_derive_prover_scalars", "hipbp_batch_generate_range_proof_seeded",
@@ -705,9 +705,16 @@
            "mul_k": 11,
            "mul_q4_k": 12,
            "add_lat": 13, "add_defer": 14, "addsub_lat_add": 15, "addsub_lat_sub": 16,
-           "addsub_defer_add": 17, "addsub_defer_sub": 18, "fold_lat": 19, "fold_defer": 20}
+           "addsub_defer_add": 17, "addsub_defer_sub": 18, "fold_lat": 19, "fold_defer": 20,
+           "add_acc": 21, "addsub_acc_add": 22, "addsub_acc_sub": 23, "fold_acc": 24, "mul_acc": 25, "sq_acc": 26,
+           "sub_acc": 27}
     _chk(lib().hipbp_field_op(ops[op], _c(r.data_ptr()), _c(a.data_ptr()), _c(b.data_ptr()) if b is not None else None,
                               _sz(a.shape[0]), _stream_ptr(stream)))
+
+
+def sm_probe(force, out, scalars, points, stream=None):
+    _chk(lib().hipbp_sm_probe(int(bool(force)), _c(out.data_ptr()), _c(scalars.data_ptr()), _c(points.data_ptr()),
+                              _sz(scalars.shape[0]), _stream_ptr(stream)))
 
 
 def sha_probe(kind, out, inp, stream=None):
diff --git a/cudabulletproof_amd/csrc/bp_capi.hip b/cudabulletproof_amd/csrc/bp_capi.hip
--- a/cudabulletproof_amd/csrc/bp_capi.hip
+++ b/cudabulletproof_amd/csrc/bp_capi.hip
@@ -1495,14 +1495,24 @@
 
 int hipbp_field_op(int op, fe25519* r, const fe25519* a, const fe25519* b, size_t count, void* stream) {
     BP_ENGINE_OR_RET(e);
-    if (op < 0 || op > 20) { g_err = "bad op"; return HIPBP_ERR_ARG; }
-    if (!a || (!b && op != 3 && op != 5 && op != 7 && op != 11 && op != 12)) { g_err = "null operand"; return HIPBP_ERR_ARG; }
+    if (op < 0 || op > 27) { g_err = "bad op"; return HIPBP_ERR_ARG; }
+    if (!a || (!b && op != 3 && op != 5 && op != 7 && op != 11 && op != 12 && op != 26)) { g_err = "null operand"; return HIPBP_ERR_ARG; }
     if (count == 0) return HIPBP_OK;
     hipStream_t s = pick(stream);
     if (op == 5)
         bp::launch_invert((bp::fe*)r, (const bp::fe*)a, count, s);
     else
         bp::launch_field_op(op, (bp::fe*)r, (const bp::fe*)a, (const bp::fe*)b, count, s);
+    BP_RET_ON(hipGetLastError());
+    return HIPBP_OK;
+}
+
+int hipbp_sm_probe(int force, ge25519* out, const fe25519* scalars, const ge25519* points, size_t count, void* stream) {
+    BP_ENGINE_OR_RET(e);
+    if (!out || !scalars || !points) { g_err = "null operand"; return HIPBP_ERR_ARG; }
+    if (count == 0) return HIPBP_OK;
+    bp::launch_sm_probe(force != 0, (bp::ge*)out, (const bp::fe*)scalars, (const bp::ge*)points, count, e->dtab,
+                        pick(stream));
     BP_RET_ON(hipGetLastError());
     return HIPBP_OK;
 }
diff --git a/cudabulletproof_amd/csrc/bp_kernels.h b/cudabulletproof_amd/csrc/bp_kernels.h
--- a/cudabulletproof_amd/csrc/bp_kernels.h
+++ b/cudabulletproof_amd/csrc/bp_kernels.h
@@ -279,6 +279,7 @@
 
 void launch_field_op(int op, fe* r, const fe* a, const fe* b, size_t count, hipStream_t s);
 void launch_sha_probe(int kind, fe* out, const fe* in, size_t count, hipStream_t s);
+void launch_sm_probe(int force, ge* out, const fe* s, const ge* P, size_t count, const ge* dtab, hipStream_t st);
 void launch_ip_shared(fe* out, const fe* a, const fe* b, size_t n, hipStream_t s);
 void launch_ip_grid(fe* out, fe* part, const fe* a, const fe* b, size_t n, hipStream_t s);
 void launch_ip_batch(fe* out, const fe* a, const fe* b, size_t n, size_t nvec, hipStream_t s);
diff --git a/cudabulletproof_amd/csrc/bp_kernels.hip b/cudabulletproof_amd/csrc/bp_kernels.hip
--- a/cudabulletproof_amd/csrc/bp_kernels.hip
+++ b/cudabulletproof_amd/csrc/bp_kernels.hip
@@ -299,7 +299,7 @@
     }
     if (i >= count) return;
     fe x = a[i], y;
-    if (op != 3 && op != 7 && op != 11) y = b[i];
+    if (op != 3 && op != 7 && op != 11 && op != 26) y = b[i];
     fe z;
     switch (op) {
         case 0: z = fe_add(x, y); break;
@@ -353,6 +353,46 @@
                 z = fe_fold512<2>(t, &acc);
                 if (acc == 0xFFFFFFFFu) z = fe_fold512<1>(t);
             }
+            break;
+        }
+        case 21: {
+            uint32_t acc = 0;
+            z = fe_add<3>(x, y, &acc);
+            if (acc == 0xFFFFFFFFu) z = fe_add(x, y);
+            break;
+        }
+        case 22:
+        case 23: {
+            fe sm, df;
+            uint32_t acc = 0;
+            fe_addsub<3>(x, y, sm, df, &acc);
+            if (acc == 0xFFFFFFFFu) fe_addsub(x, y, sm, df);
+            z = op == 22 ? sm : df;
+            break;
+        }
+        case 24: {
+            uint64_t t[8] = {x.v[0], x.v[1], x.v[2], x.v[3], y.v[0], y.v[1], y.v[2], y.v[3]};
+            uint32_t acc = 0;
+            z = fe_fold512<3>(t, &acc);
+            if (acc == 0xFFFFFFFFu) z = fe_fold512(t);
+            break;
+        }
+        case 25: {
+            Defer d;
+            z = fe_mul<3>(x, y, &d.acc, &d.gacc);
+            if (d.acc == 0xFFFFFFFFu || d.gacc > MUL_BOUNDED_WORD) z = fe_mul(x, y);
+            break;
+        }
+        case 26: {
+            Defer d;
+            z = fe_sq<3>(x, &d.acc, &d.gacc);
+            if (d.acc == 0xFFFFFFFFu || d.gacc > MUL_BOUNDED_WORD) z = fe_sq(x);
+            break;
+        }
+        case 27: {
+            uint32_t acc = 0;
+            z = fe_sub<3>(x, y, &acc);
+            if (acc == 0xFFFFFFFFu) z = fe_sub(x, y);
             break;
         }
         default:
@@ -380,6 +420,20 @@
     out[i] = r;
 }
 
+__global__ __launch_bounds__(TPB) void k_sm_probe(int force, ge* out, const fe* __restrict__ s, const ge* __restrict__ P,
+                                                  size_t count, const ge* __restrict__ dtab) {
+    __shared__ geq qs[TPB];
+    const size_t i = gid();
+    if (i >= count) return;
+    out[i] = force ? scalarmult<true, true>(s[i], P[i], &qs[threadIdx.x], dtab)
+                   : scalarmult<true, false>(s[i], P[i], &qs[threadIdx.x], dtab);
+}
+
+void launch_sm_probe(int force, ge* out, const fe* s, const ge* P, size_t count, const ge* dtab, hipStream_t st) {
+    if (count == 0) return;
+    k_sm_probe<<<nblk(count), TPB, 0, st>>>(force, out, s, P, count, dtab);
+}
+
 void launch_sha_probe(int kind, fe* out, const fe* in, size_t count, hipStream_t s) {
     if (count == 0) return;
     k_sha_probe<<<nblk(count), TPB, 0, s>>>(kind, out, in, count);
diff --git a/cudabulletproof_amd/csrc/fe25519_dev.h b/cudabulletproof_amd/csrc/fe25519_dev.h
--- a/cudabulletproof_amd/csrc/fe25519_dev.h
+++ b/cudabulletproof_amd/csrc/fe25519_dev.h
@@ -111,7 +111,7 @@
         a[2 * i] = lo32(f.v[i]); a[2 * i + 1] = hi32(f.v[i]);
         b[2 * i] = lo32(g.v[i]); b[2 * i + 1] = hi32(g.v[i]);
     }
-    if constexpr (LAT == 2) fe_add_asm_lat_acc(o, a, b, *acc); else if constexpr (LAT == 1) fe_add_asm_lat(o, a, b); else fe_add_asm(o, a, b);
+    if constexpr (LAT == 3) fe_add_asm_acc(o, a, b, *acc); else if constexpr (LAT == 2) fe_add_asm_lat_acc(o, a, b, *acc); else if constexpr (LAT == 1) fe_add_asm_lat(o, a, b); else fe_add_asm(o, a, b);
     return fe{{cat64(o[0], o[1]), cat64(o[2], o[3]), cat64(o[4], o[5]), cat64(o[6], o[7])}};
 #else
     fe h;
@@ -126,7 +126,8 @@
 #endif
 }
 
-BP_DEV fe fe_sub(const fe& f, const fe& g) {
+template <int LAT = 0>
+BP_DEV fe fe_sub(const fe& f, const fe& g, uint32_t* acc = nullptr) {
 #if BP_FIELD_ASM && defined(__HIP_DEVICE_COMPILE__)
     uint32_t a[8], b[8], o[8];
 #pragma unroll
@@ -134,7 +135,7 @@
         a[2 * i] = lo32(f.v[i]); a[2 * i + 1] = hi32(f.v[i]);
         b[2 * i] = lo32(g.v[i]); b[2 * i + 1] = hi32(g.v[i]);
     }
-    fe_sub_asm(o, a, b);
+    if constexpr (LAT == 3) fe_sub_asm_acc(o, a, b, *acc); else fe_sub_asm(o, a, b);
     return fe{{cat64(o[0], o[1]), cat64(o[2], o[3]), cat64(o[4], o[5]), cat64(o[6], o[7])}};
 #else
     fe t;
@@ -169,7 +170,8 @@
         a[2 * i] = lo32(f.v[i]); a[2 * i + 1] = hi32(f.v[i]);
         b[2 * i] = lo32(g.v[i]); b[2 * i + 1] = hi32(g.v[i]);
     }
-    if constexpr (LAT == 2) fe_addsub_asm_lat_acc(os, od, a, b, *acc);
+    if constexpr (LAT == 3) fe_addsub_asm_acc(os, od, a, b, *acc);
+    else if constexpr (LAT == 2) fe_addsub_asm_lat_acc(os, od, a, b, *acc);
     else if constexpr (LAT == 1) fe_addsub_asm_lat(os, od, a, b);
     else fe_addsub_asm(os, od, a, b);
     sum = fe{{cat64(os[0], os[1]), cat64(os[2], os[3]), cat64(os[4], os[5]), cat64(os[6], os[7])}};
@@ -190,7 +192,7 @@
         a[2 * i] = lo32(t[i]); a[2 * i + 1] = hi32(t[i]);
         xh[2 * i] = lo32(x); xh[2 * i + 1] = hi32(x);
     }
-    if constexpr (LAT == 2) fe_fold_asm_lat_acc(o, a, xh, *acc); else if constexpr (LAT == 1) fe_fold_asm_lat(o, a, xh); else fe_fold_asm(o, a, xh);
+    if constexpr (LAT == 3) fe_fold_asm_acc(o, a, xh, *acc); else if constexpr (LAT == 2) fe_fold_asm_lat_acc(o, a, xh, *acc); else if constexpr (LAT == 1) fe_fold_asm_lat(o, a, xh); else fe_fold_asm(o, a, xh);
     return fe{{cat64(o[0], o[1]), cat64(o[2], o[3]), cat64(o[4], o[5]), cat64(o[6], o[7])}};
 #else
     fe h;
@@ -208,7 +210,17 @@
 #endif
 }
 
-BP_DEV void mul512(uint64_t t[8], const fe& f, const fe& g) {
+BP_DEV void mul_gate_defer(uint32_t& gacc, uint32_t x, uint32_t y) {
+#ifdef __HIP_DEVICE_COMPILE__
+    asm("v_max3_u32 %0, %0, %1, %2" : "+v"(gacc) : "v"(x), "v"(y));
+#else
+    gacc = x > gacc ? x : gacc;
+    gacc = y > gacc ? y : gacc;
+#endif
+}
+
+template <bool DEFER = false>
+BP_DEV void mul512(uint64_t t[8], const fe& f, const fe& g, uint32_t* gacc = nullptr) {
     uint32_t a[8], b[8], w[16];
 #pragma unroll
     for (int i = 0; i < 4; i++) {
@@ -219,7 +231,8 @@
     }
 #if BP_MUL_ASM && defined(__HIP_DEVICE_COMPILE__)
     mul512_bounded_asm(w, a, b);
-    if (__builtin_expect(__any(max(a[0], b[7]) > MUL_BOUNDED_WORD), 0)) mul512_asm(w, a, b);
+    if constexpr (DEFER) mul_gate_defer(*gacc, a[0], b[7]);
+    else if (__builtin_expect(__any(max(a[0], b[7]) > MUL_BOUNDED_WORD), 0)) mul512_asm(w, a, b);
 #else
     uint64_t acc = 0;
     uint32_t c2 = 0;
@@ -243,13 +256,18 @@
     for (int i = 0; i < 8; i++) t[i] = (uint64_t)w[2 * i] | ((uint64_t)w[2 * i + 1] << 32);
 }
 
-BP_DEV fe fe_mul(const fe& f, const fe& g) {
+#ifndef BP_DEFER_GATES
+#define BP_DEFER_GATES 1
+#endif
+template <int LAT = 0>
+BP_DEV fe fe_mul(const fe& f, const fe& g, uint32_t* acc = nullptr, uint32_t* gacc = nullptr) {
     uint64_t t[8];
-    mul512(t, f, g);
-    return fe_fold512(t);
-}
-
-BP_DEV void sqr512(uint64_t t[8], const fe& f) {
+    mul512<LAT == 3 && BP_DEFER_GATES>(t, f, g, gacc);
+    return fe_fold512<LAT>(t, acc);
+}
+
+template <bool DEFER = false>
+BP_DEV void sqr512(uint64_t t[8], const fe& f, uint32_t* gacc = nullptr) {
     uint32_t a[8], o[16], w[16];
 #pragma unroll
     for (int i = 0; i < 4; i++) {
@@ -258,7 +276,8 @@
     }
 #if BP_MUL_ASM && defined(__HIP_DEVICE_COMPILE__)
     sqr512_offdiag_bounded_asm(o, a);
-    if (__builtin_expect(__any(max(a[0], a[7]) > MUL_BOUNDED_WORD), 0)) sqr512_offdiag_asm(o, a);
+    if constexpr (DEFER) mul_gate_defer(*gacc, a[0], a[7]);
+    else if (__builtin_expect(__any(max(a[0], a[7]) > MUL_BOUNDED_WORD), 0)) sqr512_offdiag_asm(o, a);
 #else
     uint64_t acc = 0;
     uint32_t c2 = 0;
@@ -296,10 +315,11 @@
     for (int i = 0; i < 8; i++) t[i] = (uint64_t)w[2 * i] | ((uint64_t)w[2 * i + 1] << 32);
 }
 
-BP_DEV fe fe_sq(const fe& f) {
+template <int LAT = 0>
+BP_DEV fe fe_sq(const fe& f, uint32_t* acc = nullptr, uint32_t* gacc = nullptr) {
     uint64_t t[8];
-    sqr512(t, f);
-    return fe_fold512(t);
+    sqr512<LAT == 3 && BP_DEFER_GATES>(t, f, gacc);
+    return fe_fold512<LAT>(t, acc);
 }
 
 BP_DEV fe fe_mul_one(const fe& f) { return fe_canon(f); }
diff --git a/cudabulletproof_amd/csrc/field_asm.h b/cudabulletproof_amd/csrc/field_asm.h
--- a/cudabulletproof_amd/csrc/field_asm.h
+++ b/cudabulletproof_amd/csrc/field_asm.h
@@ -240,4 +240,58 @@
     o1[0] = t0; o1[1] = t1; o1[2] = t2; o1[3] = t3; o1[4] = t4; o1[5] = t5; o1[6] = t6; o1[7] = t7;
     (void)scy; (void)sby; (void)vt1; (void)vt3; (void)vt4;
 }
-}
+
+__device__ __forceinline__ void fe_add_asm_acc(uint32_t o0[8], const uint32_t fa[8], const uint32_t ga[8], uint32_t& acc) {
+    const uint32_t a0 = fa[0], a1 = fa[1], a2 = fa[2], a3 = fa[3], a4 = fa[4], a5 = fa[5], a6 = fa[6], a7 = fa[7];
+    const uint32_t b0 = ga[0], b1 = ga[1], b2 = ga[2], b3 = ga[3], b4 = ga[4], b5 = ga[5], b6 = ga[6], b7 = ga[7];
+    uint32_t h0, h1, h2, h3, h4, h5, h6, h7, vt1, vt3;
+    uint64_t scy;
+    asm volatile("v_add_co_u32 %[h0], %[scy], %[a0], %[b0]\n\ts_nop 0\n\tv_addc_co_u32 %[h1], %[scy], %[a1], %[b1], %[scy]\n\ts_nop 0\n\tv_addc_co_u32 %[h2], %[scy], %[a2], %[b2], %[scy]\n\ts_nop 0\n\tv_addc_co_u32 %[h3], %[scy], %[a3], %[b3], %[scy]\n\ts_nop 0\n\tv_addc_co_u32 %[h4], %[scy], %[a4], %[b4], %[scy]\n\tv_max_u32 %[vt3], %[h1], %[h4]\n\tv_max_u32 %[acc], %[acc], %[vt3]\n\tv_addc_co_u32 %[h5], %[scy], %[a5], %[b5], %[scy]\n\ts_nop 0\n\tv_addc_co_u32 %[h6], %[scy], %[a6], %[b6], %[scy]\n\ts_nop 0\n\tv_addc_co_u32 %[h7], %[scy], %[a7], %[b7], %[scy]\n\tv_lshrrev_b32 %[vt1], 31, %[h7]\n\ts_nop 0\n\tv_cndmask_b32 %[vt1], %[vt1], 1, %[scy]"
+                 : [h0] "=&v"(h0), [h1] "=&v"(h1), [h2] "=&v"(h2), [h3] "=&v"(h3), [h4] "=&v"(h4), [h5] "=&v"(h5), [h6] "=&v"(h6), [h7] "=&v"(h7), [vt1] "=&v"(vt1), [vt3] "=&v"(vt3), [acc] "+v"(acc), [scy] "=&s"(scy)
+                 : [a0] "v"(a0), [a1] "v"(a1), [a2] "v"(a2), [a3] "v"(a3), [a4] "v"(a4), [a5] "v"(a5), [a6] "v"(a6), [a7] "v"(a7), [b0] "v"(b0), [b1] "v"(b1), [b2] "v"(b2), [b3] "v"(b3), [b4] "v"(b4), [b5] "v"(b5), [b6] "v"(b6), [b7] "v"(b7));
+    fe_fix_fast_asm(h0, h1, h4, h7, vt1);
+    o0[0] = h0; o0[1] = h1; o0[2] = h2; o0[3] = h3; o0[4] = h4; o0[5] = h5; o0[6] = h6; o0[7] = h7;
+    (void)scy; (void)vt1; (void)vt3;
+}
+
+__device__ __forceinline__ void fe_sub_asm_acc(uint32_t o0[8], const uint32_t fa[8], const uint32_t ga[8], uint32_t& acc) {
+    const uint32_t a0 = fa[0], a1 = fa[1], a2 = fa[2], a3 = fa[3], a4 = fa[4], a5 = fa[5], a6 = fa[6], a7 = fa[7];
+    const uint32_t b0 = ga[0], b1 = ga[1], b2 = ga[2], b3 = ga[3], b4 = ga[4], b5 = ga[5], b6 = ga[6], b7 = ga[7];
+    uint32_t h0, h1, h2, h3, h4, h5, h6, h7, vt1, vt3;
+    uint64_t scy;
+    asm volatile("v_max3_u32 %[vt3], %[b2], %[b4], %[b6]\n\tv_sub_co_u32 %[h0], %[scy], %[a0], %[b0]\n\ts_nop 0\n\tv_subb_co_u32 %[h1], %[scy], %[a1], %[b1], %[scy]\n\ts_nop 0\n\tv_subb_co_u32 %[h2], %[scy], %[a2], %[b2], %[scy]\n\ts_nop 0\n\tv_subb_co_u32 %[h3], %[scy], %[a3], %[b3], %[scy]\n\ts_nop 0\n\tv_subb_co_u32 %[h4], %[scy], %[a4], %[b4], %[scy]\n\tv_not_b32 %[vt1], %[h1]\n\tv_max3_u32 %[vt3], %[vt3], %[vt1], %[h2]\n\tv_max_u32 %[vt3], %[vt3], %[h4]\n\tv_max_u32 %[acc], %[acc], %[vt3]\n\tv_subb_co_u32 %[h5], %[scy], %[a5], %[b5], %[scy]\n\ts_nop 0\n\tv_subb_co_u32 %[h6], %[scy], %[a6], %[b6], %[scy]\n\ts_nop 0\n\tv_subb_co_u32 %[h7], %[scy], %[a7], %[b7], %[scy]\n\ts_nop 1\n\tv_cndmask_b32 %[vt1], 0, -1, %[scy]"
+                 : [h0] "=&v"(h0), [h1] "=&v"(h1), [h2] "=&v"(h2), [h3] "=&v"(h3), [h4] "=&v"(h4), [h5] "=&v"(h5), [h6] "=&v"(h6), [h7] "=&v"(h7), [vt1] "=&v"(vt1), [vt3] "=&v"(vt3), [acc] "+v"(acc), [scy] "=&s"(scy)
+                 : [a0] "v"(a0), [a1] "v"(a1), [a2] "v"(a2), [a3] "v"(a3), [a4] "v"(a4), [a5] "v"(a5), [a6] "v"(a6), [a7] "v"(a7), [b0] "v"(b0), [b1] "v"(b1), [b2] "v"(b2), [b3] "v"(b3), [b4] "v"(b4), [b5] "v"(b5), [b6] "v"(b6), [b7] "v"(b7));
+    fe_subp_fast_asm(h0, h1, h7, vt1);
+    o0[0] = h0; o0[1] = h1; o0[2] = h2; o0[3] = h3; o0[4] = h4; o0[5] = h5; o0[6] = h6; o0[7] = h7;
+    (void)scy; (void)vt1; (void)vt3;
+}
+
+__device__ __forceinline__ void fe_fold_asm_acc(uint32_t o0[8], const uint32_t ta[8], const uint32_t xa[8], uint32_t& acc) {
+    const uint32_t a0 = ta[0], a1 = ta[1], a2 = ta[2], a3 = ta[3], a4 = ta[4], a5 = ta[5], a6 = ta[6], a7 = ta[7];
+    const uint32_t x0 = xa[0], x1 = xa[1], x2 = xa[2], x3 = xa[3], x4 = xa[4], x5 = xa[5], x6 = xa[6], x7 = xa[7];
+    uint32_t h0, h1, h2, h3, h4, h5, h6, h7, vt1, vt3;
+    uint64_t scy;
+    asm volatile("v_max3_u32 %[vt3], %[x2], %[x4], %[x6]\n\tv_add_co_u32 %[h0], %[scy], %[a0], %[x0]\n\ts_nop 0\n\tv_addc_co_u32 %[h1], %[scy], %[a1], %[x1], %[scy]\n\ts_nop 0\n\tv_addc_co_u32 %[h2], %[scy], %[a2], %[x2], %[scy]\n\ts_nop 0\n\tv_addc_co_u32 %[h3], %[scy], %[a3], %[x3], %[scy]\n\ts_nop 0\n\tv_addc_co_u32 %[h4], %[scy], %[a4], %[x4], %[scy]\n\tv_max3_u32 %[vt3], %[vt3], %[h1], %[h4]\n\tv_max_u32 %[acc], %[acc], %[vt3]\n\tv_addc_co_u32 %[h5], %[scy], %[a5], %[x5], %[scy]\n\ts_nop 0\n\tv_addc_co_u32 %[h6], %[scy], %[a6], %[x6], %[scy]\n\ts_nop 0\n\tv_addc_co_u32 %[h7], %[scy], %[a7], %[x7], %[scy]\n\tv_lshrrev_b32 %[vt1], 31, %[h7]\n\ts_nop 0\n\tv_cndmask_b32 %[vt1], %[vt1], 1, %[scy]"
+                 : [h0] "=&v"(h0), [h1] "=&v"(h1), [h2] "=&v"(h2), [h3] "=&v"(h3), [h4] "=&v"(h4), [h5] "=&v"(h5), [h6] "=&v"(h6), [h7] "=&v"(h7), [vt1] "=&v"(vt1), [vt3] "=&v"(vt3), [acc] "+v"(acc), [scy] "=&s"(scy)
+                 : [a0] "v"(a0), [a1] "v"(a1), [a2] "v"(a2), [a3] "v"(a3), [a4] "v"(a4), [a5] "v"(a5), [a6] "v"(a6), [a7] "v"(a7), [x0] "v"(x0), [x1] "v"(x1), [x2] "v"(x2), [x3] "v"(x3), [x4] "v"(x4), [x5] "v"(x5), [x6] "v"(x6), [x7] "v"(x7));
+    fe_fix_fast_asm(h0, h1, h4, h7, vt1);
+    o0[0] = h0; o0[1] = h1; o0[2] = h2; o0[3] = h3; o0[4] = h4; o0[5] = h5; o0[6] = h6; o0[7] = h7;
+    (void)scy; (void)vt1; (void)vt3;
+}
+
+__device__ __forceinline__ void fe_addsub_asm_acc(uint32_t o0[8], uint32_t o1[8], const uint32_t fa[8], const uint32_t ga[8], uint32_t& acc) {
+    const uint32_t a0 = fa[0], a1 = fa[1], a2 = fa[2], a3 = fa[3], a4 = fa[4], a5 = fa[5], a6 = fa[6], a7 = fa[7];
+    const uint32_t b0 = ga[0], b1 = ga[1], b2 = ga[2], b3 = ga[3], b4 = ga[4], b5 = ga[5], b6 = ga[6], b7 = ga[7];
+    uint32_t h0, h1, h2, h3, h4, h5, h6, h7, t0, t1, t2, t3, t4, t5, t6, t7, vt1, vt3, vt4;
+    uint64_t scy, sby;
+    asm volatile("v_max3_u32 %[vt3], %[b2], %[b4], %[b6]\n\tv_add_co_u32 %[h0], %[scy], %[a0], %[b0]\n\tv_sub_co_u32 %[t0], %[sby], %[a0], %[b0]\n\tv_addc_co_u32 %[h1], %[scy], %[a1], %[b1], %[scy]\n\tv_subb_co_u32 %[t1], %[sby], %[a1], %[b1], %[sby]\n\tv_addc_co_u32 %[h2], %[scy], %[a2], %[b2], %[scy]\n\tv_subb_co_u32 %[t2], %[sby], %[a2], %[b2], %[sby]\n\tv_addc_co_u32 %[h3], %[scy], %[a3], %[b3], %[scy]\n\tv_subb_co_u32 %[t3], %[sby], %[a3], %[b3], %[sby]\n\tv_addc_co_u32 %[h4], %[scy], %[a4], %[b4], %[scy]\n\tv_subb_co_u32 %[t4], %[sby], %[a4], %[b4], %[sby]\n\tv_not_b32 %[vt4], %[t1]\n\tv_max3_u32 %[vt3], %[vt3], %[h1], %[h4]\n\tv_max3_u32 %[vt3], %[vt3], %[vt4], %[t2]\n\tv_max_u32 %[vt3], %[vt3], %[t4]\n\tv_max_u32 %[acc], %[acc], %[vt3]\n\tv_addc_co_u32 %[h5], %[scy], %[a5], %[b5], %[scy]\n\tv_subb_co_u32 %[t5], %[sby], %[a5], %[b5], %[sby]\n\tv_addc_co_u32 %[h6], %[scy], %[a6], %[b6], %[scy]\n\tv_subb_co_u32 %[t6], %[sby], %[a6], %[b6], %[sby]\n\tv_addc_co_u32 %[h7], %[scy], %[a7], %[b7], %[scy]\n\tv_subb_co_u32 %[t7], %[sby], %[a7], %[b7], %[sby]\n\tv_lshrrev_b32 %[vt1], 31, %[h7]\n\tv_cndmask_b32 %[vt1], %[vt1], 1, %[scy]\n\tv_cndmask_b32 %[vt4], 0, -1, %[sby]"
+                 : [h0] "=&v"(h0), [h1] "=&v"(h1), [h2] "=&v"(h2), [h3] "=&v"(h3), [h4] "=&v"(h4), [h5] "=&v"(h5), [h6] "=&v"(h6), [h7] "=&v"(h7), [t0] "=&v"(t0), [t1] "=&v"(t1), [t2] "=&v"(t2), [t3] "=&v"(t3), [t4] "=&v"(t4), [t5] "=&v"(t5), [t6] "=&v"(t6), [t7] "=&v"(t7), [vt1] "=&v"(vt1), [vt3] "=&v"(vt3), [vt4] "=&v"(vt4), [acc] "+v"(acc), [scy] "=&s"(scy), [sby] "=&s"(sby)
+                 : [a0] "v"(a0), [a1] "v"(a1), [a2] "v"(a2), [a3] "v"(a3), [a4] "v"(a4), [a5] "v"(a5), [a6] "v"(a6), [a7] "v"(a7), [b0] "v"(b0), [b1] "v"(b1), [b2] "v"(b2), [b3] "v"(b3), [b4] "v"(b4), [b5] "v"(b5), [b6] "v"(b6), [b7] "v"(b7));
+    fe_fix_fast_asm(h0, h1, h4, h7, vt1);
+    fe_subp_fast_asm(t0, t1, t7, vt4);
+    o0[0] = h0; o0[1] = h1; o0[2] = h2; o0[3] = h3; o0[4] = h4; o0[5] = h5; o0[6] = h6; o0[7] = h7;
+    o1[0] = t0; o1[1] = t1; o1[2] = t2; o1[3] = t3; o1[4] = t4; o1[5] = t5; o1[6] = t6; o1[7] = t7;
+    (void)scy; (void)sby; (void)vt1; (void)vt3; (void)vt4;
+}
+}
diff --git a/cudabulletproof_amd/csrc/ge25519_dev.h b/cudabulletproof_amd/csrc/ge25519_dev.h
--- a/cudabulletproof_amd/csrc/ge25519_dev.h
+++ b/cudabulletproof_amd/csrc/ge25519_dev.h
@@ -27,7 +27,8 @@
     return fe{{0x75EB4DCA135978A3ull, 0x00700A4D4141D8ABull, 0x8CC740797779E898ull, 0x52036CEE2B6FFE73ull}};
 }
 
-BP_DEV fe fe_mul_k(const fe& f) {
+template <int LAT = 0>
+BP_DEV fe fe_mul_k(const fe& f, uint32_t* acc = nullptr) {
 #if BP_MUL_ASM && defined(__HIP_DEVICE_COMPILE__)
     uint32_t a[8], w[16];
 #pragma unroll
@@ -39,7 +40,7 @@
     uint64_t t[8];
 #pragma unroll
     for (int i = 0; i < 8; i++) t[i] = (uint64_t)w[2 * i] | ((uint64_t)w[2 * i + 1] << 32);
-    return fe_fold512(t);
+    return fe_fold512<LAT>(t, acc);
 #else
     return fe_mul(f, k_const());
 #endif
@@ -163,6 +164,82 @@
     return ge{fe_mul(E, F), fe_mul(G, H), fe_mul(F, G), fe_mul(E, H)};
 }
 
+#ifndef BP_LANE_DEFER
+#define BP_LANE_DEFER 1
+#endif
+#ifndef BP_DEFER_CHUNK
+#define BP_DEFER_CHUNK 32
+#endif
+constexpr int DEFER_WARM = 2;
+struct Defer {
+    uint32_t acc = 0, gacc = 0;
+};
+BP_DEV bool defer_hit(const Defer& d) {
+    return __builtin_amdgcn_ballot_w64((d.acc == 0xFFFFFFFFu) | (d.gacc > MUL_BOUNDED_WORD)) != 0;
+}
+
+BP_DEV void lane_addsub_d(const fe& f, const fe& g, fe& sum, fe& diff, Defer& d) {
+#if BP_LANE_ADDSUB
+    fe_addsub<3>(f, g, sum, diff, &d.acc);
+#else
+    diff = fe_sub<3>(f, g, &d.acc);
+    sum = fe_add<3>(f, g, &d.acc);
+#endif
+}
+
+BP_DEV ge ge_dbl_d(const ge& p, Defer& d) {
+    fe A = fe_sq<3>(fe_sub<3>(p.Y, p.X, &d.acc), &d.acc, &d.gacc);
+    fe B = fe_sq<3>(fe_add<3>(p.Y, p.X, &d.acc), &d.acc, &d.gacc);
+    fe C = fe_mul_k<3>(fe_sq<3>(p.T, &d.acc, &d.gacc), &d.acc);
+    fe D = fe_sq<3>(p.Z, &d.acc, &d.gacc);
+    D = fe_add<3>(D, D, &d.acc);
+    fe E, F, G, H;
+    lane_addsub_d(B, A, H, E, d);
+    lane_addsub_d(D, C, G, F, d);
+    return ge{fe_mul<3>(E, F, &d.acc, &d.gacc), fe_mul<3>(G, H, &d.acc, &d.gacc), fe_mul<3>(F, G, &d.acc, &d.gacc),
+              fe_mul<3>(E, H, &d.acc, &d.gacc)};
+}
+
+template <bool QLDS>
+BP_DEV ge ge_add_qp_d(const ge& p, const geq* q, bool zone, Defer& d) {
+    fe A = fe_mul<3>(fe_sub<3>(p.Y, p.X, &d.acc), qget<QLDS>(&q->YmX), &d.acc, &d.gacc);
+    fe B = fe_mul<3>(fe_add<3>(p.Y, p.X, &d.acc), qget<QLDS>(&q->YpX), &d.acc, &d.gacc);
+    fe C = fe_mul_k<3>(fe_mul<3>(p.T, qget<QLDS>(&q->T), &d.acc, &d.gacc), &d.acc);
+    fe D = zone ? fe_mul_one(p.Z) : fe_mul<3>(p.Z, qget<QLDS>(&q->Z), &d.acc, &d.gacc);
+    D = fe_add<3>(D, D, &d.acc);
+    fe E, F, G, H;
+    lane_addsub_d(B, A, H, E, d);
+    lane_addsub_d(D, C, G, F, d);
+    return ge{fe_mul<3>(E, F, &d.acc, &d.gacc), fe_mul<3>(G, H, &d.acc, &d.gacc), fe_mul<3>(F, G, &d.acc, &d.gacc),
+              fe_mul<3>(E, H, &d.acc, &d.gacc)};
+}
+
+template <bool QLDS, bool ZONE = false>
+BP_DEV ge ge_add_sel_d(const ge& p, const geq* q, bool use_q, Defer& d) {
+    fe ymx = fe_sub<3>(p.Y, p.X, &d.acc);
+    fe qa = qget<QLDS>(&q->YmX);
+    fe A = fe_mul<3>(ymx, use_q ? qa : ymx, &d.acc, &d.gacc);
+    fe ypx = fe_add<3>(p.Y, p.X, &d.acc);
+    fe qb = qget<QLDS>(&q->YpX);
+    fe B = fe_mul<3>(ypx, use_q ? qb : ypx, &d.acc, &d.gacc);
+    fe qt = qget<QLDS>(&q->T);
+    fe C = fe_mul_k<3>(fe_mul<3>(p.T, use_q ? qt : p.T, &d.acc, &d.gacc), &d.acc);
+    fe D;
+    if (ZONE) {
+        fe d1 = fe_mul_one(p.Z), d2 = fe_sq<3>(p.Z, &d.acc, &d.gacc);
+        D = use_q ? d1 : d2;
+    } else {
+        fe qz = qget<QLDS>(&q->Z);
+        D = fe_mul<3>(p.Z, use_q ? qz : p.Z, &d.acc, &d.gacc);
+    }
+    D = fe_add<3>(D, D, &d.acc);
+    fe E, F, G, H;
+    lane_addsub_d(B, A, H, E, d);
+    lane_addsub_d(D, C, G, F, d);
+    return ge{fe_mul<3>(E, F, &d.acc, &d.gacc), fe_mul<3>(G, H, &d.acc, &d.gacc), fe_mul<3>(F, G, &d.acc, &d.gacc),
+              fe_mul<3>(E, H, &d.acc, &d.gacc)};
+}
+
 struct BitStream {
     uint64_t cur, n1, n2, n3;
     int left;
@@ -219,6 +296,40 @@
         if (bs_next(bs)) r = ge_add_qp<QLDS>(r, q, zone);
     }
     return r;
+}
+
+template <bool QLDS, bool FORCE>
+BP_DEV bool sm_uniform_d(ge& out, const fe& s_in, const geq* q, const ge* __restrict__ dtab, const ge* ptab, int K) {
+    fe s;
+#pragma unroll
+    for (int i = 0; i < 4; i++) {
+        uint32_t lo = __builtin_amdgcn_readfirstlane((uint32_t)s_in.v[i]);
+        uint32_t hi = __builtin_amdgcn_readfirstlane((uint32_t)(s_in.v[i] >> 32));
+        s.v[i] = (uint64_t)lo | ((uint64_t)hi << 32);
+    }
+    int lz = fe_clz256(s);
+    const bool pre = K > 0 && lz < K && __all(ptab != nullptr);
+    const int top = pre ? 255 - K : 255 - lz;
+    ge r = ld_ge(pre ? &ptab[prefix_index(s, K)] : &dtab[lz]);
+    if (top >= 0) {
+        const bool zone = __all(fe_is_one(qget<QLDS>(&q->Z)));
+        BitStream bs = bs_init(s, top);
+        r = ge_dbl(r);
+        if (bs_next(bs)) r = ge_add_qp<QLDS>(r, q, zone);
+        Defer d;
+        int n = 0;
+        for (int i = top - 1; i >= 0; i--) {
+            r = ge_dbl_d(r, d);
+            if (bs_next(bs)) r = ge_add_qp_d<QLDS>(r, q, zone, d);
+            if (++n == BP_DEFER_CHUNK) {
+                n = 0;
+                if (FORCE || __builtin_expect(defer_hit(d), 0)) return false;
+            }
+        }
+        if (__builtin_expect(defer_hit(d), 0)) return false;
+    }
+    out = r;
+    return true;
 }
 
 template <bool QLDS, bool ZONE>
@@ -243,13 +354,64 @@
     return r;
 }
 
-template <bool QLDS>
+template <bool QLDS, bool ZONE, bool FORCE>
+BP_DEV bool sm_lane_loop_d(ge& out, const fe& s, const geq* q, const ge* __restrict__ dtab, const ge* ptab, int K) {
+    int lz = fe_clz256(s);
+    const bool pre = K > 0 && lz < K && ptab != nullptr;
+    ge r = ld_ge(pre ? &ptab[prefix_index(s, K)] : &dtab[lz]);
+    int i = pre ? 255 - K : 255 - lz;
+    BitStream bs = bs_init(s, i < 0 ? 0 : i);
+    uint32_t bit = i >= 0 ? bs_next(bs) : 0;
+    bool add_phase = false;
+    for (int warm = 0; warm < DEFER_WARM && i >= 0; warm++) {
+        r = ge_add_sel<QLDS, ZONE>(r, q, add_phase);
+        if (!add_phase && bit) {
+            add_phase = true;
+        } else {
+            add_phase = false;
+            i--;
+            bit = bs_next(bs);
+        }
+    }
+    Defer d;
+    int n = 0;
+    bool hit = false;
+    while (i >= 0) {
+        r = ge_add_sel_d<QLDS, ZONE>(r, q, add_phase, d);
+        if (!add_phase && bit) {
+            add_phase = true;
+        } else {
+            add_phase = false;
+            i--;
+            bit = bs_next(bs);
+        }
+        if (++n == BP_DEFER_CHUNK) {
+            n = 0;
+            if (FORCE || __builtin_expect(defer_hit(d), 0)) {
+                hit = true;
+                break;
+            }
+        }
+    }
+    if (__builtin_expect(__builtin_amdgcn_ballot_w64(hit) != 0 || defer_hit(d), 0)) return false;
+    out = r;
+    return true;
+}
+
+template <bool QLDS, bool FORCE = false>
 BP_DEV ge sm_lane(const fe& s, const geq* q, const ge* __restrict__ dtab, const ge* ptab, int K) {
-    if (__all(fe_is_one(qget<QLDS>(&q->Z)))) return sm_lane_loop<QLDS, true>(s, q, dtab, ptab, K);
+    const bool zone = __all(fe_is_one(qget<QLDS>(&q->Z)));
+#if BP_LANE_DEFER
+    ge r;
+    if (zone ? sm_lane_loop_d<QLDS, true, FORCE>(r, s, q, dtab, ptab, K)
+             : sm_lane_loop_d<QLDS, false, FORCE>(r, s, q, dtab, ptab, K))
+        return r;
+#endif
+    if (zone) return sm_lane_loop<QLDS, true>(s, q, dtab, ptab, K);
     return sm_lane_loop<QLDS, false>(s, q, dtab, ptab, K);
 }
 
-template <bool QLDS>
+template <bool QLDS, bool FORCE = false>
 BP_DEV ge scalarmult(const fe& s, const ge& P, geq* slot, const ge* __restrict__ dtab, const ge* ptab = nullptr,
                      int K = 0) {
     geq qreg;
@@ -274,8 +436,14 @@
         uint32_t lo = (uint32_t)s.v[i], hi = (uint32_t)(s.v[i] >> 32);
         same &= (lo == __builtin_amdgcn_readfirstlane(lo)) & (hi == __builtin_amdgcn_readfirstlane(hi));
     }
-    if (__all(same)) return sm_uniform<QLDS>(s, q, dtab, ptab, K);
-    return sm_lane<QLDS>(s, q, dtab, ptab, K);
-}
-
-}
+    if (__all(same)) {
+#if BP_LANE_DEFER
+        ge r;
+        if (sm_uniform_d<QLDS, FORCE>(r, s, q, dtab, ptab, K)) return r;
+#endif
+        return sm_uniform<QLDS>(s, q, dtab, ptab, K);
+    }
+    return sm_lane<QLDS, FORCE>(s, q, dtab, ptab, K);
+}
+
+}
diff --git a/include/cudabulletproof_hip.h b/include/cudabulletproof_hip.h
--- a/include/cudabulletproof_hip.h
+++ b/include/cudabulletproof_hip.h
@@ -194,6 +194,7 @@
 int hipbp_point_tree(ge25519* result, const ge25519* points, size_t n, void* stream);
 int hipbp_field_op(int op, fe25519* r, const fe25519* a, const fe25519* b, size_t count, void* stream);
 int hipbp_sha_probe(int kind, fe25519* out, const fe25519* in, size_t count, void* stream);
+int hipbp_sm_probe(int force, ge25519* out, const fe25519* scalars, const ge25519* points, size_t count, void* stream);
 int hipbp_release_stream_workspaces(void* stream);
 int hipbp_sync(void* stream);
 
```
